# gmweir/PYFFT

Measured on AMD Instinct MI355X. Metric: Msamples/sec Welch-PSD 4096-pt Hann 50% overlap, complex64, higher is better.
Workload: dtype f32

## Files before the change

include/spectral.h:

```cpp
#ifndef SPECTRAL_H
#define SPECTRAL_H

#include <stdint.h>

#ifdef __cplusplus
extern "C" {
#endif

#define SP_DTYPE_F32 0
#define SP_DTYPE_C64 1

#define SP_SIDED_ONE 1
#define SP_SIDED_TWO 2
#define SP_SIDED_RAW 3
#define SP_SIDED_HALF 4

int sp_init(int device_id);
void sp_shutdown(void);
const char *sp_last_error(void);
int sp_set_stream(void *hip_stream);
int sp_synchronize(void);
int sp_version(void);
int sp_max_wg_fft(void);
int sp_profile_enable(int on);
int sp_profile_last_ms(double *ms);
const char *sp_profile_last_kernel(void);
int sp_device_info(int64_t out[4]);

int sp_fft_c2c(const void *in, void *out, int64_t n, int64_t batch, int direction, int mem);

#define SP_DETREND_CONST 0
#define SP_DETREND_MEAN 1
#define SP_DETREND_LINEAR 2
#define SP_DETREND_SEGMEAN 3
#define SP_DETREND_SEGLINEAR 4
int sp_welch_psd(const void *x, int x_dtype, int64_t nsig, const float *win, int nfft, int hop,
                 int64_t nframes, int detrend, double mean_re, double mean_im, int sided,
                 double scale, double *pxx_out, int mem);

int sp_welch_accum(const void *x, int x_dtype, int64_t nsig, const float *win, int nfft, int hop, int64_t nframes,
                   int64_t nmean, double *sum_out, int mem);
int sp_welch_finish(const double *mean, int64_t frames_total, int sided, double scale, double *pxx_out, int mem);
int sp_welch_export(const void *x, int x_dtype, int64_t nsig, const float *win, int nfft, int hop,
                    int64_t nframes, int64_t nmean, double *state, int mem);
int sp_welch_apply(const double *state, const float *win, int nfft, int64_t frames_total, int sided, double scale,
                   double *pxx_out, int mem);

#define SP_COMM_ID_BYTES 128
int sp_comm_unique_id(void *id_out );
int sp_comm_init(const void *id, int world, int rank);
int sp_comm_info(int out[2] );
int sp_comm_destroy(void);
int sp_welch_dist_submit(const void *x, int x_dtype, int64_t nsig, const float *win, int nfft, int hop, int64_t nframes,
                         int64_t nmean, int64_t frames_total, int sided, double scale, double *pxx_out, int *ndone);
int sp_welch_dist_flush(int *ndone);
int sp_welch_psd_dist(const void *x, int x_dtype, int64_t nsig, const float *win, int nfft, int hop, int64_t nframes,
                      int64_t nmean, int64_t frames_total, int sided, double scale, double *pxx_out);

int sp_welch_csd(const void *x, const void *y, int dtype, int64_t nsig, int nch, int64_t y_ld,
                 const float *win, int nfft, int hop, int64_t nframes, int detrend,
                 const double *mean_x , const double *mean_y , int sided,
                 double scale, double *pxx, double *pyy, double *pxy, int mem);

int sp_csd_matrix(const float *x, int nch, int64_t nsig, int64_t x_ld, const float *win, int nfft,
                  int hop, int64_t nframes, int detrend, double scale, double *g_out, int mem);
int sp_csd_matrix_means(const float *x, int nch, int64_t nsig, int64_t x_ld, const float *win, int nfft,
                        int hop, int64_t nframes, const double *means, double scale, double *g_out, int mem);
int sp_channel_means(const float *x, int nch, int64_t nsig, int64_t x_ld, double *means_out, int mem);

int sp_stft(const void *x, int x_dtype, int64_t nsig, const float *win, int nfft, int hop, int64_t nframes,
            int detrend, double mean_re, double mean_im, int sided, double amp_scale, int out_kind,
            int out_major, void *out, double *pseg_out, int mem);

int sp_istft(const void *Z, int sided, int in_major, int nch, int64_t nframes, const float *win, int nfft, int hop,
             double scale, int64_t skip, int64_t nout, void *y, int mem);

int sp_bispectrum(const void *x, const void *y, const void *z, int x_dtype, int64_t nsig, const float *win, int nfft, int hop,
                  int64_t nframes, int detrend, double mean_re, double mean_im, void *B_out, double *b2_out, double *pzz_out,
                  int mem);

int sp_stft_cog(const void *x, int x_dtype, int64_t nsig, const float *win, int nfft, int hop, int64_t nframes,
                int detrend, double mean_re, double mean_im, double fs, double fmin, double fmax, double *cog_out, int mem);

int sp_hilbert(const float *x, int64_t n_in, int64_t x_ld, int64_t nfft, int64_t batch, void *out, int mem);

int sp_frame_sum(const void *x, int x_dtype, int64_t nsig, int nch, int64_t x_ld, int nfft, int hop, int64_t nframes,
                 int detrend, double *out, int mem);

int sp_spectral_filter(const float *x, int64_t n_in, int64_t x_ld, int64_t nfft, int64_t batch, const void *H, void *out,
                       int mem);

int sp_xcorr(const float *x1, const float *x2, int64_t n, float *co_out, int mem);

int sp_fftfilt(const float *h, int ntaps, const float *x, int64_t n, int nfft, float *y, int mem);

int64_t sp_csd_epilogue_doubles(int nch, int nb, int nfft);
int sp_csd_epilogue(const double *pxx, const double *pyy, const double *pxy, int nch, int nb, int nfft, int onesided, double enbw,
                    double *out, int mem);

int sp_biquad(const double *b, const double *a, const float *x, int64_t n, float *y, int mem);

int sp_sosfilt(const double *sos, int nsec, const float *x, int64_t nrows, int64_t n, const double *zi, float *y, double *zf,
               int mem);
int sp_sosfiltfilt(const double *sos, int nsec, const float *x, int64_t nrows, int64_t n, int padtype, int64_t padlen, float *y,
                   int mem);

int sp_mean(const void *x, int x_dtype, int64_t n, double out[2], int mem);

#ifdef __cplusplus
}
#endif
#endif
```

pyfft_amd/_ffi.py:

```python
import ctypes as C
import os

import numpy as np

_HERE = os.path.dirname(os.path.abspath(__file__))
LIB_PATH = os.environ.get("SP_LIB_PATH") or os.path.join(_HERE, "lib", "libspectral.so")

DTYPE_F32, DTYPE_C64 = 0, 1
SIDED_ONE, SIDED_TWO, SIDED_RAW, SIDED_HALF = 1, 2, 3, 4
DETREND_CONST, DETREND_MEAN, DETREND_LINEAR, DETREND_SEGMEAN, DETREND_SEGLINEAR = 0, 1, 2, 3, 4

_lib = None

_vp, _i, _i64, _d = C.c_void_p, C.c_int, C.c_int64, C.c_double

SIGNATURES = {
    "sp_init": (_i, [_i]),
    "sp_shutdown": (None, []),
    "sp_last_error": (C.c_char_p, []),
    "sp_set_stream": (_i, [_vp]),
    "sp_synchronize": (_i, []),
    "sp_version": (_i, []),
    "sp_max_wg_fft": (_i, []),
    "sp_device_info": (_i, [C.POINTER(_i64)]),
    "sp_profile_enable": (_i, [_i]),
    "sp_profile_last_ms": (_i, [C.POINTER(_d)]),
    "sp_profile_last_kernel": (C.c_char_p, []),
    "sp_fft_c2c": (_i, [_vp, _vp, _i64, _i64, _i, _i]),
    "sp_welch_psd": (_i, [_vp, _i, _i64, _vp, _i, _i, _i64, _i, _d, _d, _i, _d, _vp, _i]),
    "sp_welch_accum": (_i, [_vp, _i, _i64, _vp, _i, _i, _i64, _i64, _vp, _i]),
    "sp_welch_finish": (_i, [_vp, _i64, _i, _d, _vp, _i]),
    "sp_welch_export": (_i, [_vp, _i, _i64, _vp, _i, _i, _i64, _i64, _vp, _i]),
    "sp_welch_apply": (_i, [_vp, _vp, _i, _i64, _i, _d, _vp, _i]),
    "sp_comm_unique_id": (_i, [_vp]),
    "sp_comm_init": (_i, [_vp, _i, _i]),
    "sp_comm_info": (_i, [C.POINTER(_i)]),
    "sp_comm_destroy": (_i, []),
    "sp_welch_dist_submit": (_i, [_vp, _i, _i64, _vp, _i, _i, _i64, _i64, _i64, _i, _d, _vp, C.POINTER(_i)]),
    "sp_welch_dist_flush": (_i, [C.POINTER(_i)]),
    "sp_welch_psd_dist": (_i, [_vp, _i, _i64, _vp, _i, _i, _i64, _i64, _i64, _i, _d, _vp]),
    "sp_welch_csd": (_i, [_vp, _vp, _i, _i64, _i, _i64, _vp, _i, _i, _i64, _i, _vp, _vp, _i, _d, _vp, _vp, _vp, _i]),
    "sp_csd_matrix": (_i, [_vp, _i, _i64, _i64, _vp, _i, _i, _i64, _i, _d, _vp, _i]),
    "sp_csd_matrix_means": (_i, [_vp, _i, _i64, _i64, _vp, _i, _i, _i64, _vp, _d, _vp, _i]),
    "sp_channel_means": (_i, [_vp, _i, _i64, _i64, _vp, _i]),
    "sp_stft": (_i, [_vp, _i, _i64, _vp, _i, _i, _i64, _i, _d, _d, _i, _d, _i, _i, _vp, _vp, _i]),
    "sp_istft": (_i, [_vp, _i, _i, _i, _i64, _vp, _i, _i, _d, _i64, _i64, _vp, _i]),
    "sp_bispectrum": (_i, [_vp, _vp, _vp, _i, _i64, _vp, _i, _i, _i64, _i, _d, _d, _vp, _vp, _vp, _i]),
    "sp_stft_cog": (_i, [_vp, _i, _i64, _vp, _i, _i, _i64, _i, _d, _d, _d, _d, _d, _vp, _i]),
    "sp_hilbert": (_i, [_vp, _i64, _i64, _i64, _i64, _vp, _i]),
    "sp_frame_sum": (_i, [_vp, _i, _i64, _i, _i64, _i, _i, _i64, _i, _vp, _i]),
    "sp_spectral_filter": (_i, [_vp, _i64, _i64, _i64, _i64, _vp, _vp, _i]),
    "sp_xcorr": (_i, [_vp, _vp, _i64, _vp, _i]),
    "sp_fftfilt": (_i, [_vp, _i, _vp, _i64, _i, _vp, _i]),
    "sp_biquad": (_i, [_vp, _vp, _vp, _i64, _vp, _i]),
    "sp_sosfilt": (_i, [_vp, _i, _vp, _i64, _i64, _vp, _vp, _vp, _i]),
    "sp_sosfiltfilt": (_i, [_vp, _i, _vp, _i64, _i64, _i, _i64, _vp, _i]),
    "sp_csd_epilogue_doubles": (_i64, [_i, _i, _i]),
    "sp_csd_epilogue": (_i, [_vp, _vp, _vp, _i, _i, _i, _i, _d, _vp, _i]),
    "sp_mean": (_i, [_vp, _i, _i64, C.POINTER(_d), _i]),
}


class SpectralError(RuntimeError):
    pass


def load_library():
    global _lib
    if _lib is not None:
        return _lib
    if not os.path.exists(LIB_PATH):
        raise SpectralError("libspectral.so not found at %s -- run `make` (or __graft_entry__.build()); "
                            "pyfft_amd has no CPU fallback" % LIB_PATH)
    lib = C.CDLL(LIB_PATH)
    for name, (res, args) in SIGNATURES.items():
        fn = getattr(lib, name)
        fn.restype = res
        fn.argtypes = args
    _lib = lib
    return lib


def lib():
    l = load_library()
    return l


def check(rc):
    if rc != 0:
        raise SpectralError((lib().sp_last_error() or b"unknown error").decode())


def init(device=-1):
    check(lib().sp_init(int(device)))


def ptr(a):
    if a is None:
        return None
    if isinstance(a, (int, np.integer)):
        return C.c_void_p(int(a))
    assert a.flags["C_CONTIGUOUS"]
    return C.c_void_p(a.ctypes.data)


def dtype_code(arr_dtype):
    if arr_dtype == np.float32:
        return DTYPE_F32
    if arr_dtype == np.complex64:
        return DTYPE_C64
    raise TypeError("device path takes float32 or complex64 samples, got %s" % arr_dtype)


def as_samples(x):
    x = np.asarray(x)
    if np.iscomplexobj(x):
        return np.ascontiguousarray(x, dtype=np.complex64)
    return np.ascontiguousarray(x, dtype=np.float32)
```

pyfft_amd/csrc/fft_core.h:

```cpp
#pragma once
#include <type_traits>
#include <hip/hip_runtime.h>

namespace sp {

typedef float2 cf;

__device__ __forceinline__ cf mk(float a, float b) { return make_float2(a, b); }
__device__ __forceinline__ cf operator+(cf a, cf b) { return mk(a.x + b.x, a.y + b.y); }
__device__ __forceinline__ cf operator-(cf a, cf b) { return mk(a.x - b.x, a.y - b.y); }
__device__ __forceinline__ cf operator*(float s, cf a) { return mk(s * a.x, s * a.y); }
__device__ __forceinline__ cf cmul(cf a, cf b) { return mk(a.x * b.x - a.y * b.y, a.x * b.y + a.y * b.x); }
__device__ __forceinline__ cf cmulc(cf a, cf b) { return mk(a.x * b.x + a.y * b.y, a.y * b.x - a.x * b.y); }
__device__ __forceinline__ cf cconj(cf a) { return mk(a.x, -a.y); }
__device__ __forceinline__ float cnorm(cf a) { return a.x * a.x + a.y * a.y; }

template <bool INV> __device__ __forceinline__ cf rot(cf a) { return INV ? mk(-a.y, a.x) : mk(a.y, -a.x); }
template <bool INV> __device__ __forceinline__ cf twc(cf a, float C, float S) {
    return INV ? mk(a.x * C - a.y * S, a.y * C + a.x * S) : mk(a.x * C + a.y * S, a.y * C - a.x * S);
}
template <bool INV> __device__ __forceinline__ cf twm(cf a, cf w) { return INV ? cmulc(a, w) : cmul(a, w); }

#define SP_C8 0.70710678118654752440f
#define SP_C16 0.92387953251128675613f
#define SP_S16 0.38268343236508977173f

template <bool INV> __device__ __forceinline__ void dft2(cf &a, cf &b) {
    cf t = a - b;
    a = a + b;
    b = t;
}

template <bool INV> __device__ __forceinline__ void dft4(cf &a, cf &b, cf &c, cf &d) {
    cf t0 = a + c, t1 = a - c, t2 = b + d, t3 = rot<INV>(b - d);
    a = t0 + t2;
    c = t0 - t2;
    b = t1 + t3;
    d = t1 - t3;
}

template <bool INV> __device__ __forceinline__ void dft8(cf (&x)[8]) {
    dft4<INV>(x[0], x[2], x[4], x[6]);
    dft4<INV>(x[1], x[3], x[5], x[7]);
    cf o1 = twc<INV>(x[3], SP_C8, SP_C8);
    cf o2 = rot<INV>(x[5]);
    cf o3 = twc<INV>(x[7], -SP_C8, SP_C8);
    cf e0 = x[0], e1 = x[2], e2 = x[4], e3 = x[6], o0 = x[1];
    x[0] = e0 + o0;
    x[4] = e0 - o0;
    x[1] = e1 + o1;
    x[5] = e1 - o1;
    x[2] = e2 + o2;
    x[6] = e2 - o2;
    x[3] = e3 + o3;
    x[7] = e3 - o3;
}

template <bool INV> __device__ __forceinline__ void dft16(cf (&x)[16]) {
#pragma unroll
    for (int b = 0; b < 4; ++b) dft4<INV>(x[b], x[b + 4], x[b + 8], x[b + 12]);
    x[5] = twc<INV>(x[5], SP_C16, SP_S16);
    x[9] = twc<INV>(x[9], SP_C8, SP_C8);
    x[13] = twc<INV>(x[13], SP_S16, SP_C16);
    x[6] = twc<INV>(x[6], SP_C8, SP_C8);
    x[10] = rot<INV>(x[10]);
    x[14] = twc<INV>(x[14], -SP_C8, SP_C8);
    x[7] = twc<INV>(x[7], SP_S16, SP_C16);
    x[11] = twc<INV>(x[11], -SP_C8, SP_C8);
    x[15] = twc<INV>(x[15], -SP_C16, -SP_S16);
#pragma unroll
    for (int c = 0; c < 4; ++c) dft4<INV>(x[4 * c], x[4 * c + 1], x[4 * c + 2], x[4 * c + 3]);
    cf t;
#define SP_SWAP(i, j) t = x[i]; x[i] = x[j]; x[j] = t;
    SP_SWAP(1, 4) SP_SWAP(2, 8) SP_SWAP(3, 12) SP_SWAP(6, 9) SP_SWAP(7, 13) SP_SWAP(11, 14)
#undef SP_SWAP
}

struct Tw16 {
    float f[40];
    static constexpr int TAU = 0, RB = 15, RC = 19, RD = 23, S1 = 27, S2 = 31, S3 = 35;
};

#define SP_T16 0.41421356237309504880f
#define SP_T316 2.41421356237309504880f

__device__ __forceinline__ void dft4s(cf &a, cf &b, cf &c, cf &d, float rb, float rc, float rd) {
    const cf t0 = mk(fmaf(rc, c.x, a.x), fmaf(rc, c.y, a.y));
    const cf t1 = mk(fmaf(-rc, c.x, a.x), fmaf(-rc, c.y, a.y));
    const cf t2 = mk(fmaf(rd, d.x, b.x), fmaf(rd, d.y, b.y));
    const cf t3 = mk(fmaf(-rd, d.x, b.x), fmaf(-rd, d.y, b.y));
    a = mk(fmaf(rb, t2.x, t0.x), fmaf(rb, t2.y, t0.y));
    c = mk(fmaf(-rb, t2.x, t0.x), fmaf(-rb, t2.y, t0.y));
    b = mk(fmaf(rb, t3.y, t1.x), fmaf(-rb, t3.x, t1.y));
    d = mk(fmaf(-rb, t3.y, t1.x), fmaf(rb, t3.x, t1.y));
}
__device__ __forceinline__ cf rot_tan(cf a, float t) { return mk(fmaf(t, a.y, a.x), fmaf(-t, a.x, a.y)); }

template <bool TWD, bool PREROT = false> __device__ __forceinline__ void dft16s(cf (&x)[16], const Tw16 &w) {
    if constexpr (TWD) {
        if constexpr (!PREROT) {
#pragma unroll
            for (int s = 1; s < 16; ++s) x[s] = rot_tan(x[s], w.f[Tw16::TAU + s - 1]);
        }
#pragma unroll
        for (int b = 0; b < 4; ++b) dft4s(x[b], x[b + 4], x[b + 8], x[b + 12], w.f[Tw16::RB + b], w.f[Tw16::RC + b], w.f[Tw16::RD + b]);
    } else {
#pragma unroll
        for (int b = 0; b < 4; ++b) dft4<false>(x[b], x[b + 4], x[b + 8], x[b + 12]);
    }
    x[5] = rot_tan(x[5], SP_T16);
    x[9] = mk(x[9].x + x[9].y, x[9].y - x[9].x);
    x[13] = rot_tan(x[13], SP_T316);
    x[6] = mk(x[6].x + x[6].y, x[6].y - x[6].x);
    x[10] = mk(x[10].y, -x[10].x);
    x[14] = mk(x[14].x - x[14].y, x[14].y + x[14].x);
    x[7] = rot_tan(x[7], SP_T316);
    x[11] = mk(x[11].x - x[11].y, x[11].y + x[11].x);
    x[15] = rot_tan(x[15], SP_T16);
    if constexpr (TWD) {
#pragma unroll
        for (int c = 0; c < 4; ++c) dft4s(x[4 * c], x[4 * c + 1], x[4 * c + 2], x[4 * c + 3], w.f[Tw16::S1 + c], w.f[Tw16::S2 + c], w.f[Tw16::S3 + c]);
    } else {
        dft4<false>(x[0], x[1], x[2], x[3]);
        dft4s(x[4], x[5], x[6], x[7], SP_C16, SP_C8, SP_S16 / SP_C16);
        dft4s(x[8], x[9], x[10], x[11], SP_C8, 1.f, -1.f);
        dft4s(x[12], x[13], x[14], x[15], SP_S16, -SP_C8, -SP_C16 / SP_S16);
    }
    cf t;
#define SP_SWAP(i, j) t = x[i]; x[i] = x[j]; x[j] = t;
    SP_SWAP(1, 4) SP_SWAP(2, 8) SP_SWAP(3, 12) SP_SWAP(6, 9) SP_SWAP(7, 13) SP_SWAP(11, 14)
#undef SP_SWAP
}

template <bool TWD, class Store, bool PREROT = false> __device__ __forceinline__ void dft16s_es(cf (&x)[16], const Tw16 &w, Store store) {
    if constexpr (TWD) {
        if constexpr (!PREROT) {
#pragma unroll
            for (int s = 1; s < 16; ++s) x[s] = rot_tan(x[s], w.f[Tw16::TAU + s - 1]);
        }
#pragma unroll
        for (int b = 0; b < 4; ++b) dft4s(x[b], x[b + 4], x[b + 8], x[b + 12], w.f[Tw16::RB + b], w.f[Tw16::RC + b], w.f[Tw16::RD + b]);
    } else {
#pragma unroll
        for (int b = 0; b < 4; ++b) dft4<false>(x[b], x[b + 4], x[b + 8], x[b + 12]);
    }
    x[5] = rot_tan(x[5], SP_T16);
    x[9] = mk(x[9].x + x[9].y, x[9].y - x[9].x);
    x[13] = rot_tan(x[13], SP_T316);
    x[6] = mk(x[6].x + x[6].y, x[6].y - x[6].x);
    x[10] = mk(x[10].y, -x[10].x);
    x[14] = mk(x[14].x - x[14].y, x[14].y + x[14].x);
    x[7] = rot_tan(x[7], SP_T316);
    x[11] = mk(x[11].x - x[11].y, x[11].y + x[11].x);
    x[15] = rot_tan(x[15], SP_T16);
    __builtin_amdgcn_sched_barrier(0);
#define SP_ES_OUT(c)                                                                                                 \
    store(c, x[4 * c]);                                                                                              \
    store(c + 4, x[4 * c + 1]);                                                                                      \
    store(c + 8, x[4 * c + 2]);                                                                                      \
    store(c + 12, x[4 * c + 3]);                                                                                     \
    __builtin_amdgcn_sched_barrier(0);
    if constexpr (TWD) {
        dft4s(x[0], x[1], x[2], x[3], w.f[Tw16::S1 + 0], w.f[Tw16::S2 + 0], w.f[Tw16::S3 + 0]);
        SP_ES_OUT(0)
        dft4s(x[4], x[5], x[6], x[7], w.f[Tw16::S1 + 1], w.f[Tw16::S2 + 1], w.f[Tw16::S3 + 1]);
        SP_ES_OUT(1)
        dft4s(x[8], x[9], x[10], x[11], w.f[Tw16::S1 + 2], w.f[Tw16::S2 + 2], w.f[Tw16::S3 + 2]);
        SP_ES_OUT(2)
        dft4s(x[12], x[13], x[14], x[15], w.f[Tw16::S1 + 3], w.f[Tw16::S2 + 3], w.f[Tw16::S3 + 3]);
        SP_ES_OUT(3)
    } else {
        dft4<false>(x[0], x[1], x[2], x[3]);
        SP_ES_OUT(0)
        dft4s(x[4], x[5], x[6], x[7], SP_C16, SP_C8, SP_S16 / SP_C16);
        SP_ES_OUT(1)
        dft4s(x[8], x[9], x[10], x[11], SP_C8, 1.f, -1.f);
        SP_ES_OUT(2)
        dft4s(x[12], x[13], x[14], x[15], SP_S16, -SP_C8, -SP_C16 / SP_S16);
        SP_ES_OUT(3)
    }
#undef SP_ES_OUT
}

__device__ __forceinline__ void dft4w(cf &a, cf &b, cf &c, cf &d, float wa, float wb, float wc, float wd) {
    const cf pa = mk(wa * a.x, wa * a.y), pb = mk(wb * b.x, wb * b.y);
    const cf t0 = mk(fmaf(wc, c.x, pa.x), fmaf(wc, c.y, pa.y));
    const cf t1 = mk(fmaf(-wc, c.x, pa.x), fmaf(-wc, c.y, pa.y));
    const cf t2 = mk(fmaf(wd, d.x, pb.x), fmaf(wd, d.y, pb.y));
    const cf t3 = mk(fmaf(-wd, d.x, pb.x), fmaf(-wd, d.y, pb.y));
    a = t0 + t2;
    c = t0 - t2;
    b = mk(t1.x + t3.y, t1.y - t3.x);
    d = mk(t1.x - t3.y, t1.y + t3.x);
}
struct NoMid {
    __device__ __forceinline__ void operator()(int) const {}
};
template <class Store, class Mid = NoMid> __device__ __forceinline__ void dft16s_es_win(cf (&x)[16], const float (&w)[16], Store store, Mid mid = Mid()) {
#pragma unroll
    for (int b = 0; b < 4; ++b) {
        dft4w(x[b], x[b + 4], x[b + 8], x[b + 12], w[b], w[b + 4], w[b + 8], w[b + 12]);
        if constexpr (!std::is_same<Mid, NoMid>::value) {
            if (b < 3) {
                __builtin_amdgcn_sched_barrier(0);
                mid(b);
                __builtin_amdgcn_sched_barrier(0);
            }
        }
    }
    x[5] = rot_tan(x[5], SP_T16);
    x[9] = mk(x[9].x + x[9].y, x[9].y - x[9].x);
    x[13] = rot_tan(x[13], SP_T316);
    x[6] = mk(x[6].x + x[6].y, x[6].y - x[6].x);
    x[10] = mk(x[10].y, -x[10].x);
    x[14] = mk(x[14].x - x[14].y, x[14].y + x[14].x);
    x[7] = rot_tan(x[7], SP_T316);
    x[11] = mk(x[11].x - x[11].y, x[11].y + x[11].x);
    x[15] = rot_tan(x[15], SP_T16);
    __builtin_amdgcn_sched_barrier(0);
#define SP_ES_OUT(c)                                                                                                 \
    store(c, x[4 * c]);                                                                                              \
    store(c + 4, x[4 * c + 1]);                                                                                      \
    store(c + 8, x[4 * c + 2]);                                                                                      \
    store(c + 12, x[4 * c + 3]);                                                                                     \
    __builtin_amdgcn_sched_barrier(0);
    dft4<false>(x[0], x[1], x[2], x[3]);
    SP_ES_OUT(0)
    dft4s(x[4], x[5], x[6], x[7], SP_C16, SP_C8, SP_S16 / SP_C16);
    SP_ES_OUT(1)
    dft4s(x[8], x[9], x[10], x[11], SP_C8, 1.f, -1.f);
    SP_ES_OUT(2)
    dft4s(x[12], x[13], x[14], x[15], SP_S16, -SP_C8, -SP_C16 / SP_S16);
    SP_ES_OUT(3)
#undef SP_ES_OUT
}

__device__ __forceinline__ void make_tw16(Tw16 &w, const cf (&wv)[15]) {
    float g[16];
    g[0] = 1.f;
    w.f[39] = 0.f;
#pragma unroll
    for (int s = 1; s < 16; ++s) {
        float c = wv[s - 1].x;
        if (fabsf(c) < 9.094947e-13f) c = c < 0.f ? -9.094947e-13f : 9.094947e-13f;
        g[s] = c;
        w.f[Tw16::TAU + s - 1] = -wv[s - 1].y / c;
    }
#pragma unroll
    for (int b = 0; b < 4; ++b) {
        w.f[Tw16::RB + b] = g[b + 4] / g[b];
        w.f[Tw16::RC + b] = g[b + 8] / g[b];
        w.f[Tw16::RD + b] = g[b + 12] / g[b + 4];
    }
    const float K1[4] = {1.f, SP_C16, SP_C8, SP_S16}, K2[4] = {1.f, SP_C8, 1.f, -SP_C8}, K3[4] = {1.f, SP_S16, -SP_C8, -SP_C16};
#pragma unroll
    for (int c = 0; c < 4; ++c) {
        w.f[Tw16::S1 + c] = g[1] * K1[c];
        w.f[Tw16::S2 + c] = g[2] * K2[c];
        w.f[Tw16::S3 + c] = (g[3] * K3[c]) / (g[1] * K1[c]);
    }
}

typedef float sp_f2v __attribute__((ext_vector_type(2)));
__device__ __forceinline__ cf lds_load_single(const cf *p) { return *p; }
template <int RDX, bool INV> __device__ __forceinline__ void dftR(cf (&x)[RDX]) {
    if constexpr (RDX == 2) dft2<INV>(x[0], x[1]);
    else if constexpr (RDX == 4) dft4<INV>(x[0], x[1], x[2], x[3]);
    else if constexpr (RDX == 8) dft8<INV>(x);
    else if constexpr (RDX == 16) dft16<INV>(x);
}

constexpr int ilog2c(int n) { return n <= 1 ? 0 : 1 + ilog2c(n >> 1); }

template <int N> struct FftPlan {
    static_assert(N >= 2 && (N & (N - 1)) == 0, "power of two");
    static constexpr int LOG2N = ilog2c(N);
    static constexpr int R = N < 16 ? N : 16;
    static constexpr int T = N / R;
    static constexpr int NP16 = N < 16 ? 0 : LOG2N / 4;
    static constexpr int REM = N < 16 ? N : (1 << (LOG2N % 4));
    static constexpr int NP = N < 16 ? 1 : NP16 + (REM > 1 ? 1 : 0);
    static constexpr int radix(int p) { return N < 16 ? N : (p < NP16 ? 16 : REM); }
    static constexpr int ns(int p) { int s = 1; for (int i = 0; i < p; ++i) s *= radix(i); return s; }
    static constexpr int ntw_before(int p) { int c = 0; for (int i = 1; i < p; ++i) c += (R / radix(i)) * (radix(i) - 1); return c; }
    static constexpr int NTW = ntw_before(NP);
    static constexpr int PITCH1 = T + 1;
    static constexpr int LDS_ELEMS = NP > 1 ? (R * PITCH1 > N ? R * PITCH1 : N) : 0;
};

#define SP_TW1_PITCH 44
template <int N, bool TW1LDS = false> struct WgFft {
    using PL = FftPlan<N>;
    static constexpr int R = PL::R, T = PL::T, NP = PL::NP;
    static constexpr int IMG0 = PL::LDS_ELEMS;
    static constexpr int N16 = PL::NP16 > 1 ? PL::NP16 - 1 : 0;
    static constexpr int NTR = (N >= 16 && PL::REM > 1) ? (R / PL::REM) * (PL::REM - 1) : 0;
    Tw16 t16[N16 > 0 ? N16 : 1];
    cf twr[NTR > 0 ? NTR : 1];
    const float *tw1 = nullptr;

    __device__ __forceinline__ void publish_tw1(float *table, int tid) {
        if constexpr (TW1LDS && N16 > 0) {
            if (tid < 16) {
#pragma unroll
                for (int j = 0; j < 40; ++j) table[tid * SP_TW1_PITCH + j] = t16[0].f[j];
            }
            tw1 = table;
        }
    }

    __device__ __forceinline__ void load_twiddles(const cf *__restrict__ table, int tid) {
        load_tw<1>(table, tid);
    }

    template <int P> __device__ __forceinline__ void load_tw(const cf *__restrict__ table, int tid) {
        if constexpr (P < NP) {
            constexpr int r = PL::radix(P), NS = PL::ns(P), NB = R / r;
            if constexpr (r == 16) {
                const int e = (tid % NS) * (N / (NS * 16));
                cf wv[15];
#pragma unroll
                for (int s = 1; s < 16; ++s) wv[s - 1] = table[e * s];
                make_tw16(t16[P - 1], wv);
            } else {
#pragma unroll
                for (int u = 0; u < NB; ++u) {
                    const int q = tid + T * u;
                    const int e = (q % NS) * (N / (NS * r));
#pragma unroll
                    for (int s = 1; s < r; ++s) twr[u * (r - 1) + (s - 1)] = table[e * s];
                }
            }
            load_tw<P + 1>(table, tid);
        }
    }

    template <int P> __device__ __forceinline__ void load_tw_one(const cf *__restrict__ table, int tid) {
        static_assert(P >= 1 && P < NP && PL::radix(P) == 16, "a twiddled radix-16 pass");
        constexpr int NS = PL::ns(P);
        const int e = (tid % NS) * (N / (NS * 16));
        cf wv[15];
#pragma unroll
        for (int s = 1; s < 16; ++s) wv[s - 1] = table[e * s];
        make_tw16(t16[P - 1], wv);
    }

    template <int E> static __device__ __forceinline__ int phys(int i) {
        if constexpr (E == 0) return (i % PL::radix(0)) * PL::PITCH1 + i / PL::radix(0);
        else return i;
    }

    template <int P> __device__ __forceinline__ void bfly(cf (&v)[R], int tid) const {
        constexpr int r = PL::radix(P), NB = R / r;
#pragma unroll
        for (int u = 0; u < NB; ++u) {
            cf x[r];
#pragma unroll
            for (int s = 0; s < r; ++s) x[s] = v[u + s * NB];
            if constexpr (r == 16) {
                if constexpr (TW1LDS && P == 1) {
                    Tw16 wl;
                    const float4 *row = reinterpret_cast<const float4 *>(tw1 + (tid % 16) * SP_TW1_PITCH);
#pragma unroll
                    for (int j = 0; j < 10; ++j) {
                        const float4 q = row[j];
                        wl.f[4 * j] = q.x;
                        wl.f[4 * j + 1] = q.y;
                        wl.f[4 * j + 2] = q.z;
                        wl.f[4 * j + 3] = q.w;
                    }
                    dft16s<true>(x, wl);
                } else if constexpr (P > 0) {
                    dft16s<true>(x, t16[P - 1]);
                } else {
                    dft16s<false>(x, t16[0]);
                }
            } else {
                if constexpr (P > 0) {
#pragma unroll
                    for (int s = 1; s < r; ++s) x[s] = twm<false>(x[s], twr[u * (r - 1) + (s - 1)]);
                }
                dftR<r, false>(x);
            }
#pragma unroll
            for (int s = 0; s < r; ++s) v[u + s * NB] = x[s];
        }
    }
    template <int P> __device__ __forceinline__ void scatter(const cf (&v)[R], cf *lds, int tid) const {
        constexpr int r = PL::radix(P), NS = PL::ns(P), NB = R / r;
#pragma unroll
        for (int u = 0; u < NB; ++u) {
            const int q = tid + T * u;
            const int base = (q / NS) * (NS * r) + (q % NS);
#pragma unroll
            for (int s = 0; s < r; ++s) lds[phys<P>(base + s * NS)] = v[u + s * NB];
        }
    }
    template <int P> __device__ __forceinline__ void gather(cf (&v)[R], const cf *lds, int tid) const {
        if constexpr (P == 0 && (T % 16) == 0 && PL::radix(0) == 16) {
            const int b = (tid % 16) * PL::PITCH1 + tid / 16;
#pragma unroll
            for (int t = 0; t < R; ++t) v[t] = lds_load_single(&lds[b + (T / 16) * t]);
        } else {
#pragma unroll
            for (int t = 0; t < R; ++t) v[t] = lds_load_single(&lds[phys<P>(tid + T * t)]);
        }
    }

    template <bool SINGLE, bool WL = false> __device__ __forceinline__ void run(cf (&v)[R], cf *lds0, cf *lds1, int tid) const {
        static_assert(!WL || T <= 64, "wave-local exchange: one wave holds the whole transform");
        pass<0, SINGLE, WL>(v, lds0, lds1, tid);
    }
    template <bool WL> static __device__ __forceinline__ void xsync() {
        if constexpr (WL) __builtin_amdgcn_wave_barrier();
        else __syncthreads();
    }

    template <int P> __device__ __forceinline__ void bfly_scatter(cf (&v)[R], cf *lds, int tid) const {
        constexpr int NS = PL::ns(P);
        const int base = (tid / NS) * (NS * 16) + (tid % NS);
        auto store = [&](int k, cf val) __attribute__((always_inline)) { lds[phys<P>(base + k * NS)] = val; };
        if constexpr (P > 0) dft16s_es<true>(v, t16[P - 1], store);
        else dft16s_es<false>(v, t16[0], store);
    }

    template <int P> __device__ __forceinline__ void load_tau_out(const cf *__restrict__ table, int tid, float (&tau)[16]) const {
        static_assert(P + 1 < NP && PL::radix(P) == 16 && PL::radix(P + 1) == 16 && R == 16, "between two radix-16 passes");
        constexpr int NS = PL::ns(P), NS2 = PL::ns(P + 1);
#pragma unroll
        for (int k = 0; k < 16; ++k) {
            const int p = (tid / NS) * (NS * 16) + (tid % NS) + k * NS;
            const int tc = p % T, sc = p / T;
            const int e = (tc % NS2) * (N / (NS2 * 16));
            const cf w = table[(e * sc) & (N - 1)];
            float c = w.x;
            if (fabsf(c) < 9.094947e-13f) c = c < 0.f ? -9.094947e-13f : 9.094947e-13f;
            tau[k] = sc == 0 ? 0.f : -w.y / c;
        }
    }
    template <int P, bool PREROT> __device__ __forceinline__ void bfly_scatter_rot(cf (&v)[R], const float (&tau)[16], cf *lds, int tid) const {
        constexpr int NS = PL::ns(P);
        const int base = (tid / NS) * (NS * 16) + (tid % NS);
        auto store = [&](int k, cf val) __attribute__((always_inline)) { lds[phys<P>(base + k * NS)] = rot_tan(val, tau[k]); };
        if constexpr (P > 0) dft16s_es<true, decltype(store), PREROT>(v, t16[P - 1], store);
        else dft16s_es<false>(v, t16[0], store);
    }
    __device__ __forceinline__ void bfly_scatter_win_rot(cf (&v)[R], const float (&w)[R], const float (&tau)[16], cf *lds, int tid) const {
        static_assert(R == 16, "radix-16 first pass");
        constexpr int NS = PL::ns(0);
        const int base = (tid / NS) * (NS * 16) + (tid % NS);
        auto store = [&](int k, cf val) __attribute__((always_inline)) { lds[phys<0>(base + k * NS)] = rot_tan(val, tau[k]); };
        dft16s_es_win(v, w, store);
    }
    template <int P> __device__ __forceinline__ void bfly_prerot(cf (&v)[R], int tid) const {
        (void)tid;
        static_assert(P > 0 && PL::radix(P) == 16 && R == 16, "a twiddled radix-16 pass");
        dft16s<true, true>(v, t16[P - 1]);
    }

    __device__ __forceinline__ void bfly_scatter_win(cf (&v)[R], const float (&w)[R], cf *lds, int tid) const {
        static_assert(R == 16, "radix-16 first pass");
        constexpr int NS = PL::ns(0);
        const int base = (tid / NS) * (NS * 16) + (tid % NS);
        auto store = [&](int k, cf val) __attribute__((always_inline)) { lds[phys<0>(base + k * NS)] = val; };
        dft16s_es_win(v, w, store);
    }

    template <int P, bool SINGLE, bool WL = false> __device__ __forceinline__ void pass(cf (&v)[R], cf *lds0, cf *lds1, int tid) const {
        constexpr bool LAST = (P == NP - 1);
        cf *lds = (P & 1) ? lds1 : lds0;
        if constexpr (!LAST && SINGLE) xsync<WL>();
        bfly<P>(v, tid);
        if constexpr (!LAST) {
            scatter<P>(v, lds, tid);
            xsync<WL>();
            gather<P>(v, lds, tid);
            pass<P + 1, SINGLE, WL>(v, lds0, lds1, tid);
        }
    }
};

}
```

pyfft_amd/csrc/k_welch_pipe.hip:

```cpp
#include "launch.h"
#include <type_traits>
#define SP_PIPE_AHEAD 2
namespace sp {

template <bool CPLX, int SHIFT, int MODE>
__global__ __launch_bounds__(768) void k_welch_pipe(const void *__restrict__ x_in, const float *__restrict__ win,
                                                     int64_t nframes, int64_t fpg, float *__restrict__ trend_in, XfTables tb,
                                                     float *__restrict__ partial, cf *__restrict__ spartial, int64_t x_cs, int gpr) {
    constexpr int N = 4096;
    constexpr bool RP = MODE >= 3 && MODE != 8 && MODE != 9;
    constexpr bool ONEPASS = MODE == 1 || MODE == 4 || MODE == 7 || MODE == 8 || MODE == 9, COG = MODE == 2 || MODE == 8;
    constexpr bool LOBE = MODE == 9;
    constexpr bool SPEC = MODE == 5 || MODE == 7;
    const void *x = SPEC ? (const void *)(reinterpret_cast<const float *>(x_in) + (int64_t)blockIdx.y * x_cs) : x_in;
    float *trend = SPEC ? trend_in + 4 * blockIdx.y : trend_in;
    static_assert(!RP || (!CPLX && SHIFT == 8), "the real-pair form is for real input at hop = nfft / 2");
    using PL = FftPlan<N>;
    using F = WgFft<N>;
    constexpr int T = PL::T, R = PL::R, KEEP = R - SHIFT, IMG = F::IMG0, IMGB = PL::LDS_ELEMS;
    static_assert(T == 256 && R == 16 && PL::NP == 3, "three radix-16 passes over 256 threads");
    extern __shared__ __attribute__((aligned(16))) unsigned char smem_raw[];
    cf *smem = reinterpret_cast<cf *>(smem_raw);
    cf *imgA = smem, *imgB = smem + 2 * IMG;
    const int role = __builtin_amdgcn_readfirstlane((int)threadIdx.x >> 8);
    const int tid = (int)threadIdx.x & 255;
    const int hop = SHIFT * T;

    cf mu;
    if constexpr (ONEPASS) {
        const int64_t span = (nframes - 1) * (int64_t)hop + N;
        const int64_t pitch = span / 16;
        constexpr int NU = SPEC ? 4 : 1, NTH = SPEC ? 3 * T : T, NWV = SPEC ? 12 : 4;
        const int lt = SPEC ? (int)threadIdx.x : tid;
        float sx = 0.f, sy = 0.f;
#pragma unroll
        for (int r = 0; r < 16; ++r)
#pragma unroll
            for (int u = 0; u < NU; ++u) {
                int64_t i = pitch * r + (int64_t)(lt + NTH * u);
                i = i < span ? i : span - 1;
                const cf v = load_sample(x, i, CPLX);
                sx += v.x;
                sy += v.y;
            }
        sx = wave_sum64(sx);
        sy = wave_sum64(sy);
        float *red = reinterpret_cast<float *>(smem);
        if ((SPEC || role == 0) && (tid & 63) == 0) {
            red[2 * (lt >> 6)] = sx;
            red[2 * (lt >> 6) + 1] = sy;
        }
        __syncthreads();
        double tx = 0.0, ty = 0.0;
#pragma unroll
        for (int wv = 0; wv < NWV; ++wv) {
            tx += (double)red[2 * wv];
            ty += (double)red[2 * wv + 1];
        }
        mu = mk((float)(tx / (16.0 * NTH * NU)), (float)(ty / (16.0 * NTH * NU)));
        __syncthreads();
        if (blockIdx.x == 0 && threadIdx.x == 0) {
            trend[0] = mu.x;
            trend[1] = mu.y;
            trend[2] = 0.f;
            trend[3] = 0.f;
        }
    } else {
        mu = load_trend(trend).m;
    }
    const int64_t gid = blockIdx.x;
    const int64_t g0 = gid * fpg;
    const int64_t last = nframes - 1;
    int64_t trips = (RP ? (nframes + 1) / 2 : nframes) - g0;
    trips = trips < 0 ? 0 : (trips > fpg ? fpg : trips);
    constexpr int DRAIN = 4;
    const int64_t periods = trips + DRAIN;
    F f;
    constexpr bool UPROT = !RP;
    float tau_out[16];
    if constexpr (UPROT) {
        if (role == 0) f.template load_tau_out<0>(tb.tw, tid, tau_out);
        else if (role == 1) f.template load_tau_out<1>(tb.tw, tid, tau_out);
    }

    if (role == 0 && RP) {
        const float *xr = reinterpret_cast<const float *>(x);
        float m = mu.x;
        asm volatile("" : "+v"(m));
        float w[R], sacc[SHIFT];
#pragma unroll
        for (int t = 0; t < R; ++t) w[t] = win[tid + T * t];
#pragma unroll
        for (int s = 0; s < SHIFT; ++s) sacc[s] = 0.f;
        auto issue_chunk = [&](float (&dst)[R], int64_t q) __attribute__((always_inline)) {
            const int64_t q1 = 2 * q <= nframes ? q : 0, q2 = 2 * q + 1 <= nframes ? q : 0;
            const float *b1 = xr + q1 * (int64_t)N, *b2 = xr + q2 * (int64_t)N;
#pragma unroll
            for (int t = 0; t < R; ++t) {
                const unsigned off = (unsigned)(tid + T * t);
                dst[t] = __builtin_nontemporal_load((t < R / 2 ? b1 : b2) + off);
            }
        };
        float ca[R], cb[R], cc[R];
        issue_chunk(ca, g0);
        issue_chunk(cb, g0 + 1);
#pragma unroll
        for (int t = 0; t < R; ++t) {
            ca[t] -= m;
            cb[t] -= m;
        }
        auto frame = [&](auto hb, int64_t i, cf *img, float (&cur)[R], float (&nxt)[R], float (&fill)[R]) __attribute__((always_inline)) {
            constexpr bool HB = decltype(hb)::value;
            issue_chunk(fill, g0 + i + 2);
            __builtin_amdgcn_sched_barrier(0);
            cf v[R];
            if constexpr (!ONEPASS) {
#pragma unroll
                for (int t = 0; t < R; ++t) v[t] = mk(cur[t], HB ? (t < R / 2 ? cur[t + R / 2] : nxt[t - R / 2]) : 0.f);
                if constexpr (UPROT) f.bfly_scatter_win_rot(v, w, tau_out, img, tid);
                else f.bfly_scatter_win(v, w, img, tid);
            } else {
#pragma unroll
                for (int t = 0; t < R; ++t) v[t] = mk(w[t] * cur[t], HB ? w[t] * (t < R / 2 ? cur[t + R / 2] : nxt[t - R / 2]) : 0.f);
                if constexpr (UPROT) f.template bfly_scatter_rot<0, false>(v, tau_out, img, tid);
                else f.template bfly_scatter<0>(v, img, tid);
            }
            __builtin_amdgcn_sched_barrier(0);
            if constexpr (ONEPASS) {
#pragma unroll
                for (int s = 0; s < SHIFT; ++s) sacc[s] += HB ? cur[R / 2 + s] + nxt[s] : cur[R / 2 + s];
            }
#pragma unroll
            for (int t = 0; t < R; ++t) fill[t] -= m;
        };
        const std::true_type yes;
        const std::false_type no;
        int64_t i = 0;
        for (; i + 6 < trips; i += 6) {
            frame(yes, i, imgA, ca, cb, cc);
            __syncthreads();
            frame(yes, i + 1, imgA + IMG, cb, cc, ca);
            __syncthreads();
            frame(yes, i + 2, imgA, cc, ca, cb);
            __syncthreads();
            frame(yes, i + 3, imgA + IMG, ca, cb, cc);
            __syncthreads();
            frame(yes, i + 4, imgA, cb, cc, ca);
            __syncthreads();
            frame(yes, i + 5, imgA + IMG, cc, ca, cb);
            __syncthreads();
        }
        for (; i < trips; ++i) {
            cf *img = (i & 1) ? imgA + IMG : imgA;
            const bool has_b = 2 * (g0 + i) + 1 < nframes;
            if (has_b) {
                if (i % 3 == 0) frame(yes, i, img, ca, cb, cc);
                else if (i % 3 == 1) frame(yes, i, img, cb, cc, ca);
                else frame(yes, i, img, cc, ca, cb);
            } else {
                if (i % 3 == 0) frame(no, i, img, ca, cb, cc);
                else if (i % 3 == 1) frame(no, i, img, cb, cc, ca);
                else frame(no, i, img, cc, ca, cb);
            }
            __syncthreads();
        }
#pragma unroll
        for (int d = 0; d < DRAIN; ++d) __syncthreads();
        if constexpr (ONEPASS) {
#pragma unroll
            for (int s = 0; s < SHIFT; ++s)
                spartial[((SPEC ? (int64_t)blockIdx.y * gridDim.x : 0) + gid) * hop + tid + T * s] = mk(sacc[s], 0.f);
        }
    } else if (role == 0) {
        asm volatile("" : "+v"(mu.x), "+v"(mu.y));
        float w[R];
        cf sacc[SHIFT], raw[R];
#pragma unroll
        for (int t = 0; t < R; ++t) w[t] = win[tid + T * t];
#pragma unroll
        for (int s = 0; s < SHIFT; ++s) sacc[s] = mk(0.f, 0.f);
        {
            const int64_t base = (g0 < nframes ? g0 : last) * hop + tid;
#pragma unroll
            for (int t = 0; t < R; ++t) raw[t] = load_sample(x, base + T * t, CPLX) - mu;
        }
        auto issue_part = [&](cf (&dst)[SHIFT], int64_t q, int s0, int s1) __attribute__((always_inline)) {
            const int64_t gq = g0 + q;
            const int64_t gn = gq < nframes ? gq : last;
            const int64_t ubase = gn * hop + (int64_t)T * KEEP;
#pragma unroll
            for (int s = s0; s < s1; ++s) {
                const unsigned off = (unsigned)(tid + T * s);
                if (CPLX) {
                    const sp_f2v r = __builtin_nontemporal_load(reinterpret_cast<const sp_f2v *>(x) + ubase + off);
                    dst[s] = mk(r.x, r.y);
                } else {
                    dst[s] = mk(__builtin_nontemporal_load(reinterpret_cast<const float *>(x) + ubase + off), 0.f);
                }
            }
        };
        auto issue = [&](cf (&dst)[SHIFT], int64_t q) __attribute__((always_inline)) { issue_part(dst, q, 0, SHIFT); };
        constexpr int AHEAD = (SP_PIPE_AHEAD >= 2 && SHIFT <= 8) ? (SP_PIPE_AHEAD >= 3 ? 3 : 2) : 1;
        constexpr bool SPREAD = AHEAD >= 2;
        auto frame = [&](int64_t i, cf *img, cf (&fill)[SHIFT], cf (&take)[SHIFT]) __attribute__((always_inline)) {
            if constexpr (SPREAD) issue_part(fill, i + AHEAD, 0, SHIFT / 4);
            else issue(fill, i + AHEAD);
            __builtin_amdgcn_sched_barrier(0);
            cf v[R];
            constexpr bool WINFOLD = SPREAD;
#pragma unroll
            for (int t = 0; t < R; ++t) v[t] = WINFOLD ? raw[t] : w[t] * raw[t];
            if constexpr (SPREAD) {
            {
                auto store = [&](int k, cf val) __attribute__((always_inline)) {
                    img[F::template phys<0>(tid * 16 + k)] = UPROT ? rot_tan(val, tau_out[k]) : val;
                    if (k >= 12 && k < 15) issue_part(fill, i + AHEAD, (k - 11) * (SHIFT / 4), (k - 10) * (SHIFT / 4));
                };
                if constexpr (WINFOLD) dft16s_es_win(v, w, store);
                else dft16s_es<false>(v, f.t16[0], store);
            }
            } else {
            if constexpr (UPROT) f.template bfly_scatter_rot<0, false>(v, tau_out, img, tid);
            else f.template bfly_scatter<0>(v, img, tid);
            }
            __builtin_amdgcn_sched_barrier(0);
#pragma unroll
            for (int s = 0; s < SHIFT; ++s)
                if constexpr (ONEPASS && !LOBE) sacc[s] = sacc[s] + raw[KEEP + s];
#pragma unroll
            for (int t = 0; t < KEEP; ++t) raw[t] = raw[t + SHIFT];
#pragma unroll
            for (int s = 0; s < SHIFT; ++s) raw[KEEP + s] = take[s] - mu;
        };
        int64_t i = 0;
        if constexpr (AHEAD == 3) {
            cf s0[SHIFT], s1[SHIFT], s2[SHIFT];
            issue(s1, 1);
            issue(s2, 2);
            for (; i + 2 < trips; i += 3) {
                frame(i, (i & 1) ? imgA + IMG : imgA, s0, s1);
                __syncthreads();
                frame(i + 1, ((i + 1) & 1) ? imgA + IMG : imgA, s1, s2);
                __syncthreads();
                frame(i + 2, ((i + 2) & 1) ? imgA + IMG : imgA, s2, s0);
                __syncthreads();
            }
            for (; i < trips; ++i) {
                cf *img = (i & 1) ? imgA + IMG : imgA;
                if (i % 3 == 0) frame(i, img, s0, s1);
                else if (i % 3 == 1) frame(i, img, s1, s2);
                else frame(i, img, s2, s0);
                __syncthreads();
            }
        } else if constexpr (AHEAD == 2) {
            cf nxa[SHIFT], nxb[SHIFT];
            issue(nxa, 1);
            for (; i + 1 < trips; i += 2) {
                frame(i, imgA, nxb, nxa);
                __syncthreads();
                frame(i + 1, imgA + IMG, nxa, nxb);
                __syncthreads();
            }
            if (i < trips) {
                frame(i, imgA, nxb, nxa);
                __syncthreads();
            }
        } else {
            for (; i + 1 < trips; i += 2) {
                cf nx0[SHIFT], nx1[SHIFT];
                frame(i, imgA, nx0, nx0);
                __syncthreads();
                frame(i + 1, imgA + IMG, nx1, nx1);
                __syncthreads();
            }
            if (i < trips) {
                cf nx0[SHIFT];
                frame(i, imgA, nx0, nx0);
                __syncthreads();
            }
        }
#pragma unroll
        for (int d = 0; d < DRAIN; ++d) __syncthreads();
#pragma unroll
        for (int s = 0; s < SHIFT; ++s)
            if constexpr (ONEPASS && !LOBE) spartial[gid * hop + tid + T * s] = sacc[s];
    } else if (role == 1) {
        f.template load_tw_one<1>(tb.tw, tid);
        cf va[R], vb[R];
        auto step = [&](cf (&fill)[R], cf (&use)[R], int64_t p, const cf *src, cf *dst) __attribute__((always_inline)) {
            if (p >= 1 && p <= trips) f.template gather<0>(fill, src, tid);
            if (p >= 2 && p <= trips + 1) {
                if constexpr (UPROT) f.template bfly_scatter_rot<1, true>(use, tau_out, dst, tid);
                else f.template bfly_scatter<1>(use, dst, tid);
            }
            __syncthreads();
        };
        for (int64_t p = 0; p < periods; p += 2) {
            step(va, vb, p, imgA + IMG, imgB);
            if (p + 1 < periods) step(vb, va, p + 1, imgA, imgB + IMGB);
        }
    } else {
        f.template load_tw_one<2>(tb.tw, tid);
        float acc[R];
#pragma unroll
        for (int t = 0; t < R; ++t) acc[t] = 0.f;
        cf bs_lo = mk(0.f, 0.f), bs_hi = mk(0.f, 0.f);
        const unsigned zlo = (unsigned)((tid >> 3) * 512 + (tid & 7));
        cf held[SPEC ? R : 1];
        cf va[R], vb[R];
        cf pend = mk(0.f, 0.f);
        auto flush = [&](int64_t i) __attribute__((always_inline)) {
            const int sel = (int)(i & 63), li = tid & 63;
            const int64_t gg = g0 + (i - sel) + li;
            if (li <= sel && gg < nframes) reinterpret_cast<cf *>(partial)[(int64_t)(tid >> 6) * nframes + gg] = pend;
        };
        auto step = [&](cf (&fill)[R], cf (&use)[R], int64_t p, const cf *src) __attribute__((always_inline)) {
            if (p >= 3 && p <= trips + 2) {
                f.template gather<1>(fill, src, tid);
            }
            if (p >= 4 && p <= trips + 3) {
                if constexpr (UPROT) f.template bfly_prerot<2>(use, tid);
                else f.template bfly<2>(use, tid);
                if constexpr (SPEC) {
                    const int64_t pr = g0 + (p - 4);
                    const bool lone = (pr & 1) == 0 && p == trips + 3;
                    if ((pr & 1) == 0 && !lone) {
#pragma unroll
                        for (int t = 0; t < R; ++t) held[t] = use[t];
                    } else {
                        float4 *zb = reinterpret_cast<float4 *>(partial) + ((pr >> 1) * (int64_t)gpr * 512 + (int64_t)blockIdx.y * 8);
                        unsigned bl = zlo;
                        asm volatile("" : "+v"(bl));
#pragma unroll
                        for (int t = 0; t < R; ++t) {
                            const float4 q = lone ? make_float4(use[t].x, use[t].y, 0.f, 0.f)
                                                  : make_float4(held[t].x, held[t].y, use[t].x, use[t].y);
                            st_stream(zb + (bl + 16384u * t), q);
                        }
                    }
                } else if constexpr (COG) {
                    if constexpr (MODE == 8) {
                        const int64_t gf = g0 + (p - 4);
                        cf *lobe = reinterpret_cast<cf *>(partial) + 4 * nframes + gf * 8;
                        if (gf < nframes) {
                            if (tid <= 3) lobe[3 + tid] = use[0];
                            if (tid >= T - 3) lobe[3 - (T - tid)] = use[R - 1];
                        }
                    }
                    float numc = 0.f, den = 0.f;
#pragma unroll
                    for (int t = 0; t < R; ++t) {
                        const float pw = cnorm(use[t]);
                        numc = fmaf(pw, (float)(T * t - (t >= R / 2 ? N : 0)), numc);
                        den += pw;
                    }
                    float num = fmaf((float)tid, den, numc);
                    num = wave_sum64(num);
                    den = wave_sum64(den);
                    const int64_t i = p - 4;
                    if ((tid & 63) == (int)(i & 63)) pend = mk(num, den);
                    if ((i & 63) == 63 || i == trips - 1) flush(i);
                } else {
#pragma unroll
                    for (int t = 0; t < R; ++t) acc[t] = fmaf(use[t].y, use[t].y, fmaf(use[t].x, use[t].x, acc[t]));
                    if constexpr (LOBE) {
                        bs_lo = bs_lo + use[0];
                        bs_hi = bs_hi + use[R - 1];
                    }
                }
            }
            __syncthreads();
        };
        for (int64_t p = 0; p < periods; p += 2) {
            step(va, vb, p, imgB + IMGB);
            if (p + 1 < periods) step(vb, va, p + 1, imgB);
        }
        if constexpr (!COG && !SPEC) {
#pragma unroll
            for (int t = 0; t < R; ++t) partial[gid * N + tid + T * t] = acc[t];
            if constexpr (LOBE) {
                if (tid <= 3) spartial[gid * 8 + 3 + tid] = bs_lo;
                if (tid >= T - 3) spartial[gid * 8 + 3 - (T - tid)] = bs_hi;
                if (tid == 4) spartial[gid * 8 + 7] = mk(0.f, 0.f);
            }
        }
    }
}

bool welch_pipe_eligible(const Xf &xf, int hop) {
    return !xf.blue && xf.L == 4096 && (hop == 2048 || hop == 1024 || hop == 4096);
}

int launch_welch_pipe(LaunchCtx c, const void *x, bool cplx, const float *win, int hop, int64_t nframes, float *trend,
                      const Xf &xf, float *partial, const RunPart &rp, cf *spartial, int mode, int nch, int64_t x_cs, int gpr) {
    const size_t lds = sizeof(cf) * 4 * (size_t)FftPlan<4096>::LDS_ELEMS;
#define PIPE_(CP, S, OP)                                                                                  \
    {                                                                                                 \
        static bool once = false;                                                                     \
        if (!once) {                                                                                  \
            if (hipFuncSetAttribute((const void *)k_welch_pipe<CP, S, OP>, hipFuncAttributeMaxDynamicSharedMemorySize, (int)lds) != hipSuccess) \
                return -1;                                                                            \
            once = true;                                                                              \
        }                                                                                             \
        if (c.stop)                                                                                   \
            hipExtLaunchKernelGGL((k_welch_pipe<CP, S, OP>), dim3(rp.blocks, gy), dim3(768), lds, c.stream, nullptr, c.stop, 0, x, win, \
                                  nframes, rp.fpg, trend, xf.tb, partial, spartial, x_cs, gpr);       \
        else                                                                                          \
            hipLaunchKernelGGL((k_welch_pipe<CP, S, OP>), dim3(rp.blocks, gy), dim3(768), lds, c.stream, x, win, nframes, rp.fpg, trend, \
                               xf.tb, partial, spartial, x_cs, gpr);                                  \
    }
    const int shift = hop / 256;
    const unsigned gy = mode == 5 ? (unsigned)nch : 1u;
#define PIPE_S_(CP, OP)                                                                               \
    if (shift == 8) PIPE_(CP, 8, OP) else if (shift == 4) PIPE_(CP, 4, OP) else PIPE_(CP, 16, OP)
    if (mode == 5) {
        if (cplx || shift != 8 || nch < 1 || gpr < 1) return -1;
        if (spartial) PIPE_(false, 8, 7) else PIPE_(false, 8, 5)
    } else if (mode == 3) {
        if (cplx || shift != 8) return -1;
        if (spartial) PIPE_(false, 8, 4) else PIPE_(false, 8, 3)
    } else if (mode == 2 && spartial) {
        if (shift == 8) { if (cplx) PIPE_(true, 8, 8) else PIPE_(false, 8, 8) }
        else if (shift == 4) { if (cplx) PIPE_(true, 4, 8) else PIPE_(false, 4, 8) }
        else return -1;
    } else if (mode == 2) {
        if (cplx) { PIPE_S_(true, 2) } else { PIPE_S_(false, 2) }
    } else if (mode == 9) {
        if (!spartial || shift == 16) return -1;
        if (shift == 8) { if (cplx) PIPE_(true, 8, 9) else PIPE_(false, 8, 9) }
        else { if (cplx) PIPE_(true, 4, 9) else PIPE_(false, 4, 9) }
    } else if (spartial) {
        if (cplx) { PIPE_S_(true, 1) } else { PIPE_S_(false, 1) }
    } else {
        if (cplx) { PIPE_S_(true, 0) } else { PIPE_S_(false, 0) }
    }
#undef PIPE_S_
#undef PIPE_
    return 0;
}

}
```

pyfft_amd/csrc/launch.h:

```cpp
#pragma once
#include <stdlib.h>
#include "kernels.h"
#include <hip/hip_runtime.h>
#include <hip/hip_ext.h>

namespace sp {

inline bool env_flag(const char *name) {
    const char *v = getenv(name);
    return v && v[0] && v[0] != '0';
}
inline int env_int(const char *name, int dflt) {
    const char *v = getenv(name);
    return v ? atoi(v) : dflt;
}

struct LaunchCtx {
    hipStream_t stream;
    int ncu;
    hipEvent_t stop = nullptr;
};

struct Xf {
    XfTables tb;
    int L;
    bool blue;
};

inline int fpw_of(int L) {
    const int R = L < 16 ? L : 16, T = L / R, WG = T >= 256 ? T : 256;
    return WG / T;
}

struct RunPart {
    int64_t groups, fpg;
    int blocks;
};
inline RunPart run_partition(int L, int64_t nframes, int ncu, int groups_per_cu = 0) {
    if (groups_per_cu <= 0) groups_per_cu = 4;
    const int fpw = fpw_of(L);
    const int64_t target = (int64_t)ncu * groups_per_cu * fpw;
    int64_t f = (nframes + target - 1) / target;
    if (f < 1) f = 1;
    const int64_t G = (nframes + f - 1) / f;
    RunPart r;
    r.fpg = f;
    r.blocks = (int)((G + fpw - 1) / fpw);
    r.groups = (int64_t)r.blocks * fpw;
    return r;
}
inline RunPart run_partition_2d(int L, int64_t nframes, int ncu, int ny, int64_t slots = 0) {
    const int fpw = fpw_of(L);
    int64_t target = ((int64_t)ncu * 8 + ny - 1) / (ny > 0 ? ny : 1) * fpw;
    if (target < 8 * fpw) target = 8 * fpw;
    int64_t f = (nframes + target - 1) / target;
    if (f < 1) f = 1;
    if (slots > 0 && ny > 0) {
        const int64_t wg = ((nframes + f - 1) / f + fpw - 1) / fpw * ny;
        int64_t rounds = (wg + slots / 2) / slots;
        if (rounds < 1) rounds = 1;
        const int64_t groups = rounds * slots / ny * fpw;
        if (groups >= 1) {
            const int64_t f2 = (nframes + groups - 1) / groups;
            if (f2 >= 1 && f2 <= 4 * f) f = f2;
        }
    }
    const int64_t G = (nframes + f - 1) / f;
    RunPart r;
    r.fpg = f;
    r.blocks = (int)((G + fpw - 1) / fpw);
    r.groups = (int64_t)r.blocks * fpw;
    return r;
}
inline int strided_blocks(int L, int64_t items, int ncu, int per_cu = 4) {
    const int fpw = fpw_of(L);
    int64_t b = (items + fpw - 1) / fpw;
    int64_t cap = (int64_t)ncu * (L >= 4096 ? per_cu : 16);
    if (L == 2048) {
        const int64_t q = b / 4;
        if (q < cap) cap = q > (int64_t)ncu * 2 ? q : (int64_t)ncu * 2;
    }
    if (b > cap) b = cap;
    if (b < 1) b = 1;
    return (int)b;
}

int resident_per_cu(const void *fn, int threads, size_t lds_bytes);
int welch_rp_groups_per_cu(const Xf &xf, bool lin);
int csd_pair_resident(const Xf &xf, bool lin, bool onepass);
int stft_rp_groups_per_cu(const Xf &xf, bool lin, int hop, int sided, int out_power, bool pseg);

int launch_fft_c2c(LaunchCtx c, const cf *in, cf *out, int64_t batch, int inverse, const Xf &xf,
                   BigTw bt = BigTw{nullptr, nullptr, 0, 0});
int launch_fft_cols(LaunchCtx c, const cf *in, cf *out, int64_t ncols, int64_t nouter, int64_t es, int64_t os, int64_t twmul,
                    int conj_in, const Xf &xf, BigTw bt, int64_t hmask_n = 0,
                    ColsIn ci = ColsIn{0, nullptr, nullptr, nullptr, 0}, int tw_outer = 0);
int launch_fft_rows_rev(LaunchCtx c, const cf *in, cf *out, int64_t A, int64_t B, int conj_out, float scale, const Xf &xf,
                        RowsOut ro = RowsOut{nullptr, 0, 0, nullptr});
int launch_transpose_c(LaunchCtx c, const cf *in, cf *out, int64_t rows, int64_t cols, int conj, float scale, int64_t batch = 1);
int launch_pack_real(LaunchCtx c, const float *x, int64_t n_in, const double *mean, int64_t L, cf *out);
int launch_cmul_vec(LaunchCtx c, const cf *a, const cf *b, int64_t n, int conj_out, cf *out, int64_t batch = 1);
int launch_blue_pre(LaunchCtx c, const cf *in, const cf *chirp, int64_t n, int64_t L, int conj_in, cf *out, int64_t batch = 1);
int launch_blue_post(LaunchCtx c, const cf *in, const cf *chirp, int64_t n, int conj_out, float scale, cf *out, int64_t batch = 1,
                     int64_t in_ld = 0);
int launch_hilbert_mask(LaunchCtx c, cf *X, int64_t n);
int launch_xc_pack(LaunchCtx c, const float *x1, const float *x2, int64_t n, int64_t L, const double *mom, cf *z);
int launch_xc_mid(LaunchCtx c, const cf *Z, int64_t L, cf *R);
int launch_xc_mid_half(LaunchCtx c, const cf *Z, int64_t L, BigTw bt, cf *Zp);
int launch_xc_out(LaunchCtx c, const cf *r, int64_t n, int64_t L, const double *mom, float *co);
bool welch_carry_eligible(const Xf &xf, int hop, bool lin);
int launch_welch(LaunchCtx c, const void *x, bool cplx, const float *win, int hop, int64_t nframes, const float *trend,
                 bool lin, const Xf &xf, float *partial, const RunPart &rp, bool allow_carry, cf *spartial,
                 const char **kname, int segmean = 0);
bool welch_pipe_eligible(const Xf &xf, int hop);
int launch_welch_pipe(LaunchCtx c, const void *x, bool cplx, const float *win, int hop, int64_t nframes, float *trend,
                      const Xf &xf, float *partial, const RunPart &rp, cf *spartial, int mode = 0, int nch = 1, int64_t x_cs = 0,
                      int gpr = 0);
int launch_op_estimate(LaunchCtx c, const void *x, bool cplx, int64_t nsig, double *part, float *trend);
int launch_op_reduce(LaunchCtx c, const void *x, bool cplx, const float *trend, const float *partial, const cf *spartial,
                     int64_t G, const Xf &xf, int hop, int64_t nframes, int64_t nmean, OnePass st, double *sum_out);
int launch_op_finish(LaunchCtx c, const void *x, bool cplx, const float *trend, const float *win, OnePass st,
                     const double *mean_in, int64_t nmean, const Xf &xf, int hop, int64_t nframes, cf *cw, const cf *Wf,
                     int sided, double scale, double *out, bool export_state = false);
int launch_op_apply(LaunchCtx c, const double *state, const cf *Wf, int n, int sided, double scale, double *out,
                    const double *mean = nullptr);
int opx_tot_blocks();
int launch_welch_opx(LaunchCtx c, const void *x, bool cplx, bool pair, const float *win, int hop, int64_t nframes,
                     const float *trend, const Xf &xf, const RunPart &rp, float *partial, cf *cpart);
int launch_opx_reduce(LaunchCtx c, const float *partial, const cf *cpart, int64_t G, const Xf &xf, const void *x, bool cplx,
                      const float *trend, int hop, int64_t nframes, int64_t nmean, double *A, double *csum, double *tpart);
int launch_opx_finish(LaunchCtx c, const float *win, const double *A, const double *csum, const double *tpart, const float *trend,
                      int hop, int64_t nframes, int64_t nmean, bool sym, const Xf &xf, double *out);
int launch_op_fused(LaunchCtx c, const void *x, bool cplx, const float *trend, const float *win, const float *partial,
                    const cf *spartial, int64_t G, int n, int hop, int64_t nframes, int64_t nmean, OnePass st, unsigned *ticket,
                    CogLobe lb, const double *mean_in, int sided, double scale, double *out, bool export_state,
                    OpPrev prev = OpPrev{nullptr, nullptr, nullptr, 0, 0.0}, bool light = false, double cola_c = 0.0);
int launch_welch_finish(LaunchCtx c, const float *partial, int64_t G, const Xf &xf, int sided, double scale, double *out,
                        int sym = 0);
int launch_welch_rp(LaunchCtx c, const float *x, const float *win, int hop, int64_t nframes, const float *trend, bool lin,
                    const Xf &xf, float *partial, const RunPart &rp);
int launch_stft_rp(LaunchCtx c, const float *x, const float *win, int hop, int64_t nframes, const float *trend, bool lin,
                   const Xf &xf, const RunPart &rp, int sided, float amp, int out_power, void *out, double *pseg,
                   int nchan = 1, int64_t x_cs = 0, int64_t out_cs = 0, int out_ld = 0);
int launch_csd(LaunchCtx c, const void *x, const void *y, bool cplx, int nch, int64_t y_ld, const float *win, int hop,
               int64_t nframes, const float *trend_x, const float *trend_y, bool lin, const Xf &xf, float *partial,
               const RunPart &rp, int segmean = 0);
int launch_csd_finish(LaunchCtx c, const float *partial, int64_t G, const Xf &xf, int nch, int sided, double scale,
                      double *pxx, double *pyy, double *pxy);
int launch_stft(LaunchCtx c, const void *x, bool cplx, const float *win, int hop, int64_t nframes, const float *trend,
                bool lin, const Xf &xf, const RunPart &rp, int sided, float amp, int out_power, void *out, double *pseg, int segmean = 0,
                cf *cog = nullptr, int klo = 0, int khi = 0);
int launch_cog_finish(LaunchCtx c, const cf *acc, int wpf, int64_t nframes, double df, double *out);
int launch_cog_carry(LaunchCtx c, const void *x, bool cplx, const float *win, int hop, int64_t nframes, const float *trend,
                     const Xf &xf, cf *cog, const RunPart &rp, int klo, int khi);
bool csd_rp_eligible(const Xf &xf);
int launch_csd_rp(LaunchCtx c, const float *x, const float *y, int nch, int64_t y_ld, const float *win, int hop,
                  int64_t nframes, const float *trend_x, const float *trend_y, bool lin, const Xf &xf, float *partial,
                  const RunPart &rp);
int launch_csd_rp_finish(LaunchCtx c, const float *partial, int64_t G, const Xf &xf, int nch, int sided, double scale,
                         double *pxx, double *pyy, double *pxy);
int launch_pairspec(LaunchCtx c, const float *x, const float *win, int hop, int64_t nframes, const float *trend, bool lin,
                    const Xf &xf, const RunPart &rp, cf *Zx);
int launch_csd_pair(LaunchCtx c, const float *y, int nch, int64_t y_ld, const float *win, int hop, int64_t nframes,
                    float *trend_y, bool lin, const Xf &xf, const cf *Zx, float *partial, const RunPart &rp, cf *spartial = nullptr);
int launch_csd_pair_finish(LaunchCtx c, const float *partial, int64_t G, const Xf &xf, int nch, int sided, double scale,
                           double *pyy, double *pxy, const double *st_y = nullptr, const double *st_x = nullptr, const cf *Wf = nullptr,
                           const float *trend_x = nullptr, const float *trend_y = nullptr, int64_t nmean = 0, int64_t M = 0);
#define SP_COLSUM_SLICES 256
int launch_colsum_real(LaunchCtx c, const float *x, const float *trend, int H, int64_t M, cf *out);
int launch_csdm_finish(LaunchCtx c, double *G, int nch, int nb, double scale);
int launch_csdm_transpose_kgc(LaunchCtx c, const cf *Xs, cf *Xt, int nch, int nchp, int64_t m, int64_t mp, int nb);
int launch_csdm_mfma(LaunchCtx c, const cf *Xt, int nch, int nchp, int64_t mp, int nb, double *G);
int launch_csdm_bf16(LaunchCtx c, const cf *Xs, cf *Xt_tail, int nch, int64_t m, int nb, double *G, int ld, int two_pieces = 0, int init = 0);
int launch_csdm_fold(LaunchCtx c, const double *H, double *G, int nch, int n, const double *st = nullptr, const cf *Wf = nullptr,
                     const float *trend = nullptr, int64_t nmean = 0, int64_t M = 0, double scale = 1.0, int init = 0);
int launch_cm_blocksums(LaunchCtx c, const cf *spartial, int nch, int runs, int hop, double *Sl);
int launch_op_finish_channels(LaunchCtx c, const void *x, int64_t x_cs, int nch, const float *trend, const float *win,
                              const double *Sl, const cf *Wf, int hop, int64_t nframes, int64_t nmean, const Xf &xf, double *out,
                              bool cplx = false);
int launch_cog_finish_op(LaunchCtx c, const cf *acc, int wpf, int64_t nframes, double df, double *out, const cf *lobe, CogLobe lb,
                         const double *st, const float *trend, int64_t nmean, int n);
int launch_csdm_fused(LaunchCtx c, const cf *Xs, cf *Xt_tail, int nch, int64_t m, int nb, double *G, int ld = 0);
int launch_hilbert_mid(LaunchCtx c, cf *Z, int64_t M, BigTw bt);
int launch_hilbert_rowsmid(LaunchCtx c, cf *Tm, int64_t A, int64_t B, const Xf &xc, BigTw btN, const cf *tw2c);
int launch_xc_rowsmid(LaunchCtx c, cf *Tm, int64_t A, int64_t B, const Xf &xc, const Xf &xc2, BigTw btL, BigTw btM);
int launch_fft_cols_lag(LaunchCtx c, const cf *in, int64_t ncols, int64_t nouter, int64_t es, int64_t os, const Xf &xf, RowsOut ro);
int launch_fft_cols_inv(LaunchCtx c, const cf *in, cf *out, int64_t ncols, int64_t nouter, int64_t es, int64_t os, int64_t twmul,
                        const Xf &xf, BigTw bt, float scale, const RowsOut *analytic);
int launch_hilbert(LaunchCtx c, const float *x, int64_t n_in, int64_t x_ld, int64_t batch, const Xf &xf, cf *out,
                   const cf *H = nullptr);
int launch_spec_mul(LaunchCtx c, cf *X, const cf *H, int64_t n);
int frame_sum_slices(int ncu, int nch, int nfft, int64_t nframes);
int launch_frame_sum(LaunchCtx c, const void *x, bool cplx, int64_t x_ld, int nch, int nfft, int hop, int64_t nframes,
                     const float *trend, bool lin, double *out, double *part);
int launch_fftfilt(LaunchCtx c, const float *x, int64_t n, int ntaps, const cf *Hs, const Xf &xf, float *y);
int launch_xcorr(LaunchCtx c, const float *x1, const float *x2, int64_t n, const double *mom, const Xf &xf, float *co);
int launch_moments(LaunchCtx c, const void *x, bool cplx, int64_t n, int mode, double *partial_scratch, double *out_d,
                   float *trend_f, int nsignals = 1, int64_t x_cs = 0);
int launch_moments_xc(LaunchCtx c, const float *x, int64_t n, double *partial, double *out_d, double *xc_out, int64_t x_cs);
int launch_transpose(LaunchCtx c, const void *in, void *out, int64_t rows, int64_t cols, int elem_bytes);
int launch_long_segstats(LaunchCtx c, const void *x, bool cplx, int64_t f0, int64_t m, int hop, int nfft, int mode, float *rec);
int launch_long_pack(LaunchCtx c, const void *x, bool cplx, const float *win, int nfft, int hop, int64_t f0, int64_t m,
                     const float *trend, bool lin, const float *segrec, cf *S, double *pseg);
int launch_long_acc_psd(LaunchCtx c, const cf *S, int64_t m, int nfft, double *acc);
int launch_long_acc_csd(LaunchCtx c, const cf *Sx, const cf *Sy, int64_t m, int nfft, double *ayy, double *axy);
int launch_long_finish(LaunchCtx c, const double *acc, int nfft, int sided, double scale, bool cplx, double *out);
int launch_long_stft_out(LaunchCtx c, const cf *S, int64_t m, int nfft, int sided, float amp, int out_power, void *out,
                         int64_t f0, int nb);
int launch_long_cog(LaunchCtx c, const cf *S, int64_t m, int nfft, int klo, int khi, cf *acc, int64_t f0);

int64_t biquad_tiles(int64_t n);
int launch_biquad(LaunchCtx c, const double *b, const double *a, const float *x, int64_t n, float *y, double *work);

#define SP_SOS_MAXK 8
struct SosIO {
    const float *x;
    int64_t x_ld, n;
    int64_t len;
    int64_t pad;
    int padtype;
    int rev;
    float *y;
    int64_t y_ld, out_off, out_n;
};
int64_t sos_tiles(int64_t len);
int64_t sos_work_doubles(int nsec, int64_t len, int64_t nrows);
int sos_plan_doubles(int nsec);
void sos_build_plan(const double *sos, int nsec, int64_t len, double *plan);
int launch_sos_pass(LaunchCtx c, int nsec, const double *plan, const SosIO &io, int64_t nrows, int zmode, const double *zi,
                    double *zf, double *work);

int launch_epi_elem(LaunchCtx c, const double *pxx, const double *pyy, const double *pxy, int nch, int nb, int nfft, int onesided,
                    double enbw, double *cxy, double *cxy2, double *phi, double *lxx, double *lyy, double *lxy);
int launch_epi_spec(LaunchCtx c, const double *pxx, const double *pyy, const double *pxy, const double *cxy, int nch, int nb,
                    int nfft, int onesided, cf *X, double *rowmax );
int launch_epi_corr(LaunchCtx c, const cf *X, int nch, int nfft, int onesided, double *rxx, double *ryy, double *rxy, double *icxy,
                    double *ee, double *cc, const double *rowmax);

int bispec_tile_dim();
int bispec_frame_chunk();
size_t bispec_part_floats();
int launch_bispec_tile(LaunchCtx c, const cf *X, const cf *Y, const cf *Z, int nb, int c0, int64_t m, const int2 *tiles, int ntiles,
                       float *part);
int launch_bispec_pzz(LaunchCtx c, const cf *Z, int nb, int64_t m, double *ppart);
int launch_bispec_reduce(LaunchCtx c, const float *part, const double *ppart, int ntiles, int64_t m, int nb, int first, double *acc,
                         double *p64);
int launch_bispec_finish(LaunchCtx c, const double *acc, const double *p64, const int *tmap, int ntd, int nb, int c0, int sym, int64_t M,
                         void *B, double *b2, double *pzz);
int launch_bispec_trend_shift(LaunchCtx c, const float *src, float *dst, int nrec, int64_t off);

int istft_resident(const Xf &xf, int mode);
int launch_istft(LaunchCtx c, const cf *Z, int64_t z_cs, int64_t zbase, int64_t M, int64_t fbeg, int64_t fend, int64_t fpg, int halo,
                 const float *win, float wscale, int hop, const Xf &xf, int mode, const float *rcp, int64_t head_len, int64_t skip,
                 int64_t nout, void *y, int nch, int emit_tail);
int launch_istft_gather(LaunchCtx c, const cf *in, int64_t M, int nb, int64_t f0, int64_t m, cf *out, int nch);

#define SP_CASE_P(Lv, MACRO) case Lv: { MACRO(XfPow2<Lv>) } break;
#define SP_CASE_B(Lv, MACRO) case Lv: { MACRO(XfBlue<Lv>) } break;
#define SP_DISPATCH_X(xf, MACRO)                                                                      \
    if (!(xf).blue) {                                                                                 \
        switch ((xf).L) {                                                                             \
            SP_CASE_P(2, MACRO) SP_CASE_P(4, MACRO) SP_CASE_P(8, MACRO) SP_CASE_P(16, MACRO)          \
            SP_CASE_P(32, MACRO) SP_CASE_P(64, MACRO) SP_CASE_P(128, MACRO) SP_CASE_P(256, MACRO)     \
            SP_CASE_P(512, MACRO) SP_CASE_P(1024, MACRO) SP_CASE_P(2048, MACRO) SP_CASE_P(4096, MACRO) \
            SP_CASE_P(8192, MACRO)                                                                    \
            default: return -1;                                                                       \
        }                                                                                             \
    } else {                                                                                          \
        switch ((xf).L) {                                                                             \
            SP_CASE_B(16, MACRO) SP_CASE_B(32, MACRO) SP_CASE_B(64, MACRO) SP_CASE_B(128, MACRO)      \
// ... 16 lines not shown
```

pyfft_amd/csrc/spectral.hip:

```cpp
#include "../../include/spectral.h"
#include "launch.h"
#include "table_cache.h"

#include <hip/hip_runtime.h>
#include <rccl/rccl.h>
#include <dlfcn.h>
#include <limits.h>
#include <math.h>
#include <stdarg.h>
#include <stdio.h>
#include <stdlib.h>
#include <string.h>

#include <map>
#include <mutex>
#include <string>
#include <vector>

using namespace sp;

#define SP_VERSION 107
#define SP_MAX_WG_FFT 8192
#define SP_MAX_BIG_LOG2 26

namespace {

thread_local std::string g_err;

int fail(const char *fmt, ...) {
    char buf[512];
    va_list ap;
    va_start(ap, fmt);
    vsnprintf(buf, sizeof buf, fmt, ap);
    va_end(ap);
    g_err = buf;
    return -1;
}

#define HIPCHK(expr)                                                                                  \
    do {                                                                                              \
        hipError_t e_ = (expr);                                                                       \
        if (e_ != hipSuccess) return fail("%s failed: %s (%s:%d)", #expr, hipGetErrorString(e_), __FILE__, __LINE__); \
    } while (0)
#define LAUNCHCHK(expr)                                                                               \
    do {                                                                                              \
        if ((expr) != 0) return fail("%s: no kernel instantiated for this transform length (%s:%d)", #expr, __FILE__, __LINE__); \
        HIPCHK(hipGetLastError());                                                                    \
    } while (0)

struct Scratch {
    void *p = nullptr;
    size_t cap = 0;
    int ensure(size_t bytes) {
        if (bytes <= cap) return 0;
        if (p) (void)hipFree(p);
        p = nullptr;
        cap = 0;
        size_t want = bytes + (bytes >> 3) + 4096;
        if (hipMalloc(&p, want) != hipSuccess) return fail("hipMalloc(%zu) failed", want);
        cap = want;
        return 0;
    }
    void release() {
        if (p) (void)hipFree(p);
        p = nullptr;
        cap = 0;
    }
};

struct BlueTab {
    cf *chirp, *bf;
    int L;
};

struct Ctx {
    bool ready = false;
    int device = 0;
    int ncu = 256;
    hipStream_t stream = nullptr;
    std::map<int64_t, cf *> twiddles;
    std::map<int64_t, BlueTab> blue;
    Scratch in0, in1, out0, work, small, trends, onepass, ticket, epi;
    Scratch pend_trend;
    Scratch bigA, bigB, bigT, blueA, blueB, longrec;
    Scratch sosY, sosZ;
    Scratch bsIn, bsS, bsP, bsA;
    Scratch cmS, cmT, cmG, cmH, cmO;
    std::map<int64_t, BigTw> bigtw;
    std::map<int64_t, BlueTab> blue_big;
    std::mutex mu;
    bool profile = false, prof_valid = false;
    hipEvent_t ev0 = nullptr, ev1 = nullptr, ev_sw = nullptr;
    const char *last_kernel = "";
} g;

LaunchCtx lc() { return LaunchCtx{g.stream, g.ncu}; }

struct Pending {
    bool valid = false;
    const void *xd = nullptr;
    bool cplx = false;
    int64_t nsig = 0, nframes = 0, nmean = 0;
    int nfft = 0, hop = 0;
    Xf xf;
    const float *win_d = nullptr;
    const cf *Wf = nullptr;
    OnePass st;
    float *trend_f = nullptr;
    cf *cw = nullptr;
    double *sum_d = nullptr;
    double *state = nullptr;
} g_pend;

struct ProfScope {
    bool on;
    hipStream_t st;
    explicit ProfScope(hipStream_t s = nullptr) : on(g.profile), st(s ? s : g.stream) {
        if (on) (void)hipEventRecord(g.ev0, st);
    }
    ~ProfScope() {
        if (on) {
            (void)hipEventRecord(g.ev1, st);
            g.prof_valid = true;
        }
    }
};

int ensure_init() {
    if (g.ready) return 0;
    return sp_init(-1);
}

bool is_pow2(int64_t n) { return n >= 1 && (n & (n - 1)) == 0; }
int64_t next_pow2(int64_t n) {
    int64_t p = 1;
    while (p < n) p <<= 1;
    return p;
}

int get_twiddles(int64_t n, const cf **out) {
    auto it = g.twiddles.find(n);
    if (it != g.twiddles.end()) {
        *out = it->second;
        return 0;
    }
    std::vector<cf> h((size_t)n);
    for (int64_t m = 0; m < n; ++m) {
        const double a = -2.0 * M_PI * (double)m / (double)n;
        h[(size_t)m] = make_float2((float)cos(a), (float)sin(a));
    }
    cf *d = nullptr;
    HIPCHK(hipMalloc((void **)&d, sizeof(cf) * (size_t)n));
    HIPCHK(hipMemcpy(d, h.data(), sizeof(cf) * (size_t)n, hipMemcpyHostToDevice));
    g.twiddles[n] = d;
    *out = d;
    return 0;
}

int get_xf(int64_t n, Xf *xf) {
    if (n < 2) return fail("transform length %lld too short", (long long)n);
    if (is_pow2(n) && n <= SP_MAX_WG_FFT) {
        xf->L = (int)n;
        xf->blue = false;
        xf->tb.n = (int)n;
        xf->tb.chirp = xf->tb.bf = nullptr;
        return get_twiddles(n, &xf->tb.tw);
    }
    int64_t L = next_pow2(2 * n - 1);
    if (L < 16) L = 16;
    if (L > SP_MAX_WG_FFT)
        return fail("transform length %lld not supported yet (powers of two up to %d, other lengths up to %d)",
                    (long long)n, SP_MAX_WG_FFT, SP_MAX_WG_FFT / 2);
    xf->L = (int)L;
    xf->blue = true;
    xf->tb.n = (int)n;
    if (get_twiddles(L, &xf->tb.tw)) return -1;
    auto it = g.blue.find(n);
    if (it == g.blue.end()) {
        std::vector<cf> ch((size_t)n), bw((size_t)L, make_float2(0.f, 0.f));
        for (int64_t m = 0; m < n; ++m) {
            const int64_t q = (m * m) % (2 * n);
            const double a = M_PI * (double)q / (double)n;
            ch[(size_t)m] = make_float2((float)cos(a), (float)-sin(a));
            const cf b = make_float2((float)(cos(a) / (double)L), (float)(sin(a) / (double)L));
            bw[(size_t)m] = b;
            if (m > 0) bw[(size_t)(L - m)] = b;
        }
        BlueTab t;
        t.L = (int)L;
        HIPCHK(hipMalloc((void **)&t.chirp, sizeof(cf) * (size_t)n));
        HIPCHK(hipMalloc((void **)&t.bf, sizeof(cf) * (size_t)L));
        HIPCHK(hipMemcpy(t.chirp, ch.data(), sizeof(cf) * (size_t)n, hipMemcpyHostToDevice));
        HIPCHK(hipMemcpy(t.bf, bw.data(), sizeof(cf) * (size_t)L, hipMemcpyHostToDevice));
        Xf p2;
        if (get_xf(L, &p2)) return -1;
        LAUNCHCHK(launch_fft_c2c(lc(), t.bf, t.bf, 1, 0, p2));
        HIPCHK(hipStreamSynchronize(g.stream));
        g.blue[n] = t;
        it = g.blue.find(n);
    }
// ... 314 lines not shown
    }
    const int64_t L = is_pow2(n) ? n : next_pow2(2 * n - 1);
    if (L > ((int64_t)1 << SP_MAX_BIG_LOG2))
        return fail("transform length %lld needs a %lld-point multi-pass transform; the limit is 2^%d", (long long)n,
                    (long long)L, SP_MAX_BIG_LOG2);
    int64_t slice = (int64_t)(SP_LONG_SLICE_BYTES / (sizeof(cf) * (size_t)L));
    if (slice < 1) slice = 1;
    if (slice > 32768) slice = 32768;
    if (is_pow2(n)) {
        for (int64_t b0 = 0; b0 < batch; b0 += slice) {
            const int64_t m = batch - b0 < slice ? batch - b0 : slice;
            if (dev_fft_big_pow2(in + b0 * n, out + b0 * n, n, inverse, 0, m)) return -1;
        }
        return 0;
    }
    BlueTab bt;
    if (get_blue_big(n, &bt)) return -1;
    if (slice > batch) slice = batch;
    if (g.blueA.ensure(sizeof(cf) * (size_t)L * (size_t)slice)) return -1;
    cf *A = (cf *)g.blueA.p;
    for (int64_t b0 = 0; b0 < batch; b0 += slice) {
        const int64_t m = batch - b0 < slice ? batch - b0 : slice;
        LAUNCHCHK(launch_blue_pre(lc(), in + b0 * n, bt.chirp, n, L, inverse, A, m));
        if (dev_fft_big_pow2(A, A, L, 0, 0, m)) return -1;
        LAUNCHCHK(launch_cmul_vec(lc(), A, bt.bf, L, 0, A, m));
        if (dev_fft_big_pow2(A, A, L, 1, 0, m)) return -1;
        LAUNCHCHK(launch_blue_post(lc(), A, bt.chirp, n, inverse, inverse ? (float)(1.0 / (double)n) : 1.f, out + b0 * n, m, L));
    }
    return 0;
}


#define SP_LONG_CHUNK_BYTES ((size_t)192 << 20)
int64_t long_chunk_frames(int nfft, int64_t nframes) {
    int64_t m = (int64_t)(SP_LONG_CHUNK_BYTES / (sizeof(cf) * (size_t)nfft));
    if (m > 32768) m = 32768;
    if (m > nframes) m = nframes;
    if (m < 1) m = 1;
    return m;
}
int long_spectra(const void *xd, bool cplx, const float *win_d, int nfft, int hop, int64_t f0, int64_t m, const float *trend,
                 bool lin, int segmean, cf *buf, double *pseg_d) {
    const float *rec = nullptr;
    if (segmean) {
        if (g.longrec.ensure(sizeof(float) * 4 * (size_t)m)) return -1;
        LAUNCHCHK(launch_long_segstats(lc(), xd, cplx, f0, m, hop, nfft, segmean, (float *)g.longrec.p));
        rec = (const float *)g.longrec.p;
    }
    LAUNCHCHK(launch_long_pack(lc(), xd, cplx, win_d, nfft, hop, f0, m, trend, lin, rec, buf, pseg_d));
    return dev_fft_any(buf, buf, nfft, m, 0);
}


int get_window_spectrum(const float *win, int nfft, const Xf &xf, void **Wf_d) {
    bool fresh = false;
    if (get_table_keyed(3, win, sizeof(float) * (size_t)nfft, nullptr, sizeof(cf) * (size_t)nfft, Wf_d, &fresh)) return -1;
    if (fresh) {
        std::vector<cf> wc((size_t)nfft);
        for (int i = 0; i < nfft; ++i) wc[(size_t)i] = make_float2(win[i], 0.f);
        HIPCHK(hipMemcpy(*Wf_d, wc.data(), sizeof(cf) * (size_t)nfft, hipMemcpyHostToDevice));
        LAUNCHCHK(launch_fft_c2c(lc(), (const cf *)*Wf_d, (cf *)*Wf_d, 1, 0, xf));
    }
    return 0;
}

#define SP_PIPE_MINFPC_DEFAULT 2
static bool welch_pipe_wanted(const Xf &xf, int hop, int64_t nframes) {
    const int mode = env_int("SP_WELCH_PIPE", 1);
    const int64_t minfpc = SP_PIPE_MINFPC_DEFAULT;
    return welch_pipe_eligible(xf, hop) && (mode >= 2 || (mode == 1 && nframes >= minfpc * (int64_t)g.ncu - minfpc));
}

static bool cog_window_lobe(const float *win, int n, CogLobe *lb) {
    struct Entry {
        uint64_t key;
        int n;
        bool ok;
        CogLobe lb;
    };
    static std::vector<Entry> cache;
    const uint64_t h = mix_key(window_key(win, n), 11, 0);
    for (const Entry &e : cache)
        if (e.key == h && e.n == n) {
            *lb = e.lb;
            return e.ok;
        }
    Entry e{h, n, false, CogLobe{}};
    double tot = 0.0;
    for (int i = 0; i < n; ++i) tot += (double)win[i] * (double)win[i];
    tot *= (double)n;
    double in = 0.0, peak = 0.0;
    CogLobe l{};
    l.K = 3;
    for (int ks = -3; ks <= 3; ++ks) {
        double re = 0.0, im = 0.0;
        for (int i = 0; i < n; ++i) {
            const double a = -2.0 * M_PI * (double)(((int64_t)ks * i) % n) / (double)n;
            re += (double)win[i] * std::cos(a);
            im += (double)win[i] * std::sin(a);
        }
        l.wr[ks + 3] = re;
        l.wi[ks + 3] = im;
        in += re * re + im * im;
        if (re * re + im * im > peak) peak = re * re + im * im;
    }
    e.ok = peak > 0.0 && std::fabs(tot - in) <= 1e-9 * tot;
    e.lb = l;
    if (cache.size() < 64) cache.push_back(e);
    *lb = l;
    return e.ok;
}


static bool window_cola(const float *win, int n, int hop, double *c_out) {
    struct Entry {
        uint64_t key;
        int n, hop;
        bool ok;
        double c;
    };
    static std::vector<Entry> cache;
    if (hop < 1 || n % hop != 0) return false;
    const uint64_t h = mix_key(window_key(win, n), 7, (uint64_t)hop);
    for (const Entry &e : cache)
        if (e.key == h && e.n == n && e.hop == hop) {
            *c_out = e.c;
            return e.ok;
        }
    double lo = 1e300, hi = -1e300, sum = 0.0;
    for (int i = 0; i < hop; ++i) {
        double c = 0.0;
        for (int j = i; j < n; j += hop) c += (double)win[j];
        lo = c < lo ? c : lo;
        hi = c > hi ? c : hi;
        sum += c;
    }
    Entry e{h, n, hop, false, sum / (double)hop};
    e.ok = e.c > 0.0 && (hi - lo) <= 2e-6 * e.c;
    if (cache.size() < 64) cache.push_back(e);
    *c_out = e.c;
    return e.ok;
}

struct FusedOut {
    bool export_state;
    int sided;
    double scale;
    double *out;
    bool done;
    OpPrev prev = OpPrev{nullptr, nullptr, nullptr, 0, 0.0};
    hipEvent_t prev_wait = nullptr;
    bool prev_done = false;
};
unsigned *get_ticket(Scratch &t) {
    if (!t.p) {
        if (t.ensure(1024)) return nullptr;
        if (hipMemset(t.p, 0, 1024) != hipSuccess) return nullptr;
    }
    return (unsigned *)t.p;
}
struct SplitLaunch {
    Scratch *work, *onepass, *trend, *ticket;
    hipStream_t epi;
    hipEvent_t ev_main;
    int reserve_cus = 0;
};

int welch_export_generic(const void *xd, bool cplx, int64_t nsig, const float *win, int nfft, int hop, int64_t nframes,
                         int64_t nmean, const Xf &xf, double *st_d, const void **win_out = nullptr, const SplitLaunch *sl = nullptr) {
    Scratch &S_work = sl ? *sl->work : g.work, &S_trend = sl ? *sl->trend : g.pend_trend;
    void *win_d;
    if (get_table(1, win, sizeof(float) * (size_t)nfft, &win_d, nullptr)) return -1;
    if (win_out) *win_out = win_d;
    void *Wf_d;
    if (get_window_spectrum(win, nfft, xf, &Wf_d)) return -1;
    if (S_trend.ensure(256)) return -1;
    float *trend = (float *)S_trend.p;
    const bool pair = !cplx && nframes >= 2 && !env_flag("SP_NO_REALPAIR");
    const int ncu_p = (sl && sl->reserve_cus > 0 && sl->reserve_cus < g.ncu) ? g.ncu - sl->reserve_cus : g.ncu;
    const RunPart rp = run_partition(xf.L, pair ? (nframes + 1) / 2 : nframes, ncu_p);
    auto pad = [](size_t b) { return (b + 255) & ~(size_t)255; };
    const size_t b_part = pad(sizeof(float) * (size_t)rp.groups * xf.L), b_cpart = pad(sizeof(cf) * (size_t)rp.groups * nfft);
    const size_t b_red = pad(sizeof(double) * (3 * (size_t)nfft + 2 * (size_t)opx_tot_blocks()));
    if (S_work.ensure(b_part + b_cpart + b_red)) return -1;
    char *w0 = (char *)S_work.p;
    float *partial = (float *)w0;
    cf *cpart = (cf *)(w0 + b_part);
    double *A = (double *)(w0 + b_part + b_cpart), *csum = A + nfft, *tpart = csum + 2 * (size_t)nfft;
    const LaunchCtx mc = lc();
    LAUNCHCHK(launch_op_estimate(mc, xd, cplx, nsig, nullptr, trend));
    {
        ProfScope ps(mc.stream);
        LAUNCHCHK(launch_welch_opx(mc, xd, cplx, pair, (const float *)win_d, hop, nframes, trend, xf, rp, partial, cpart));
    }
    g.last_kernel = pair ? "k_welch_opx(realpair)" : "k_welch_opx";
    LaunchCtx ec = mc;
    if (sl) {
        HIPCHK(hipEventRecord(sl->ev_main, mc.stream));
        HIPCHK(hipStreamWaitEvent(sl->epi, sl->ev_main, 0));
        ec = LaunchCtx{sl->epi, g.ncu};
    }
    LAUNCHCHK(launch_opx_reduce(ec, partial, cpart, rp.groups, xf, xd, cplx, trend, hop, nframes, nmean, A, csum, tpart));
    LAUNCHCHK(launch_opx_finish(ec, (const float *)win_d, A, csum, tpart, trend, hop, nframes, nmean, pair, xf, st_d));
    return 0;
}

int welch_accum_locked(const void *xd, bool cplx, int64_t nsig, const float *win, int nfft, int hop, int64_t nframes,
                       int64_t nmean, bool want_sum, FusedOut *fo = nullptr, const SplitLaunch *sl = nullptr) {
    Scratch &S_work = sl ? *sl->work : g.work, &S_one = sl ? *sl->onepass : g.onepass, &S_trend = sl ? *sl->trend : g.pend_trend;
    Scratch &S_ticket = sl ? *sl->ticket : g.ticket;
    if (!wg_capable(nfft))
        return fail("sharded / split Welch PSD (sp_welch_accum, sp_welch_export, sp_welch_dist_*): segments longer than one workgroup "
                    "transform are not sharded (nfft = %d; powers of two up to %d, other lengths up to %d) -- the "
                    "long-segment regime has few, large frames: run sp_welch_psd on one GPU", nfft, SP_MAX_WG_FFT, SP_MAX_WG_FFT / 2);
    Xf xf;
    if (get_xf(nfft, &xf)) return -1;
    if (nmean < 1 || nmean > nsig) return fail("sp_welch_accum: nmean must be in [1, nsig]");
    if (!welch_carry_eligible(xf, hop, false)) {
        if (nmean > nframes * (int64_t)hop + nfft - 1)
            return fail("one-pass Welch: %lld own samples (nmean) cannot belong to %lld frames of %d with hop %d (at most "
                        "nframes * hop + nfft - 1 = %lld)", (long long)nmean, (long long)nframes, nfft, hop,
                        (long long)(nframes * (int64_t)hop + nfft - 1));
        if (fo && fo->export_state) {
            if (welch_export_generic(xd, cplx, nsig, win, nfft, hop, nframes, nmean, xf, fo->out, nullptr, sl)) return -1;
            fo->done = true;
            g_pend.valid = false;
            return 0;
        }
        if (fo || sl) return fail("internal: generic one-pass Welch exports its state only");
        if (S_one.ensure(sizeof(double) * (5 * (size_t)nfft + 8))) return -1;
        double *st_d = (double *)S_one.p;
        const void *win_d = nullptr;
        if (welch_export_generic(xd, cplx, nsig, win, nfft, hop, nframes, nmean, xf, st_d, &win_d)) return -1;
        void *Wf_d;
        if (get_window_spectrum(win, nfft, xf, &Wf_d)) return -1;
        g_pend = Pending{};
        g_pend.valid = true;
        g_pend.xd = xd;
        g_pend.cplx = cplx;
        g_pend.nsig = nsig;
        g_pend.nframes = nframes;
        g_pend.nmean = nmean;
        g_pend.nfft = nfft;
        g_pend.hop = hop;
        g_pend.xf = xf;
        g_pend.win_d = (const float *)win_d;
        g_pend.Wf = (const cf *)Wf_d;
        g_pend.state = st_d;
        g_pend.sum_d = st_d + 5 * (size_t)nfft + 3;
        return 0;
    }
    void *win_d;
    if (get_table(1, win, sizeof(float) * (size_t)nfft, &win_d, nullptr)) return -1;
    void *Wf_d;
    if (get_window_spectrum(win, nfft, xf, &Wf_d)) return -1;
    if (S_trend.ensure(256)) return -1;
    TrendBuf tb{(float *)S_trend.p, nullptr};
    const bool realpair = !cplx && 2 * hop == nfft && nframes >= 2 && !env_flag("SP_NO_REALPAIR") &&
                          welch_pipe_wanted(xf, hop, (nframes + 1) / 2);
    const bool pipe = realpair || ((hop != nfft || env_int("SP_WELCH_PIPE", 1) >= 2) && welch_pipe_wanted(xf, hop, nframes));
    const int ncu_p = (sl && sl->reserve_cus > 0 && sl->reserve_cus < g.ncu) ? g.ncu - sl->reserve_cus : g.ncu;
    const RunPart rp = realpair ? run_partition(xf.L, (nframes + 1) / 2, ncu_p, 1)
                                : (pipe ? run_partition(xf.L, nframes, ncu_p, 1) : run_partition(xf.L, nframes, g.ncu));
    if (S_work.ensure(sizeof(float) * (size_t)rp.groups * xf.L)) return -1;
    const size_t sp_bytes = sizeof(cf) * (size_t)rp.groups * (size_t)hop;
    const size_t st_doubles = (size_t)nfft + 2 * (size_t)hop + 8;
    const size_t sp_pad = (sp_bytes + 255) & ~(size_t)255;
    const size_t st_pad = (sizeof(double) * st_doubles + 255) & ~(size_t)255;
    if (S_one.ensure(sp_pad + st_pad + sizeof(cf) * (size_t)nfft)) return -1;
    cf *spartial = (cf *)S_one.p;
    double *stp = (double *)((char *)S_one.p + sp_pad);
    OnePass st;
    st.A = stp;
    st.Sl = stp + nfft;
    st.tot = st.Sl + 2 * (size_t)hop;
    st.dlt = st.tot + 2;
    double *sum_d = st.dlt + 2;
    cf *cw = (cf *)((char *)S_one.p + sp_pad + st_pad);
    float *partial = (float *)S_work.p;
    double *est = moments_scratch();
    if (!est) return -1;
    (void)est;
    st.sym = realpair ? 1 : 0;
    CogLobe lobe{};
    double cola_c = 0.0;
    const bool fused_ok = fo && !want_sum && !env_flag("SP_OP_UNFUSED") && cog_window_lobe(win, nfft, &lobe);
    const bool lobesum = fused_ok && pipe && !realpair && hop != nfft && !env_flag("SP_OP_NOLOBESUM") && window_cola(win, nfft, hop, &cola_c);
    if (!lobesum) cola_c = 0.0;
    const LaunchCtx mc = lc();
    const bool stop_ev = sl && pipe && !g.profile;
    if (pipe) {
        ProfScope ps(mc.stream);
        LaunchCtx mcs = mc;
        if (stop_ev) mcs.stop = sl->ev_main;
        LAUNCHCHK(launch_welch_pipe(mcs, xd, cplx, (const float *)win_d, hop, nframes, tb.f, xf, partial, rp, spartial,
                                    realpair ? 3 : (lobesum ? 9 : 0)));
        g.last_kernel = realpair ? "k_welch_pipe(onepass,realpair)" : (lobesum ? "k_welch_pipe(onepass,lobesum)" : "k_welch_pipe(onepass)");
    } else {
        ProfScope ps(mc.stream);
        LAUNCHCHK(launch_welch(mc, xd, cplx, (const float *)win_d, hop, nframes, tb.f, false, xf, partial, rp, true,
                               spartial, &g.last_kernel));
    }
    if (!want_sum) st.dlt = nullptr;
    LaunchCtx ec = lc();
    if (sl) {
        if (!stop_ev) HIPCHK(hipEventRecord(sl->ev_main, mc.stream));
        HIPCHK(hipStreamWaitEvent(sl->epi, sl->ev_main, 0));
        ec = LaunchCtx{sl->epi, g.ncu};
    }
    if (fused_ok) {
        unsigned *ticket = get_ticket(S_ticket);
        if (!ticket) return fail("ticket allocation failed");
        if (fo->prev.st && fo->prev_wait) HIPCHK(hipStreamWaitEvent(ec.stream, fo->prev_wait, 0));
        LAUNCHCHK(launch_op_fused(ec, xd, cplx, tb.f, (const float *)win_d, partial, spartial, rp.groups, nfft, hop, nframes, nmean,
                                  st, ticket, lobe, nullptr, fo->sided, fo->scale, fo->out, fo->export_state, fo->prev,
                                  sl != nullptr, cola_c));
        fo->done = true;
        fo->prev_done = fo->prev.st != nullptr;
        g_pend.valid = false;
        return 0;
    }
    LAUNCHCHK(launch_op_reduce(ec, xd, cplx, tb.f, partial, spartial, rp.groups, xf, hop, nframes, nmean, st,
                               want_sum ? sum_d : nullptr));
    g_pend.state = nullptr;
    g_pend.valid = true;
    g_pend.xd = xd;
    g_pend.cplx = cplx;
    g_pend.nsig = nsig;
    g_pend.nframes = nframes;
    g_pend.nmean = nmean;
    g_pend.nfft = nfft;
    g_pend.hop = hop;
    g_pend.xf = xf;
    g_pend.win_d = (const float *)win_d;
    g_pend.Wf = (const cf *)Wf_d;
    g_pend.st = st;
    g_pend.trend_f = tb.f;
    g_pend.cw = cw;
    g_pend.sum_d = sum_d;
    return 0;
}

int welch_finish_locked(const double *mean_d , int64_t frames_total, int sided, double scale,
                        double *out_d, const LaunchCtx *ctx = nullptr) {
    if (!g_pend.valid) return fail("sp_welch_finish: no pending sp_welch_accum");
    g_pend.valid = false;
    if (g_pend.state) {
        LAUNCHCHK(launch_op_apply(ctx ? *ctx : lc(), g_pend.state, g_pend.Wf, g_pend.nfft, sided, scale / (double)frames_total, out_d,
                                  mean_d));
        return 0;
    }
    LAUNCHCHK(launch_op_finish(ctx ? *ctx : lc(), g_pend.xd, g_pend.cplx, g_pend.trend_f, g_pend.win_d, g_pend.st, mean_d, g_pend.nmean,
                               g_pend.xf, g_pend.hop, g_pend.nframes, g_pend.cw, g_pend.Wf, sided,
                               scale / (double)frames_total, out_d));
    return 0;
}

struct Rccl {
    void *dl = nullptr;
    ncclResult_t (*GetUniqueId)(ncclUniqueId *) = nullptr;
    ncclResult_t (*CommInitRank)(ncclComm_t *, int, ncclUniqueId, int) = nullptr;
    ncclResult_t (*CommInitRankConfig)(ncclComm_t *, int, ncclUniqueId, int, void *) = nullptr;
    ncclResult_t (*CommDestroy)(ncclComm_t) = nullptr;
    ncclResult_t (*AllReduce)(const void *, void *, size_t, ncclDataType_t, ncclRedOp_t, ncclComm_t, hipStream_t) = nullptr;
    const char *(*GetErrorString)(ncclResult_t) = nullptr;
} rccl;

int rccl_load() {
    if (rccl.dl) return 0;
    const char *names[] = {"librccl.so.1", "/opt/rocm/lib/librccl.so.1", "librccl.so"};
    void *h = nullptr;
    for (const char *nm : names)
        if ((h = dlopen(nm, RTLD_NOW | RTLD_LOCAL))) break;
    if (!h) return fail("RCCL not found (librccl.so.1): %s", dlerror());
    *(void **)&rccl.GetUniqueId = dlsym(h, "ncclGetUniqueId");
    *(void **)&rccl.CommInitRank = dlsym(h, "ncclCommInitRank");
    *(void **)&rccl.CommInitRankConfig = dlsym(h, "ncclCommInitRankConfig");
    *(void **)&rccl.CommDestroy = dlsym(h, "ncclCommDestroy");
    *(void **)&rccl.AllReduce = dlsym(h, "ncclAllReduce");
    *(void **)&rccl.GetErrorString = dlsym(h, "ncclGetErrorString");
    if (!rccl.GetUniqueId || !rccl.CommInitRank || !rccl.CommDestroy || !rccl.AllReduce || !rccl.GetErrorString)
        return fail("librccl lacks an expected symbol");
    rccl.dl = h;
    return 0;
}
#define NCCLCHK(expr)                                                                                 \
    do {                                                                                              \
        ncclResult_t r_ = (expr);                                                                     \
        if (r_ != ncclSuccess) return fail("%s failed: %s (%s:%d)", #expr, rccl.GetErrorString(r_), __FILE__, __LINE__); \
    } while (0)

struct Comm {
    ncclComm_t comm = nullptr;
    int world = 0, rank = -1;
    int ctas = 0;
} gcomm;

static int dist_rccl_ctas() {
    const int v = env_int("SP_DIST_RCCL_CTAS", 4);
    return v < 0 ? 0 : (v > 64 ? 64 : v);
}
static int dist_reserved_cus() {
    if (getenv("SP_DIST_RESERVE_CUS")) {
        const int v = env_int("SP_DIST_RESERVE_CUS", 0);
        return v < 0 ? 0 : (v > g.ncu / 2 ? g.ncu / 2 : v);
    }
    const int want = 2 * gcomm.ctas > 8 ? 2 * gcomm.ctas : 8;
    return (gcomm.comm && gcomm.world > 1) ? (want + 7) / 8 * 8 : 0;
}

struct EngineSlot {
    bool busy = false;
    std::vector<float> win;
    int64_t frames_total = 0;
    int sided = 0;
    double scale = 0;
    double *out = nullptr;
};
struct Engine {
    hipStream_t epi = nullptr;
    hipEvent_t ev_main[2] = {nullptr, nullptr}, ev_epi[2] = {nullptr, nullptr};
    Scratch work[2], onepass[2], trend[2], ticket[2], st[2];
    EngineSlot slot[2];
    int64_t nsub = 0;
    bool with_comm = false;
} geng;

int engine_init() {
    if (geng.epi) return 0;
    HIPCHK(hipStreamCreateWithFlags(&geng.epi, hipStreamNonBlocking));
    for (int i = 0; i < 2; ++i) {
        HIPCHK(hipEventCreateWithFlags(&geng.ev_main[i], hipEventDisableTiming));
        HIPCHK(hipEventCreateWithFlags(&geng.ev_epi[i], hipEventDisableTiming));
    }
    return 0;
}
void engine_release() {
    if (!geng.epi) return;
    (void)hipStreamSynchronize(geng.epi);
    for (int i = 0; i < 2; ++i) {
        (void)hipEventDestroy(geng.ev_main[i]);
        (void)hipEventDestroy(geng.ev_epi[i]);
        geng.ev_main[i] = geng.ev_epi[i] = nullptr;
        geng.work[i].release();
        geng.onepass[i].release();
        geng.trend[i].release();
        geng.ticket[i].release();
        geng.st[i].release();
        geng.slot[i].busy = false;
    }
    (void)hipStreamDestroy(geng.epi);
    geng.epi = nullptr;
    geng.nsub = 0;
}

int engine_apply_locked(int s) {
    EngineSlot &sl = geng.slot[s];
    const int nfft = (int)sl.win.size();
    Xf xf;
    if (get_xf(nfft, &xf)) return -1;
    void *Wf_d;
    if (get_window_spectrum(sl.win.data(), nfft, xf, &Wf_d)) return -1;
    LAUNCHCHK(launch_op_apply(LaunchCtx{geng.epi, g.ncu}, (const double *)geng.st[s].p, (const cf *)Wf_d, nfft, sl.sided,
                              sl.scale / (double)sl.frames_total, sl.out));
    return 0;
}

bool welch_generic_shape(int nfft, int hop) {
    if (!wg_capable(nfft)) return false;
    Xf xf;
    if (get_xf(nfft, &xf)) return false;
    return !welch_carry_eligible(xf, hop, false);
}

int welch_export_locked(const void *xd, bool cplx, int64_t nsig, const float *win, int nfft, int hop, int64_t nframes,
                        int64_t nmean, double *st_d, const OpPrev *prev = nullptr, hipEvent_t prev_wait = nullptr,
                        bool *prev_done = nullptr, const SplitLaunch *sl = nullptr) {
    FusedOut fo{true, SP_SIDED_RAW, 1.0, st_d, false};
    if (prev) {
        fo.prev = *prev;
        fo.prev_wait = prev_wait;
    }
    if (welch_accum_locked(xd, cplx, nsig, win, nfft, hop, nframes, nmean, false, &fo, sl)) return -1;
    g_pend.valid = false;
    if (prev_done) *prev_done = fo.prev_done;
    if (fo.done) return 0;
    LAUNCHCHK(launch_op_finish(sl ? LaunchCtx{sl->epi, g.ncu} : lc(), g_pend.xd, g_pend.cplx, g_pend.trend_f, g_pend.win_d, g_pend.st, nullptr, g_pend.nmean,
                               g_pend.xf, g_pend.hop, g_pend.nframes, g_pend.cw, g_pend.Wf, SP_SIDED_RAW, 1.0, st_d, true));
    return 0;
}

}

extern "C" {

int sp_version(void) { return SP_VERSION; }
int sp_max_wg_fft(void) { return SP_MAX_WG_FFT; }
const char *sp_last_error(void) { return g_err.c_str(); }

int sp_init(int device_id) {
    std::lock_guard<std::mutex> lk(g.mu);
    if (g.ready && (device_id < 0 || device_id == g.device)) return 0;
    if (g.ready)
        return fail("libspectral is bound to device %d for the life of the process (asked for %d)", g.device, device_id);
    int count = 0;
    if (hipGetDeviceCount(&count) != hipSuccess || count <= 0)
        return fail("no HIP device visible (libspectral has no CPU fallback)");
    if (device_id < 0) {
        if (hipGetDevice(&device_id) != hipSuccess) device_id = 0;
    }
    if (device_id >= count) return fail("device %d out of range (%d visible)", device_id, count);
    HIPCHK(hipSetDevice(device_id));
    hipDeviceProp_t prop;
    HIPCHK(hipGetDeviceProperties(&prop, device_id));
    if (strncmp(prop.gcnArchName, "gfx950", 6) != 0)
        return fail("device %d is %s; libspectral is built for gfx950 only", device_id, prop.gcnArchName);
    g.device = device_id;
    g.ncu = prop.multiProcessorCount > 0 ? prop.multiProcessorCount : 256;
    g.ready = true;
    return 0;
}

void sp_shutdown(void) {
    (void)sp_comm_destroy();
    std::lock_guard<std::mutex> lk(g.mu);
    if (!g.ready) return;
    engine_release();
    (void)hipDeviceSynchronize();
    for (auto &kv : g.twiddles) (void)hipFree(kv.second);
    g.twiddles.clear();
    for (auto &kv : g.blue) {
        (void)hipFree(kv.second.chirp);
        (void)hipFree(kv.second.bf);
    }
    g.blue.clear();
    g.in0.release();
    g.in1.release();
    g.out0.release();
    g.work.release();
    g.small.release();
    g.trends.release();
    g.onepass.release();
    g.ticket.release();
    g.epi.release();
    g.pend_trend.release();
    g.cmS.release();
    g.cmT.release();
    g.cmG.release();
    g.cmH.release();
    g.cmO.release();
    g.bigA.release();
    g.bigB.release();
    g.bigT.release();
    g.blueA.release();
    g.blueB.release();
    g.longrec.release();
    for (auto &kv : g.bigtw) {
        (void)hipFree((void *)kv.second.hi);
        (void)hipFree((void *)kv.second.lo);
    }
    g.bigtw.clear();
    for (auto &kv : g.blue_big) {
        (void)hipFree(kv.second.chirp);
        (void)hipFree(kv.second.bf);
    }
    g.blue_big.clear();
    g_pend.valid = false;
    tables_release();
    g.ready = false;
}

int sp_set_stream(void *hip_stream) {
    if (ensure_init()) return -1;
    ApiLock lk;
    hipStream_t ns = (hipStream_t)hip_stream;
    if (ns != g.stream) {
        if (!g.ev_sw && hipEventCreateWithFlags(&g.ev_sw, hipEventDisableTiming) != hipSuccess) g.ev_sw = nullptr;
        if (g.ev_sw) {
            if (hipEventRecord(g.ev_sw, g.stream) == hipSuccess) (void)hipStreamWaitEvent(ns, g.ev_sw, 0);
            (void)hipGetLastError();
        }
        g.stream = ns;
    }
    return 0;
}

int sp_synchronize(void) {
    if (ensure_init()) return -1;
    HIPCHK(hipStreamSynchronize(g.stream));
    return 0;
}

int sp_profile_enable(int on) {
    if (ensure_init()) return -1;
    if (on && !g.ev0) {
        HIPCHK(hipEventCreate(&g.ev0));
        HIPCHK(hipEventCreate(&g.ev1));
    }
    g.profile = on != 0;
    g.prof_valid = false;
    return 0;
}

int sp_profile_last_ms(double *ms) {
    if (ensure_init()) return -1;
    if (!g.profile || !g.prof_valid) return fail("sp_profile_last_ms: no profiled launch recorded");
    HIPCHK(hipEventSynchronize(g.ev1));
    float t = 0.f;
    HIPCHK(hipEventElapsedTime(&t, g.ev0, g.ev1));
    *ms = (double)t;
    return 0;
}

const char *sp_profile_last_kernel(void) { return g.last_kernel; }

int sp_device_info(int64_t out[4]) {
    if (ensure_init()) return -1;
    hipDeviceProp_t prop;
    HIPCHK(hipGetDeviceProperties(&prop, g.device));
    out[0] = prop.multiProcessorCount;
    out[1] = (int64_t)prop.maxSharedMemoryPerMultiProcessor;
    out[2] = prop.clockRate;
    out[3] = prop.warpSize;
    return 0;
}

int sp_mean(const void *x, int x_dtype, int64_t n, double out[2], int mem) {
    if (ensure_init()) return -1;
    if (n <= 0) return fail("sp_mean: n must be positive");
    ApiLock lk;
    const size_t esz = x_dtype == SP_DTYPE_C64 ? 8 : 4;
    const void *xd = x;
    if (!mem) {
        if (g.in0.ensure(esz * (size_t)n)) return -1;
        HIPCHK(hipMemcpyAsync(g.in0.p, x, esz * (size_t)n, hipMemcpyHostToDevice, g.stream));
        xd = g.in0.p;
    }
    TrendBuf tb;
    if (get_trendbuf(1, &tb)) return -1;
    if (set_trend(tb, 0, xd, x_dtype == SP_DTYPE_C64, n, 1, 0, 0)) return -1;
    double h[2];
    HIPCHK(hipMemcpyAsync(h, tb.d, sizeof h, hipMemcpyDeviceToHost, g.stream));
    HIPCHK(hipStreamSynchronize(g.stream));
    out[0] = h[0];
    out[1] = h[1];
    return 0;
}

int sp_fft_c2c(const void *in, void *out, int64_t n, int64_t batch, int direction, int mem) {
    if (ensure_init()) return -1;
    if (n < 1 || batch < 0) return fail("sp_fft_c2c: bad n/batch");
    if (direction != -1 && direction != 1) return fail("sp_fft_c2c: direction must be -1 or +1");
    if (batch == 0) return 0;
    ApiLock lk;
    const size_t bytes = sizeof(cf) * (size_t)n * (size_t)batch;
    const cf *din = (const cf *)in;
    cf *dout = (cf *)out;
    if (!mem) {
        if (g.in0.ensure(bytes)) return -1;
        HIPCHK(hipMemcpyAsync(g.in0.p, in, bytes, hipMemcpyHostToDevice, g.stream));
        din = (const cf *)g.in0.p;
        dout = (cf *)g.in0.p;
    }
    if (dev_fft_any(din, dout, n, batch, direction > 0)) return -1;
    if (!mem) {
        HIPCHK(hipMemcpyAsync(out, dout, bytes, hipMemcpyDeviceToHost, g.stream));
        HIPCHK(hipStreamSynchronize(g.stream));
    }
    return 0;
}

int sp_welch_psd(const void *x, int x_dtype, int64_t nsig, const float *win, int nfft, int hop, int64_t nframes,
                 int detrend, double mean_re, double mean_im, int sided, double scale, double *pxx_out, int mem) {
    if (ensure_init()) return -1;
    if (check_frames("sp_welch_psd", nsig, nfft, hop, nframes)) return -1;
    if (sided < 1 || sided > 3) return fail("sp_welch_psd: bad sided");
    if (detrend < 0 || detrend > 4) return fail("sp_welch_psd: detrend must be 0..4");
    const int segmean = detrend == SP_DETREND_SEGMEAN ? 1 : (detrend == SP_DETREND_SEGLINEAR ? 2 : 0);
    if (segmean) {
        detrend = SP_DETREND_CONST;
        mean_re = mean_im = 0.0;
    }
    ApiLock lk;
    const bool lng = !wg_capable(nfft);
    Xf xf;
    if (!lng && get_xf(nfft, &xf)) return -1;
    const bool cplx = x_dtype == SP_DTYPE_C64;
    const size_t esz = cplx ? 8 : 4;
    const void *xd = x;
    if (!mem) {
        if (g.in0.ensure(esz * (size_t)nsig)) return -1;
        HIPCHK(hipMemcpyAsync(g.in0.p, x, esz * (size_t)nsig, hipMemcpyHostToDevice, g.stream));
        xd = g.in0.p;
    }
    const int nb = nbins_host(nfft, sided);
    double *out_d = pxx_out;
    if (!mem) {
        if (g.out0.ensure(sizeof(double) * (size_t)nb)) return -1;
        out_d = (double *)g.out0.p;
    }
    const bool allow_carry = !env_flag("SP_WELCH_GENERIC");
    if (lng) {
        void *win_d;
        if (get_table(1, win, sizeof(float) * (size_t)nfft, &win_d, nullptr)) return -1;
        TrendBuf tb;
        if (get_trendbuf(1, &tb)) return -1;
        if (set_trend(tb, 0, xd, cplx, nsig, detrend, mean_re, mean_im)) return -1;
        const int64_t mc = long_chunk_frames(nfft, nframes);
        if (g.bigA.ensure(sizeof(cf) * (size_t)mc * (size_t)nfft) || g.work.ensure(sizeof(double) * (size_t)nfft)) return -1;
        cf *S = (cf *)g.bigA.p;
        double *acc = (double *)g.work.p;
        HIPCHK(hipMemsetAsync(acc, 0, sizeof(double) * (size_t)nfft, g.stream));
        for (int64_t f0 = 0; f0 < nframes; f0 += mc) {
            const int64_t m = nframes - f0 < mc ? nframes - f0 : mc;
            if (long_spectra(xd, cplx, (const float *)win_d, nfft, hop, f0, m, tb.f, detrend == 2, segmean, S, nullptr)) return -1;
            LAUNCHCHK(launch_long_acc_psd(lc(), S, m, nfft, acc));
        }
        LAUNCHCHK(launch_long_finish(lc(), acc, nfft, sided, scale / (double)nframes, false, out_d));
        g.last_kernel = "k_long_acc_psd";
    } else if (detrend == SP_DETREND_MEAN && allow_carry && !segmean && !env_flag("SP_WELCH_TWOPASS") &&
               welch_carry_eligible(xf, hop, false) &&
               (cplx || (2 * hop == nfft && nframes >= 2 && !env_flag("SP_NO_REALPAIR") &&
                         welch_pipe_wanted(xf, hop, (nframes + 1) / 2)))) {
        FusedOut fo{false, sided, scale / (double)nframes, out_d, false};
        if (welch_accum_locked(xd, cplx, nsig, win, nfft, hop, nframes, nsig, false, &fo)) return -1;
        if (!fo.done && welch_finish_locked(nullptr, nframes, sided, scale, out_d)) return -1;
    } else {
        void *win_d;
        if (get_table(1, win, sizeof(float) * (size_t)nfft, &win_d, nullptr)) return -1;
        TrendBuf tb;
        if (get_trendbuf(1, &tb)) return -1;
        if (set_trend(tb, 0, xd, cplx, nsig, detrend, mean_re, mean_im)) return -1;
        const bool pair = !cplx && nframes >= 2 && !segmean && !env_flag("SP_NO_REALPAIR");
        const bool pipe = !pair && !segmean && detrend != 2 && allow_carry && welch_pipe_wanted(xf, hop, nframes);
        const bool pipe_rp = pair && detrend != 2 && allow_carry && 2 * hop == nfft && welch_pipe_wanted(xf, hop, (nframes + 1) / 2);
        const RunPart rp = pipe_rp ? run_partition(xf.L, (nframes + 1) / 2, g.ncu, 1)
                                   : (pipe ? run_partition(xf.L, nframes, g.ncu, 1)
                                           : (pair ? run_partition(xf.L, (nframes + 1) / 2, g.ncu,
                                                                   welch_rp_groups_per_cu(xf, detrend == 2))
                                                   : run_partition(xf.L, nframes, g.ncu)));
        if (g.work.ensure(sizeof(float) * (size_t)rp.groups * xf.L)) return -1;
        float *partial = (float *)g.work.p;
        {
            ProfScope ps;
            if (pipe_rp) {
                LAUNCHCHK(launch_welch_pipe(lc(), xd, false, (const float *)win_d, hop, nframes, tb.f, xf, partial, rp, nullptr, 3));
                g.last_kernel = "k_welch_pipe(realpair)";
            } else if (pair) {
                LAUNCHCHK(launch_welch_rp(lc(), (const float *)xd, (const float *)win_d, hop, nframes, tb.f, detrend == 2, xf,
                                          partial, rp));
                g.last_kernel = "k_welch_rp";
            } else if (pipe) {
                LAUNCHCHK(launch_welch_pipe(lc(), xd, cplx, (const float *)win_d, hop, nframes, tb.f, xf, partial, rp, nullptr));
                g.last_kernel = "k_welch_pipe";
            } else {
                LAUNCHCHK(launch_welch(lc(), xd, cplx, (const float *)win_d, hop, nframes, tb.f, detrend == 2, xf, partial,
                                       rp, allow_carry, nullptr, &g.last_kernel, segmean));
            }
        }
        LAUNCHCHK(launch_welch_finish(lc(), partial, rp.groups, xf, sided, scale / (double)nframes, out_d, pair ? 1 : 0));
    }
    if (!mem) {
        HIPCHK(hipMemcpyAsync(pxx_out, out_d, sizeof(double) * (size_t)nb, hipMemcpyDeviceToHost, g.stream));
        HIPCHK(hipStreamSynchronize(g.stream));
    }
    return 0;
}

int sp_welch_accum(const void *x, int x_dtype, int64_t nsig, const float *win, int nfft, int hop, int64_t nframes,
                   int64_t nmean, double *sum_out, int mem) {
    if (ensure_init()) return -1;
    if (check_frames("sp_welch_accum", nsig, nfft, hop, nframes)) return -1;
    ApiLock lk;
    const bool cplx = x_dtype == SP_DTYPE_C64;
    const size_t esz = cplx ? 8 : 4;
    const void *xd = x;
    if (!mem) {
        if (g.in0.ensure(esz * (size_t)nsig)) return -1;
        HIPCHK(hipMemcpyAsync(g.in0.p, x, esz * (size_t)nsig, hipMemcpyHostToDevice, g.stream));
        xd = g.in0.p;
    }
    if (welch_accum_locked(xd, cplx, nsig, win, nfft, hop, nframes, nmean, true)) return -1;
    if (sum_out) {
        if (mem) HIPCHK(hipMemcpyAsync(sum_out, g_pend.sum_d, sizeof(double) * 2, hipMemcpyDeviceToDevice, g.stream));
        else {
            HIPCHK(hipMemcpyAsync(sum_out, g_pend.sum_d, sizeof(double) * 2, hipMemcpyDeviceToHost, g.stream));
            HIPCHK(hipStreamSynchronize(g.stream));
        }
    }
    return 0;
}

int sp_welch_finish(const double *mean, int64_t frames_total, int sided, double scale, double *pxx_out, int mem) {
    if (ensure_init()) return -1;
    if (sided < 1 || sided > 3) return fail("sp_welch_finish: bad sided");
    if (frames_total < 1) return fail("sp_welch_finish: frames_total must be positive");
    ApiLock lk;
    if (!g_pend.valid) return fail("sp_welch_finish: no pending sp_welch_accum");
    const int nb = nbins_host(g_pend.nfft, sided);
    double *out_d = pxx_out;
    const double *mean_d = mean;
    if (!mem) {
        if (g.out0.ensure(sizeof(double) * (size_t)nb + 64)) return -1;
        out_d = (double *)g.out0.p;
        if (mean) {
            double *md = out_d + nb + 2;
            HIPCHK(hipMemcpyAsync(md, mean, sizeof(double) * 2, hipMemcpyHostToDevice, g.stream));
            mean_d = md;
        }
    }
    if (welch_finish_locked(mean_d, frames_total, sided, scale, out_d)) return -1;
    if (!mem) {
        HIPCHK(hipMemcpyAsync(pxx_out, out_d, sizeof(double) * (size_t)nb, hipMemcpyDeviceToHost, g.stream));
        HIPCHK(hipStreamSynchronize(g.stream));
    }
    return 0;
}

int sp_welch_export(const void *x, int x_dtype, int64_t nsig, const float *win, int nfft, int hop, int64_t nframes,
                    int64_t nmean, double *state, int mem) {
    if (ensure_init()) return -1;
    if (check_frames("sp_welch_export", nsig, nfft, hop, nframes)) return -1;
    ApiLock lk;
    const bool cplx = x_dtype == SP_DTYPE_C64;
    const size_t esz = cplx ? 8 : 4;
    const void *xd = x;
    if (!mem) {
        if (g.in0.ensure(esz * (size_t)nsig)) return -1;
        HIPCHK(hipMemcpyAsync(g.in0.p, x, esz * (size_t)nsig, hipMemcpyHostToDevice, g.stream));
        xd = g.in0.p;
    }
    const size_t nst = 5 * (size_t)nfft + 8;
    double *st_d = state;
    if (!mem) {
        if (g.out0.ensure(sizeof(double) * nst)) return -1;
        st_d = (double *)g.out0.p;
    }
    if (welch_export_locked(xd, cplx, nsig, win, nfft, hop, nframes, nmean, st_d)) return -1;
    if (!mem) {
        HIPCHK(hipMemcpyAsync(state, st_d, sizeof(double) * nst, hipMemcpyDeviceToHost, g.stream));
        HIPCHK(hipStreamSynchronize(g.stream));
    }
    return 0;
}

int sp_welch_apply(const double *state, const float *win, int nfft, int64_t frames_total, int sided, double scale,
                   double *pxx_out, int mem) {
    if (ensure_init()) return -1;
    if (sided < 1 || sided > 3) return fail("sp_welch_apply: bad sided");
    if (frames_total < 1) return fail("sp_welch_apply: frames_total must be positive");
    ApiLock lk;
    if (!wg_capable(nfft))
        return fail("sp_welch_apply: segments longer than one workgroup transform are not sharded (nfft = %d, at most %d)", nfft,
                    SP_MAX_WG_FFT);
    Xf xf;
    if (get_xf(nfft, &xf)) return -1;
    void *Wf_d;
    if (get_window_spectrum(win, nfft, xf, &Wf_d)) return -1;
    const int nb = nbins_host(nfft, sided);
    const size_t nst = 5 * (size_t)nfft + 8;
    const double *st_d = state;
    double *out_d = pxx_out;
    if (!mem) {
        if (g.out0.ensure(sizeof(double) * (nst + (size_t)nb) + 64)) return -1;
        double *sd = (double *)g.out0.p;
        HIPCHK(hipMemcpyAsync(sd, state, sizeof(double) * nst, hipMemcpyHostToDevice, g.stream));
        st_d = sd;
        out_d = sd + nst;
    }
    LAUNCHCHK(launch_op_apply(lc(), st_d, (const cf *)Wf_d, nfft, sided, scale / (double)frames_total, out_d));
    if (!mem) {
        HIPCHK(hipMemcpyAsync(pxx_out, out_d, sizeof(double) * (size_t)nb, hipMemcpyDeviceToHost, g.stream));
        HIPCHK(hipStreamSynchronize(g.stream));
    }
    return 0;
}

int sp_comm_unique_id(void *id_out) {
    if (!id_out) return fail("sp_comm_unique_id: null pointer");
    std::lock_guard<std::mutex> lk(g.mu);
    if (rccl_load()) return -1;
    static_assert(sizeof(ncclUniqueId) == SP_COMM_ID_BYTES, "ncclUniqueId size");
    ncclUniqueId id;
    NCCLCHK(rccl.GetUniqueId(&id));
    memcpy(id_out, &id, sizeof id);
    return 0;
}

int sp_comm_init(const void *id_in, int world, int rank) {
    if (ensure_init()) return -1;
    if (!id_in || world < 1 || rank < 0 || rank >= world) return fail("sp_comm_init: bad id/world/rank");
    ApiLock lk;
    if (gcomm.comm) return fail("sp_comm_init: a communicator exists already (sp_comm_destroy first)");
    if (geng.nsub) return fail("sp_comm_init: streaming steps are in flight (sp_welch_dist_flush first)");
    if (rccl_load()) return -1;
    HIPCHK(hipSetDevice(g.device));
    ncclUniqueId id;
    memcpy(&id, id_in, sizeof id);
    struct ConfigV217 {
        size_t size;
        unsigned magic, version;
        int blocking, cgaClusterSize, minCTAs, maxCTAs;
        const char *netName;
    };
    const int ctas = dist_rccl_ctas();
    gcomm.ctas = 0;
    if (rccl.CommInitRankConfig && ctas > 0) {
        ConfigV217 cfg{sizeof(ConfigV217), 0xcafebeefu, 21700u, INT_MIN, INT_MIN, 1, ctas, nullptr};
        NCCLCHK(rccl.CommInitRankConfig(&gcomm.comm, world, id, rank, &cfg));
        gcomm.ctas = ctas;
    } else {
        NCCLCHK(rccl.CommInitRank(&gcomm.comm, world, id, rank));
    }
    gcomm.world = world;
    gcomm.rank = rank;
    return 0;
}
// ... 252 lines not shown
            LAUNCHCHK(launch_csd_pair_finish(lc(), partial, rpp.groups, xf, nch, sided, scale / (double)nframes, pyy_d, pxy_d));
        }
        if (g.bigT.ensure(sizeof(float) * (size_t)rpx.groups * xf.L)) return -1;
        float *px = (float *)g.bigT.p;
        LAUNCHCHK(launch_welch_rp(lc(), (const float *)xd, (const float *)win_d, hop, nframes, tb.f, detrend == 2, xf, px, rpx));
        LAUNCHCHK(launch_welch_finish(lc(), px, rpx.groups, xf, sided, scale / (double)nframes, pxx_d, 1));
    } else if (!cplx && !segmean && csd_rp_eligible(xf) && !env_flag("SP_NO_REALPAIR")) {
        LAUNCHCHK(launch_csd_rp(lc(), (const float *)xd, (const float *)yd, nch, y_ld, (const float *)win_d, hop, nframes,
                                tb.f, tb.f + 4, detrend == 2, xf, partial, rp));
        LAUNCHCHK(launch_csd_rp_finish(lc(), partial, rp.groups, xf, nch, sided, scale / (double)nframes, pxx_d, pyy_d,
                                       pxy_d));
    } else {
        LAUNCHCHK(launch_csd(lc(), xd, yd, cplx, nch, y_ld, (const float *)win_d, hop, nframes, tb.f, tb.f + 4,
                             detrend == 2, xf, partial, rp, segmean));
        LAUNCHCHK(launch_csd_finish(lc(), partial, rp.groups, xf, nch, sided, scale / (double)nframes, pxx_d, pyy_d,
                                    pxy_d));
    }
    if (!mem) {
        HIPCHK(hipMemcpyAsync(pxx, pxx_d, sizeof(double) * nb, hipMemcpyDeviceToHost, g.stream));
        HIPCHK(hipMemcpyAsync(pyy, pyy_d, sizeof(double) * nb * nch, hipMemcpyDeviceToHost, g.stream));
        HIPCHK(hipMemcpyAsync(pxy, pxy_d, sizeof(double) * nb * nch * 2, hipMemcpyDeviceToHost, g.stream));
        HIPCHK(hipStreamSynchronize(g.stream));
    }
    return 0;
}

__global__ void k_set_trends(const double *__restrict__ means, float *__restrict__ trend, int nch) {
    const int c = blockIdx.x * blockDim.x + threadIdx.x;
    if (c < nch) {
        trend[4 * c + 0] = (float)means[c];
        trend[4 * c + 1] = 0.f;
        trend[4 * c + 2] = 0.f;
        trend[4 * c + 3] = 0.f;
    }
}

static int csd_matrix_impl(const char *who, const float *x, int nch, int64_t nsig, int64_t x_ld, const float *win, int nfft,
                           int hop, int64_t nframes, int detrend, const double *means_host, double scale, double *g_out,
                           int mem) {
    if (ensure_init()) return -1;
    if (check_frames(who, nsig, nfft, hop, nframes)) return -1;
    if (nch < 1 || x_ld < nsig) return fail("%s: bad nch / x_ld", who);
    if (detrend < 0 || detrend > 2) return fail("%s: detrend must be 0, 1 or 2", who);
    ApiLock lk;
    const bool lng = !wg_capable(nfft);
    Xf xf;
    xf.L = 0;
    xf.blue = true;
    if (!lng && get_xf(nfft, &xf)) return -1;
    const int nb = nfft / 2 + 1;
    const float *xd = x;
    if (!mem) {
        const size_t ib = sizeof(float) * (size_t)x_ld * (size_t)nch;
        if (g.in0.ensure(ib)) return -1;
        HIPCHK(hipMemcpyAsync(g.in0.p, x, ib, hipMemcpyHostToDevice, g.stream));
        xd = (const float *)g.in0.p;
    }
    void *win_d;
    if (get_table(1, win, sizeof(float) * (size_t)nfft, &win_d, nullptr)) return -1;
    TrendBuf tb;
    if (get_trendbuf(2 * nch, &tb)) return -1;
    const size_t gbytes = sizeof(double) * 2 * (size_t)nb * (size_t)nch * (size_t)nch;
    double *G = g_out;
    if (!mem) {
        if (g.cmG.ensure(gbytes)) return -1;
        G = (double *)g.cmG.p;
    }
    bool g_zeroed = false;
    int64_t mc = ((int64_t)1 << 31) / ((int64_t)nch * nb);
    if (mc > 16384) mc = 16384;
    if (mc < 32) mc = 32;
    mc &= ~(int64_t)31;
    {
        const int64_t nchunks = (nframes + mc - 1) / mc;
        mc = (nframes + nchunks - 1) / nchunks;
        mc = (mc + 31) & ~(int64_t)31;
    }
    if (lng) {
        const int64_t lm = long_chunk_frames(nfft, nframes);
        if (mc > lm) mc = lm;
    }
    if (mc > nframes) mc = nframes;
    const bool use_fused = nch <= 64 && !env_flag("SP_CSDM_TRANSPOSED");
    const int nchp = (nch + 63) / 64 * 64;
    const int64_t mcp = (mc + 31) / 32 * 32;
    const bool rp_stft = !lng && !xf.blue && xf.L >= 32 && nch <= 65535;
    const bool use_bf16 = use_fused && rp_stft && !env_flag("SP_CSDM_FP32");
    const int split2 = env_flag("SP_CSDM_SPLIT3") ? 0 : ((nframes + 1) / 2 >= 1024 ? 1 : 0);
    const int ld = use_bf16 ? (nb + 7) / 8 * 8 : ((use_fused && (rp_stft || lng)) ? (nb + 15) / 16 * 16 : nb);
    const size_t sbytes = use_bf16 ? sizeof(cf) * 2 * (size_t)64 * (size_t)((mc + 1) / 2) * (size_t)ld
                                   : sizeof(cf) * (size_t)nch * (size_t)mc * (size_t)ld;
    const size_t tbytes = sizeof(cf) * (size_t)nchp * (size_t)mcp * (use_fused ? 16 : (size_t)nb);
    if (g.cmS.ensure(sbytes) || g.cmT.ensure(tbytes)) return -1;
    cf *Xs = (cf *)g.cmS.p, *Xt = (cf *)g.cmT.p;
    auto pipe_spec = [&](int64_t m) {
        const int64_t minp = 32;
        return use_bf16 && nfft == 4096 && 2 * hop == nfft && detrend != 2 && (m + 1) / 2 >= minp * (int64_t)((g.ncu + nch - 1) / nch) &&
               welch_pipe_wanted(xf, hop, (int64_t)1 << 40) && !env_flag("SP_CSDM_NOPIPESPEC");
    };
    const bool cm_onepass = detrend == 1 && !means_host && nframes <= mc && pipe_spec(nframes) && !env_flag("SP_CSDM_TWOPASS");
    if (cm_onepass) {
        HIPCHK(hipMemsetAsync(tb.f, 0, sizeof(float) * 4 * (size_t)nch, g.stream));
    } else if (means_host) {
        double *md = tb.d;
        HIPCHK(hipMemcpyAsync(md, means_host, sizeof(double) * (size_t)nch, hipMemcpyHostToDevice, g.stream));
        hipLaunchKernelGGL(k_set_trends, dim3((nch + 63) / 64), dim3(64), 0, g.stream, md, tb.f, nch);
    } else if (detrend == 0) {
        HIPCHK(hipMemsetAsync(tb.f, 0, sizeof(float) * 4 * (size_t)nch, g.stream));
    } else if (nch <= 512) {
        double *scr = moments_scratch();
        if (!scr) return -1;
        LAUNCHCHK(launch_moments(lc(), xd, false, nsig, detrend, scr, tb.d, tb.f, nch, x_ld));
    } else {
        for (int c = 0; c < nch; ++c)
            if (set_trend(tb, c, xd + (size_t)x_ld * (size_t)c, false, nsig, detrend, 0, 0)) return -1;
    }
    size_t op_sp = 0, op_sl = 0;
    int op_runs = 0;
    bool fold_pending = false;
    for (int64_t f0 = 0; f0 < nframes; f0 += mc) {
        const int64_t m = nframes - f0 < mc ? nframes - f0 : mc;
        hipLaunchKernelGGL(k_trend_shift, dim3((nch + 63) / 64), dim3(64), 0, g.stream, tb.f, tb.f + 4 * nch, nch,
                           (double)f0 * (double)hop);
        if (lng) {
            if (g.bigA.ensure(sizeof(cf) * (size_t)m * (size_t)nfft)) return -1;
            cf *S = (cf *)g.bigA.p;
            for (int c = 0; c < nch; ++c) {
                if (long_spectra(xd + (size_t)x_ld * (size_t)c, false, (const float *)win_d, nfft, hop, f0, m, tb.f + 4 * c,
                                 detrend == 2, 0, S, nullptr))
                    return -1;
                LAUNCHCHK(launch_long_stft_out(lc(), S, m, nfft, SP_SIDED_HALF, 1.f, 0, Xs + (size_t)c * (size_t)m * (size_t)ld, 0, ld));
            }
        } else if (pipe_spec(m)) {
            const int64_t pairs = (m + 1) / 2;
            const int runs = (g.ncu + nch - 1) / nch > 0 ? (g.ncu + nch - 1) / nch : 1;
            RunPart rp;
            rp.fpg = ((pairs + runs - 1) / runs + 1) & ~(int64_t)1;
            rp.blocks = (int)((pairs + rp.fpg - 1) / rp.fpg);
            rp.groups = rp.blocks;
            const size_t zbytes = (size_t)128 * 64 * 512 * (size_t)((pairs + 1) / 2);
            const size_t hbytes = sizeof(double) * 2 * (size_t)nfft * (size_t)nch * (size_t)nch;
            if (g.cmS.ensure(zbytes) || g.cmH.ensure(hbytes)) return -1;
            Xs = (cf *)g.cmS.p;
            const int h_init = fold_pending ? 0 : 1;
            fold_pending = true;
            cf *spartial = nullptr;
            if (cm_onepass) {
                op_sp = sizeof(cf) * (size_t)nch * (size_t)rp.blocks * (size_t)hop;
                op_sl = sizeof(double) * 2 * (size_t)hop * (size_t)nch;
                if (g.cmO.ensure(op_sp + op_sl + sizeof(double) * (size_t)(5 * nfft + 8) * (size_t)nch)) return -1;
                spartial = (cf *)g.cmO.p;
                op_runs = rp.blocks;
            }
            LAUNCHCHK(launch_welch_pipe(lc(), xd + (size_t)f0 * (size_t)hop, false, (const float *)win_d, hop, m, tb.f + 4 * nch, xf,
                                        (float *)Xs, rp, spartial, 5, nch, x_ld, nfft / 8));
            LAUNCHCHK(launch_csdm_bf16(lc(), Xs, Xt, nch, pairs, nfft, (double *)g.cmH.p, nfft, split2, h_init));
            continue;
        } else if (use_bf16) {
            const RunPart rp = run_partition_2d(xf.L, (m + 1) / 2, g.ncu, nch);
            LAUNCHCHK(launch_stft_rp(lc(), xd + (size_t)f0 * (size_t)hop, (const float *)win_d, hop, m, tb.f + 4 * nch,
                                     detrend == 2, xf, rp, SP_SIDED_HALF, 1.f, 2, Xs, nullptr, nch, x_ld,
                                     ((m + 1) / 2) * (int64_t)ld * 2, ld));
        } else if (rp_stft && (m >= 2 || ld != nb)) {
            const RunPart rp = run_partition_2d(xf.L, (m + 1) / 2, g.ncu, nch);
            LAUNCHCHK(launch_stft_rp(lc(), xd + (size_t)f0 * (size_t)hop, (const float *)win_d, hop, m, tb.f + 4 * nch,
                                     detrend == 2, xf, rp, SP_SIDED_HALF, 1.f, 0, Xs, nullptr, nch, x_ld,
                                     (int64_t)m * ld, ld));
        } else {
            const RunPart rp = run_partition(xf.L, m, g.ncu, 2);
            for (int c = 0; c < nch; ++c)
                LAUNCHCHK(launch_stft(lc(), xd + (size_t)x_ld * (size_t)c + (size_t)f0 * (size_t)hop, false,
                                      (const float *)win_d, hop, m, tb.f + 4 * (nch + c), detrend == 2, xf, rp, SP_SIDED_HALF,
                                      1.f, 0, Xs + (size_t)c * (size_t)m * (size_t)nb, nullptr));
        }
        if (!g_zeroed) {
            HIPCHK(hipMemsetAsync(G, 0, gbytes, g.stream));
            g_zeroed = true;
        }
        if (use_bf16) {
            LAUNCHCHK(launch_csdm_bf16(lc(), Xs, Xt, nch, m, nb, G, ld, split2));
        } else if (use_fused) {
            LAUNCHCHK(launch_csdm_fused(lc(), Xs, Xt, nch, m, nb, G, ld));
        } else {
            const int64_t mp = (m + 31) / 32 * 32;
            LAUNCHCHK(launch_csdm_transpose_kgc(lc(), Xs, Xt, nch, nchp, m, mp, nb));
            LAUNCHCHK(launch_csdm_mfma(lc(), Xt, nch, nchp, mp, nb, G));
        }
    }
    const double gscale = scale / (double)nframes;
    const int fold_init = (fold_pending && !g_zeroed) ? 1 : 0;
    if (cm_onepass) {
        void *Wf_d;
        if (get_window_spectrum(win, nfft, xf, &Wf_d)) return -1;
        double *Sl = (double *)((char *)g.cmO.p + op_sp), *st = (double *)((char *)g.cmO.p + op_sp + op_sl);
        LAUNCHCHK(launch_cm_blocksums(lc(), (const cf *)g.cmO.p, nch, op_runs, hop, Sl));
        LAUNCHCHK(launch_op_finish_channels(lc(), xd, x_ld, nch, tb.f + 4 * nch, (const float *)win_d, Sl, (const cf *)Wf_d, hop,
                                            nframes, nsig, xf, st));
        LAUNCHCHK(launch_csdm_fold(lc(), (const double *)g.cmH.p, G, nch, nfft, st, (const cf *)Wf_d, tb.f + 4 * nch, nsig, nframes,
                                   gscale, fold_init));
    } else if (fold_pending) {
        LAUNCHCHK(launch_csdm_fold(lc(), (const double *)g.cmH.p, G, nch, nfft, nullptr, nullptr, nullptr, 0, 0, gscale, fold_init));
    }
    if (!fold_init) LAUNCHCHK(launch_csdm_finish(lc(), G, nch, nb, gscale));
    if (!mem) {
        HIPCHK(hipMemcpyAsync(g_out, G, gbytes, hipMemcpyDeviceToHost, g.stream));
        HIPCHK(hipStreamSynchronize(g.stream));
    }
    return 0;
}

int sp_csd_matrix(const float *x, int nch, int64_t nsig, int64_t x_ld, const float *win, int nfft, int hop,
                  int64_t nframes, int detrend, double scale, double *g_out, int mem) {
    return csd_matrix_impl("sp_csd_matrix", x, nch, nsig, x_ld, win, nfft, hop, nframes, detrend, nullptr, scale, g_out, mem);
}

int sp_csd_matrix_means(const float *x, int nch, int64_t nsig, int64_t x_ld, const float *win, int nfft, int hop,
                        int64_t nframes, const double *means, double scale, double *g_out, int mem) {
    if (!means) return fail("sp_csd_matrix_means: means is NULL");
    return csd_matrix_impl("sp_csd_matrix_means", x, nch, nsig, x_ld, win, nfft, hop, nframes, 0, means, scale, g_out, mem);
}

int sp_channel_means(const float *x, int nch, int64_t nsig, int64_t x_ld, double *means_out, int mem) {
    if (ensure_init()) return -1;
    if (nch < 1 || nch > 512 || nsig < 1 || x_ld < nsig) return fail("sp_channel_means: need 1 <= nch <= 512, 1 <= nsig <= x_ld");
    ApiLock lk;
    const float *xd = x;
    if (!mem) {
        const size_t ib = sizeof(float) * (size_t)x_ld * (size_t)nch;
        if (g.in0.ensure(ib)) return -1;
        HIPCHK(hipMemcpyAsync(g.in0.p, x, ib, hipMemcpyHostToDevice, g.stream));
        xd = (const float *)g.in0.p;
    }
    TrendBuf tb;
    if (get_trendbuf(nch, &tb)) return -1;
    double *scr = moments_scratch();
    if (!scr) return -1;
    LAUNCHCHK(launch_moments(lc(), xd, false, nsig, 1, scr, tb.d, tb.f, nch, x_ld));
    HIPCHK(hipMemcpy2DAsync(means_out, sizeof(double), tb.d, sizeof(double) * 8, sizeof(double), (size_t)nch,
                            mem ? hipMemcpyDeviceToDevice : hipMemcpyDeviceToHost, g.stream));
    if (!mem) HIPCHK(hipStreamSynchronize(g.stream));
    return 0;
}

int sp_stft(const void *x, int x_dtype, int64_t nsig, const float *win, int nfft, int hop, int64_t nframes,
            int detrend, double mean_re, double mean_im, int sided, double amp_scale, int out_kind, int out_major,
            void *out, double *pseg_out, int mem) {
    if (ensure_init()) return -1;
    if (check_frames("sp_stft", nsig, nfft, hop, nframes)) return -1;
    if (sided < 1 || sided > 4) return fail("sp_stft: bad sided");
    if (detrend < 0 || detrend > 4) return fail("sp_stft: detrend must be 0..4");
    const int segmean = detrend == SP_DETREND_SEGMEAN ? 1 : (detrend == SP_DETREND_SEGLINEAR ? 2 : 0);
    if (segmean) {
        detrend = SP_DETREND_CONST;
        mean_re = mean_im = 0.0;
    }
    ApiLock lk;
    const bool lng = !wg_capable(nfft);
    Xf xf;
    if (!lng && get_xf(nfft, &xf)) return -1;
    const bool cplx = x_dtype == SP_DTYPE_C64;
    const size_t esz = cplx ? 8 : 4;
    const size_t osz = out_kind ? 4 : 8;
    const size_t nb = (size_t)nbins_host(nfft, sided);
    const size_t obytes = osz * nb * (size_t)nframes;
    const void *xd = x;
    if (!mem) {
        if (g.in0.ensure(esz * (size_t)nsig)) return -1;
        HIPCHK(hipMemcpyAsync(g.in0.p, x, esz * (size_t)nsig, hipMemcpyHostToDevice, g.stream));
        xd = g.in0.p;
    }
    void *win_d;
    if (get_table(1, win, sizeof(float) * (size_t)nfft, &win_d, nullptr)) return -1;
    TrendBuf tb;
    if (get_trendbuf(1, &tb)) return -1;
    if (set_trend(tb, 0, xd, cplx, nsig, detrend, mean_re, mean_im)) return -1;
    void *fin = out;
    double *pseg_d = pseg_out;
    if (!mem) {
        if (g.out0.ensure(obytes + (pseg_out ? sizeof(double) * (size_t)nframes + 16 : 0))) return -1;
        fin = g.out0.p;
        if (pseg_out) pseg_d = (double *)((char *)g.out0.p + ((obytes + 15) & ~(size_t)15));
    }
    void *fm = fin;
    if (out_major == 1) {
        if (g.work.ensure(obytes)) return -1;
        fm = g.work.p;
    }
    if (pseg_d) HIPCHK(hipMemsetAsync(pseg_d, 0, sizeof(double) * (size_t)nframes, g.stream));
    const bool pair = !lng && !cplx && !segmean && !xf.blue && xf.L >= 32 && nframes >= 2 && !env_flag("SP_NO_REALPAIR");
    if (lng) {
        const int64_t mc = long_chunk_frames(nfft, nframes);
        if (g.bigA.ensure(sizeof(cf) * (size_t)mc * (size_t)nfft)) return -1;
        cf *S = (cf *)g.bigA.p;
        for (int64_t f0 = 0; f0 < nframes; f0 += mc) {
            const int64_t m = nframes - f0 < mc ? nframes - f0 : mc;
            if (long_spectra(xd, cplx, (const float *)win_d, nfft, hop, f0, m, tb.f, detrend == 2, segmean, S, pseg_d)) return -1;
            LAUNCHCHK(launch_long_stft_out(lc(), S, m, nfft, sided, (float)amp_scale, out_kind, fm, f0, (int)nb));
        }
    } else if (pair) {
        const RunPart rp = run_partition(xf.L, (nframes + 1) / 2, g.ncu,
                                         stft_rp_groups_per_cu(xf, detrend == 2, hop, sided, out_kind, pseg_d != nullptr));
        LAUNCHCHK(launch_stft_rp(lc(), (const float *)xd, (const float *)win_d, hop, nframes, tb.f, detrend == 2, xf, rp, sided,
                                 (float)amp_scale, out_kind, fm, pseg_d));
    } else {
        const RunPart rp = run_partition(xf.L, nframes, g.ncu);
        LAUNCHCHK(launch_stft(lc(), xd, cplx, (const float *)win_d, hop, nframes, tb.f, detrend == 2, xf, rp, sided,
                              (float)amp_scale, out_kind, fm, pseg_d, segmean));
    }
    if (out_major == 1) LAUNCHCHK(launch_transpose(lc(), fm, fin, nframes, (int64_t)nb, (int)osz));
    if (!mem) {
        HIPCHK(hipMemcpyAsync(out, fin, obytes, hipMemcpyDeviceToHost, g.stream));
        if (pseg_out)
            HIPCHK(hipMemcpyAsync(pseg_out, pseg_d, sizeof(double) * (size_t)nframes, hipMemcpyDeviceToHost, g.stream));
        HIPCHK(hipStreamSynchronize(g.stream));
    }
    return 0;
}

int sp_stft_cog(const void *x, int x_dtype, int64_t nsig, const float *win, int nfft, int hop, int64_t nframes,
                int detrend, double mean_re, double mean_im, double fs, double fmin, double fmax, double *cog_out, int mem) {
    if (ensure_init()) return -1;
    if (check_frames("sp_stft_cog", nsig, nfft, hop, nframes)) return -1;
    if (detrend < 0 || detrend > 4) return fail("sp_stft_cog: detrend must be 0..4");
    if (!(fs > 0.0) || fmin < 0.0 || fmax < fmin) return fail("sp_stft_cog: need fs > 0 and 0 <= fmin <= fmax");
    const int segmean = detrend == SP_DETREND_SEGMEAN ? 1 : (detrend == SP_DETREND_SEGLINEAR ? 2 : 0);
    if (segmean) {
        detrend = SP_DETREND_CONST;
        mean_re = mean_im = 0.0;
    }
    ApiLock lk;
    const bool lng = !wg_capable(nfft);
    Xf xf;
    if (!lng && get_xf(nfft, &xf)) return -1;
    const bool cplx = x_dtype == SP_DTYPE_C64;
    const size_t esz = cplx ? 8 : 4;
    const void *xd = x;
    if (!mem) {
        if (g.in0.ensure(esz * (size_t)nsig)) return -1;
        HIPCHK(hipMemcpyAsync(g.in0.p, x, esz * (size_t)nsig, hipMemcpyHostToDevice, g.stream));
        xd = g.in0.p;
    }
    void *win_d;
    if (get_table(1, win, sizeof(float) * (size_t)nfft, &win_d, nullptr)) return -1;
    TrendBuf tb;
    if (get_trendbuf(1, &tb)) return -1;
    const double df = fs / (double)nfft;
    const double eps = 1e-9;
    const int klo = (int)std::ceil(fmin / df - eps);
    const double kh = std::floor(fmax / df + eps);
    const int khi = kh > (double)nfft ? nfft : (int)kh;
    const int wpf = lng ? 1 : (xf.L / 16 >= 64 ? xf.L / 16 / 64 : 1);
    const bool cog_pipe = !lng && !segmean && detrend != 2 && klo <= 0 && khi >= nfft / 2 && !env_flag("SP_COG_GENERIC") &&
                          welch_pipe_wanted(xf, hop, nframes);
    CogLobe lobe_w{};
    const bool cog_op = cog_pipe && detrend == SP_DETREND_MEAN && xf.L == 4096 && (hop == 2048 || hop == 1024) &&
                        !env_flag("SP_COG_TWOPASS") && cog_window_lobe(win, nfft, &lobe_w);
    if (cog_op) {
        HIPCHK(hipMemsetAsync(tb.f, 0, sizeof(float) * 4, g.stream));
    } else if (set_trend(tb, 0, xd, cplx, nsig, detrend, mean_re, mean_im)) {
        return -1;
    }
    const size_t abytes = sizeof(cf) * (size_t)wpf * (size_t)nframes + (cog_op ? sizeof(cf) * 8 * (size_t)nframes : 0);
    if (g.work.ensure(abytes)) return -1;
    cf *acc = (cf *)g.work.p;
    double *fin = cog_out;
    if (!mem) {
        if (g.out0.ensure(sizeof(double) * (size_t)nframes)) return -1;
        fin = (double *)g.out0.p;
    }
    if (lng) {
        const int64_t mc = long_chunk_frames(nfft, nframes);
        if (g.bigA.ensure(sizeof(cf) * (size_t)mc * (size_t)nfft)) return -1;
        cf *S = (cf *)g.bigA.p;
        for (int64_t f0 = 0; f0 < nframes; f0 += mc) {
            const int64_t m = nframes - f0 < mc ? nframes - f0 : mc;
            if (long_spectra(xd, cplx, (const float *)win_d, nfft, hop, f0, m, tb.f, detrend == 2, segmean, S, nullptr)) return -1;
            LAUNCHCHK(launch_long_cog(lc(), S, m, nfft, klo, khi, acc, f0));
        }
    } else {
        const bool pipe = cog_pipe;
        const RunPart rp = pipe ? run_partition(xf.L, nframes, g.ncu, 1) : run_partition(xf.L, nframes, g.ncu);
        int generic = 1;
        if (cog_op) {
            const size_t b_sp = sizeof(cf) * (size_t)rp.groups * (size_t)hop, b_sl = sizeof(double) * (size_t)(2 * hop > nfft ? 2 * hop : nfft);
            if (g.cmO.ensure(b_sp + b_sl + sizeof(double) * (size_t)(5 * nfft + 8))) return -1;
            cf *spartial = (cf *)g.cmO.p;
            double *Sl = (double *)((char *)g.cmO.p + b_sp), *st = (double *)((char *)g.cmO.p + b_sp + b_sl);
            void *Wf_d;
            if (get_window_spectrum(win, nfft, xf, &Wf_d)) return -1;
            LAUNCHCHK(launch_welch_pipe(lc(), xd, cplx, (const float *)win_d, hop, nframes, tb.f, xf, (float *)acc, rp, spartial, 2));
            LAUNCHCHK(launch_cm_blocksums(lc(), spartial, 1, (int)rp.groups, hop, Sl));
            LAUNCHCHK(launch_op_finish_channels(lc(), xd, 0, 1, tb.f, (const float *)win_d, Sl, (const cf *)Wf_d, hop, nframes, nsig, xf,
                                                st, cplx));
            LAUNCHCHK(launch_cog_finish_op(lc(), acc, wpf, nframes, df, fin, acc + (size_t)wpf * (size_t)nframes, lobe_w, st, tb.f, nsig,
                                           nfft));
            if (!mem) {
                HIPCHK(hipMemcpyAsync(cog_out, fin, sizeof(double) * (size_t)nframes, hipMemcpyDeviceToHost, g.stream));
                HIPCHK(hipStreamSynchronize(g.stream));
            }
            return 0;
        }
        if (pipe) {
            LAUNCHCHK(launch_welch_pipe(lc(), xd, cplx, (const float *)win_d, hop, nframes, tb.f, xf, (float *)acc, rp, nullptr, 2));
            generic = 0;
        } else if (!segmean && detrend != 2 && !env_flag("SP_COG_GENERIC"))
            generic = launch_cog_carry(lc(), xd, cplx, (const float *)win_d, hop, nframes, tb.f, xf, acc, rp, klo, khi);
        if (generic < 0) return fail("sp_stft_cog: launch failed");
        if (generic)
            LAUNCHCHK(launch_stft(lc(), xd, cplx, (const float *)win_d, hop, nframes, tb.f, detrend == 2, xf, rp, 2, 1.f, 1, nullptr,
                                  nullptr, segmean, acc, klo, khi));
    }
    LAUNCHCHK(launch_cog_finish(lc(), acc, wpf, nframes, df, fin));
    if (!mem) {
        HIPCHK(hipMemcpyAsync(cog_out, fin, sizeof(double) * (size_t)nframes, hipMemcpyDeviceToHost, g.stream));
        HIPCHK(hipStreamSynchronize(g.stream));
    }
    return 0;
}

int sp_bispectrum(const void *x, const void *y, const void *z, int x_dtype, int64_t nsig, const float *win, int nfft, int hop,
                  int64_t nframes, int detrend, double mean_re, double mean_im, void *B_out, double *b2_out, double *pzz_out,
                  int mem) {
    if (ensure_init()) return -1;
    if (nfft < 8 || nfft > 4096 || !wg_capable(nfft)) return fail("sp_bispectrum: nfft %d outside 8 .. 4096", nfft);
    if (check_frames("sp_bispectrum", nsig, nfft, hop, nframes)) return -1;
    if (x_dtype != SP_DTYPE_F32 && x_dtype != SP_DTYPE_C64) return fail("sp_bispectrum: unknown dtype %d", x_dtype);
    if (detrend < SP_DETREND_CONST || detrend > SP_DETREND_LINEAR) return fail("sp_bispectrum: detrend must be 0, 1 or 2");
    if (!x || !B_out || !b2_out) return fail("sp_bispectrum: x, B_out and b2_out are required");
    ApiLock lk;
    Xf xf;
    if (get_xf(nfft, &xf)) return -1;
    const bool cplx = x_dtype == SP_DTYPE_C64;
    const bool sym = y == nullptr && z == nullptr;
    const int nsp = sym ? 1 : 3;
    const int nb = cplx ? nfft : nfft / 2 + 1, c0 = cplx ? nfft / 2 : 0;
    const int sided = cplx ? SP_SIDED_TWO : SP_SIDED_HALF;
    const size_t esz = cplx ? 8 : 4;
    const void *src[3] = {x, y ? y : x, z ? z : x};
    const void *xd[3] = {x, src[1], src[2]};
    if (!mem) {
        if (g.bsIn.ensure(esz * (size_t)nsig * (size_t)nsp)) return -1;
        for (int k = 0; k < nsp; ++k) {
            xd[k] = (char *)g.bsIn.p + esz * (size_t)nsig * (size_t)k;
            HIPCHK(hipMemcpyAsync((void *)xd[k], src[k], esz * (size_t)nsig, hipMemcpyHostToDevice, g.stream));
        }
    }
    if (sym) xd[1] = xd[2] = xd[0];
    const int T = bispec_tile_dim(), ntd = (nb + T - 1) / T;
    std::vector<int> tbl((size_t)ntd * ntd, -1);
    std::vector<int> tl;
    for (int ti = 0; ti < ntd; ++ti)
        for (int tj = 0; tj < (sym ? ti + 1 : ntd); ++tj) {
            const int imax = std::min(ti * T + T, nb) - 1, jmax = std::min(tj * T + T, nb) - 1;
            if (ti * T + tj * T - c0 > nb - 1 || imax + jmax - c0 < 0) continue;
            tbl[(size_t)ti * ntd + tj] = (int)tl.size() / 2;
            tl.push_back(ti);
            tl.push_back(tj);
        }
    const int ntiles = (int)tl.size() / 2;
    const size_t nmap = tbl.size() + (tbl.size() & 1);
    tbl.resize(nmap, -1);
    tbl.insert(tbl.end(), tl.begin(), tl.end());
    void *tab_d;
    if (get_table(6, tbl.data(), sizeof(int) * tbl.size(), &tab_d, nullptr)) return -1;
    const int *tmap_d = (const int *)tab_d;
    const int2 *tiles_d = (const int2 *)((const int *)tab_d + nmap);
    const int64_t FC = bispec_frame_chunk();
    const size_t budget = (size_t)std::max(1, env_int("SP_BISPEC_MIB", 256)) << 20;
    const size_t part_bytes = sizeof(float) * bispec_part_floats() * (size_t)ntiles;
    const size_t spec_bytes = sizeof(cf) * (size_t)nb * (size_t)nsp * (size_t)FC;
    int64_t cpc = (int64_t)std::min(budget / spec_bytes, budget / part_bytes);
    cpc = std::max<int64_t>(1, std::min<int64_t>(cpc, 4096));
    const int64_t mc = std::min(nframes, cpc * FC);
    const int64_t nfc = (mc + FC - 1) / FC;
    if (g.bsS.ensure(sizeof(cf) * (size_t)nb * (size_t)nsp * (size_t)mc) || g.bsP.ensure(part_bytes * (size_t)nfc) ||
        g.bsA.ensure(sizeof(double) * (bispec_part_floats() * (size_t)ntiles + (size_t)nb * (size_t)(nfc + 1))))
        return -1;
    cf *S[3];
    for (int k = 0; k < 3; ++k) S[k] = (cf *)g.bsS.p + (size_t)nb * (size_t)mc * (size_t)(sym ? 0 : k);
    float *part = (float *)g.bsP.p;
    double *acc = (double *)g.bsA.p, *p64 = acc + bispec_part_floats() * (size_t)ntiles, *ppart = p64 + nb;
    void *win_d;
    if (get_table(1, win, sizeof(float) * (size_t)nfft, &win_d, nullptr)) return -1;
    TrendBuf tb;
    if (get_trendbuf(6, &tb)) return -1;
    for (int k = 0; k < nsp; ++k)
        if (set_trend(tb, k, xd[k], cplx, nsig, detrend, mean_re, mean_im)) return -1;
    for (int64_t f0 = 0; f0 < nframes; f0 += mc) {
        const int64_t m = std::min(mc, nframes - f0);
        LAUNCHCHK(launch_bispec_trend_shift(lc(), tb.f, tb.f + 12, nsp, f0 * (int64_t)hop));
        const RunPart rp = run_partition(xf.L, m, g.ncu);
        for (int k = 0; k < nsp; ++k)
            LAUNCHCHK(launch_stft(lc(), (const char *)xd[k] + esz * (size_t)(f0 * hop), cplx, (const float *)win_d, hop, m,
                                  tb.f + 12 + 4 * k, detrend == SP_DETREND_LINEAR, xf, rp, sided, 1.f, 0, S[k], nullptr));
        {
            ProfScope ps;
            LAUNCHCHK(launch_bispec_tile(lc(), S[0], S[1], S[2], nb, c0, m, tiles_d, ntiles, part));
        }
        LAUNCHCHK(launch_bispec_pzz(lc(), S[2], nb, m, ppart));
        LAUNCHCHK(launch_bispec_reduce(lc(), part, ppart, ntiles, m, nb, f0 == 0, acc, p64));
    }
    void *Bd = B_out;
    double *b2d = b2_out, *pzd = pzz_out;
    const size_t nn = (size_t)nb * (size_t)nb;
    if (!mem) {
        if (g.out0.ensure(sizeof(double) * (3 * nn + (size_t)nb))) return -1;
        Bd = g.out0.p;
        b2d = (double *)g.out0.p + 2 * nn;
        pzd = pzz_out ? b2d + nn : nullptr;
    }
    LAUNCHCHK(launch_bispec_finish(lc(), acc, p64, tmap_d, ntd, nb, c0, sym ? 1 : 0, nframes, Bd, b2d, pzd));
    if (!mem) {
        HIPCHK(hipMemcpyAsync(B_out, Bd, 2 * sizeof(double) * nn, hipMemcpyDeviceToHost, g.stream));
        HIPCHK(hipMemcpyAsync(b2_out, b2d, sizeof(double) * nn, hipMemcpyDeviceToHost, g.stream));
        if (pzz_out) HIPCHK(hipMemcpyAsync(pzz_out, pzd, sizeof(double) * (size_t)nb, hipMemcpyDeviceToHost, g.stream));
        HIPCHK(hipStreamSynchronize(g.stream));
    }
    return 0;
}

static int64_t istft_head_len(int n, int hop, int64_t M) {
    return M * (int64_t)hop >= (int64_t)(n - hop) ? (int64_t)(n - hop) : (M - 1) * (int64_t)hop + n;
}
static void istft_envelope(const float *win, int n, int hop, int64_t M, std::vector<float> *out) {
    const int64_t H = istft_head_len(n, hop, M);
    const bool whole = H != (int64_t)(n - hop);
    std::vector<double> per((size_t)hop, 0.0), head((size_t)H, 0.0), tail(whole ? 0 : (size_t)(n - hop), 0.0);
    for (int j = 0; j < n; ++j) per[(size_t)(j % hop)] += (double)win[j] * (double)win[j];
    if (whole) {
        for (int64_t g = 0; g < M; ++g)
            for (int j = 0; j < n; ++j) head[(size_t)(g * hop + j)] += (double)win[j] * (double)win[j];
    } else {
        for (int a = 0; a < n - hop; ++a) head[(size_t)a] = (double)win[a] * (double)win[a] + (a >= hop ? head[(size_t)(a - hop)] : 0.0);
        for (int i = n - hop - 1; i >= 0; --i)
            tail[(size_t)i] = (double)win[i + hop] * (double)win[i + hop] + (i + hop < n - hop ? tail[(size_t)(i + hop)] : 0.0);
    }
    out->clear();
    out->reserve(per.size() + head.size() + tail.size());
    for (const std::vector<double> *v : {&per, &head, &tail})
        for (double e : *v) out->push_back(e > 1e-10 ? (float)(1.0 / e) : 1.f);
}

int sp_istft(const void *Z, int sided, int in_major, int nch, int64_t nframes, const float *win, int nfft, int hop, double scale,
             int64_t skip, int64_t nout, void *y, int mem) {
    if (!Z || !win || !y) return fail("sp_istft: Z, win and y are required");
    if (sided != SP_SIDED_HALF && sided != SP_SIDED_RAW) return fail("sp_istft: sided must be SP_SIDED_HALF or SP_SIDED_RAW");
    if (in_major != 0 && in_major != 1) return fail("sp_istft: in_major must be 0 or 1");
    if (nfft < 2 || hop < 1 || hop > nfft) return fail("sp_istft: need nfft >= 2 and 1 <= hop <= nfft (nfft %d, hop %d)", nfft, hop);
    if (nframes < 1 || nch < 1) return fail("sp_istft: nframes and nch must be at least 1");
    if (!wg_capable(nfft))
        return fail("sp_istft: nfft %d not supported (powers of two up to %d, other lengths up to %d)", nfft, SP_MAX_WG_FFT,
                    SP_MAX_WG_FFT / 2);
    if (nframes > ((int64_t)1 << 40) / hop) return fail("sp_istft: too many frames");
    const int64_t M = nframes, Lout = (M - 1) * (int64_t)hop + nfft;
    if (skip < 0 || nout < 1 || skip > Lout || nout > Lout - skip)
        return fail("sp_istft: skip %lld + nout %lld outside the %lld overlap-added samples", (long long)skip, (long long)nout,
// ... 563 lines not shown
```

Baseline: 487,900.

## Replace block-wide barriers in welch pipe with LDS counter hand-off between producer/consumer waves

Removes the per-frame __syncthreads between the fill role and the FFT roles in k_welch_pipe, replacing them with per-wave LDS counters (filled/drained events) that waits spin on with a bounded sleep loop. The image-reuse wait is injected mid-butterfly via a new Half callback so compute overlaps the wait. It also adds fences around wave barriers, a device status word recording spin overruns, and host-side checks that fail the call if an overrun happened. The cost targeted is whole-workgroup barrier stalls between pipeline stages; the risk is spin overhead, extra host checks, and an invalid result if a bound is exceeded.

```diff
diff --git a/include/spectral.h b/include/spectral.h
--- a/include/spectral.h
+++ b/include/spectral.h
@@ -25,6 +25,7 @@
 int sp_profile_enable(int on);
 int sp_profile_last_ms(double *ms);
 const char *sp_profile_last_kernel(void);
+int sp_pipe_status(void);
 int sp_device_info(int64_t out[4]);
 
 int sp_fft_c2c(const void *in, void *out, int64_t n, int64_t batch, int direction, int mem);
diff --git a/pyfft_amd/_ffi.py b/pyfft_amd/_ffi.py
--- a/pyfft_amd/_ffi.py
+++ b/pyfft_amd/_ffi.py
@@ -26,6 +26,7 @@
     "sp_profile_enable": (_i, [_i]),
     "sp_profile_last_ms": (_i, [C.POINTER(_d)]),
     "sp_profile_last_kernel": (C.c_char_p, []),
+    "sp_pipe_status": (_i, []),
     "sp_fft_c2c": (_i, [_vp, _vp, _i64, _i64, _i, _i]),
     "sp_welch_psd": (_i, [_vp, _i, _i64, _vp, _i, _i, _i64, _i, _d, _d, _i, _d, _vp, _i]),
     "sp_welch_accum": (_i, [_vp, _i, _i64, _vp, _i, _i, _i64, _i64, _vp, _i]),
diff --git a/pyfft_amd/csrc/fft_core.h b/pyfft_amd/csrc/fft_core.h
--- a/pyfft_amd/csrc/fft_core.h
+++ b/pyfft_amd/csrc/fft_core.h
@@ -96,7 +96,14 @@
 }
 __device__ __forceinline__ cf rot_tan(cf a, float t) { return mk(fmaf(t, a.y, a.x), fmaf(-t, a.x, a.y)); }
 
-template <bool TWD, bool PREROT = false> __device__ __forceinline__ void dft16s(cf (&x)[16], const Tw16 &w) {
+struct NoMid {
+    __device__ __forceinline__ void operator()(int) const {}
+};
+__device__ __forceinline__ void pin16(cf (&x)[16]) {
+#pragma unroll
+    for (int s = 0; s < 16; ++s) asm volatile("" : "+v"(x[s].x), "+v"(x[s].y));
+}
+template <bool TWD, bool PREROT = false, class Half = NoMid> __device__ __forceinline__ void dft16s(cf (&x)[16], const Tw16 &w, Half half = Half()) {
     if constexpr (TWD) {
         if constexpr (!PREROT) {
 #pragma unroll
@@ -107,6 +114,12 @@
     } else {
 #pragma unroll
         for (int b = 0; b < 4; ++b) dft4<false>(x[b], x[b + 4], x[b + 8], x[b + 12]);
+    }
+    if constexpr (!std::is_same<Half, NoMid>::value) {
+        pin16(x);
+        __builtin_amdgcn_sched_barrier(0);
+        half(0);
+        __builtin_amdgcn_sched_barrier(0);
     }
     x[5] = rot_tan(x[5], SP_T16);
     x[9] = mk(x[9].x + x[9].y, x[9].y - x[9].x);
@@ -132,7 +145,7 @@
 #undef SP_SWAP
 }
 
-template <bool TWD, class Store, bool PREROT = false> __device__ __forceinline__ void dft16s_es(cf (&x)[16], const Tw16 &w, Store store) {
+template <bool TWD, class Store, bool PREROT = false, class Half = NoMid> __device__ __forceinline__ void dft16s_es(cf (&x)[16], const Tw16 &w, Store store, Half half = Half()) {
     if constexpr (TWD) {
         if constexpr (!PREROT) {
 #pragma unroll
@@ -154,6 +167,11 @@
     x[11] = mk(x[11].x - x[11].y, x[11].y + x[11].x);
     x[15] = rot_tan(x[15], SP_T16);
     __builtin_amdgcn_sched_barrier(0);
+    if constexpr (!std::is_same<Half, NoMid>::value) {
+        pin16(x);
+        half(0);
+        __builtin_amdgcn_sched_barrier(0);
+    }
 #define SP_ES_OUT(c)                                                                                                 \
     store(c, x[4 * c]);                                                                                              \
     store(c + 4, x[4 * c + 1]);                                                                                      \
@@ -193,10 +211,7 @@
     b = mk(t1.x + t3.y, t1.y - t3.x);
     d = mk(t1.x - t3.y, t1.y + t3.x);
 }
-struct NoMid {
-    __device__ __forceinline__ void operator()(int) const {}
-};
-template <class Store, class Mid = NoMid> __device__ __forceinline__ void dft16s_es_win(cf (&x)[16], const float (&w)[16], Store store, Mid mid = Mid()) {
+template <class Store, class Mid = NoMid, class Half = NoMid> __device__ __forceinline__ void dft16s_es_win(cf (&x)[16], const float (&w)[16], Store store, Mid mid = Mid(), Half half = Half()) {
 #pragma unroll
     for (int b = 0; b < 4; ++b) {
         dft4w(x[b], x[b + 4], x[b + 8], x[b + 12], w[b], w[b + 4], w[b + 8], w[b + 12]);
@@ -218,6 +233,11 @@
     x[11] = mk(x[11].x - x[11].y, x[11].y + x[11].x);
     x[15] = rot_tan(x[15], SP_T16);
     __builtin_amdgcn_sched_barrier(0);
+    if constexpr (!std::is_same<Half, NoMid>::value) {
+        pin16(x);
+        half(0);
+        __builtin_amdgcn_sched_barrier(0);
+    }
 #define SP_ES_OUT(c)                                                                                                 \
     store(c, x[4 * c]);                                                                                              \
     store(c + 4, x[4 * c + 1]);                                                                                      \
@@ -412,16 +432,21 @@
         pass<0, SINGLE, WL>(v, lds0, lds1, tid);
     }
     template <bool WL> static __device__ __forceinline__ void xsync() {
-        if constexpr (WL) __builtin_amdgcn_wave_barrier();
-        else __syncthreads();
-    }
-
-    template <int P> __device__ __forceinline__ void bfly_scatter(cf (&v)[R], cf *lds, int tid) const {
+        if constexpr (WL) {
+            __builtin_amdgcn_fence(__ATOMIC_RELEASE, "wavefront");
+            __builtin_amdgcn_wave_barrier();
+            __builtin_amdgcn_fence(__ATOMIC_ACQUIRE, "wavefront");
+        } else {
+            __syncthreads();
+        }
+    }
+
+    template <int P, class Half = NoMid> __device__ __forceinline__ void bfly_scatter(cf (&v)[R], cf *lds, int tid, Half half = Half()) const {
         constexpr int NS = PL::ns(P);
         const int base = (tid / NS) * (NS * 16) + (tid % NS);
         auto store = [&](int k, cf val) __attribute__((always_inline)) { lds[phys<P>(base + k * NS)] = val; };
-        if constexpr (P > 0) dft16s_es<true>(v, t16[P - 1], store);
-        else dft16s_es<false>(v, t16[0], store);
+        if constexpr (P > 0) dft16s_es<true, decltype(store), false, Half>(v, t16[P - 1], store, half);
+        else dft16s_es<false, decltype(store), false, Half>(v, t16[0], store, half);
     }
 
     template <int P> __device__ __forceinline__ void load_tau_out(const cf *__restrict__ table, int tid, float (&tau)[16]) const {
@@ -438,32 +463,35 @@
             tau[k] = sc == 0 ? 0.f : -w.y / c;
         }
     }
-    template <int P, bool PREROT> __device__ __forceinline__ void bfly_scatter_rot(cf (&v)[R], const float (&tau)[16], cf *lds, int tid) const {
+    template <int P, bool PREROT, class Half = NoMid>
+    __device__ __forceinline__ void bfly_scatter_rot(cf (&v)[R], const float (&tau)[16], cf *lds, int tid, Half half = Half()) const {
         constexpr int NS = PL::ns(P);
         const int base = (tid / NS) * (NS * 16) + (tid % NS);
         auto store = [&](int k, cf val) __attribute__((always_inline)) { lds[phys<P>(base + k * NS)] = rot_tan(val, tau[k]); };
-        if constexpr (P > 0) dft16s_es<true, decltype(store), PREROT>(v, t16[P - 1], store);
-        else dft16s_es<false>(v, t16[0], store);
-    }
-    __device__ __forceinline__ void bfly_scatter_win_rot(cf (&v)[R], const float (&w)[R], const float (&tau)[16], cf *lds, int tid) const {
+        if constexpr (P > 0) dft16s_es<true, decltype(store), PREROT, Half>(v, t16[P - 1], store, half);
+        else dft16s_es<false, decltype(store), false, Half>(v, t16[0], store, half);
+    }
+    template <class Half = NoMid>
+    __device__ __forceinline__ void bfly_scatter_win_rot(cf (&v)[R], const float (&w)[R], const float (&tau)[16], cf *lds, int tid, Half half = Half()) const {
         static_assert(R == 16, "radix-16 first pass");
         constexpr int NS = PL::ns(0);
         const int base = (tid / NS) * (NS * 16) + (tid % NS);
         auto store = [&](int k, cf val) __attribute__((always_inline)) { lds[phys<0>(base + k * NS)] = rot_tan(val, tau[k]); };
-        dft16s_es_win(v, w, store);
-    }
-    template <int P> __device__ __forceinline__ void bfly_prerot(cf (&v)[R], int tid) const {
+        dft16s_es_win(v, w, store, NoMid(), half);
+    }
+    template <int P, class Half = NoMid> __device__ __forceinline__ void bfly_prerot(cf (&v)[R], int tid, Half half = Half()) const {
         (void)tid;
         static_assert(P > 0 && PL::radix(P) == 16 && R == 16, "a twiddled radix-16 pass");
-        dft16s<true, true>(v, t16[P - 1]);
-    }
-
-    __device__ __forceinline__ void bfly_scatter_win(cf (&v)[R], const float (&w)[R], cf *lds, int tid) const {
+        dft16s<true, true, Half>(v, t16[P - 1], half);
+    }
+
+    template <class Half = NoMid>
+    __device__ __forceinline__ void bfly_scatter_win(cf (&v)[R], const float (&w)[R], cf *lds, int tid, Half half = Half()) const {
         static_assert(R == 16, "radix-16 first pass");
         constexpr int NS = PL::ns(0);
         const int base = (tid / NS) * (NS * 16) + (tid % NS);
         auto store = [&](int k, cf val) __attribute__((always_inline)) { lds[phys<0>(base + k * NS)] = val; };
-        dft16s_es_win(v, w, store);
+        dft16s_es_win(v, w, store, NoMid(), half);
     }
 
     template <int P, bool SINGLE, bool WL = false> __device__ __forceinline__ void pass(cf (&v)[R], cf *lds0, cf *lds1, int tid) const {
diff --git a/pyfft_amd/csrc/k_welch_pipe.hip b/pyfft_amd/csrc/k_welch_pipe.hip
--- a/pyfft_amd/csrc/k_welch_pipe.hip
+++ b/pyfft_amd/csrc/k_welch_pipe.hip
@@ -3,10 +3,37 @@
 #define SP_PIPE_AHEAD 2
 namespace sp {
 
+#define SP_PIPE_SPINS (1u << 18)
+struct PipeSync {
+    unsigned *cnt;
+    unsigned overran;
+    __device__ __forceinline__ void wait(int ev, int64_t need) {
+        if (need <= 0 || overran) return;
+        const unsigned *c = cnt + 4 * ev + (threadIdx.x & 3);
+        const unsigned target = (unsigned)need;
+#pragma nounroll
+        for (unsigned n = 0; n < SP_PIPE_SPINS; ++n) {
+            const unsigned v = __hip_atomic_load(c, __ATOMIC_ACQUIRE, __HIP_MEMORY_SCOPE_WORKGROUP);
+            if (__builtin_amdgcn_ballot_w64((int)(v - target) < 0) == 0) return;
+            __builtin_amdgcn_s_sleep(1);
+        }
+        overran = 1u + (unsigned)ev;
+    }
+    __device__ __forceinline__ void report(unsigned *status) const {
+        if (overran && (threadIdx.x & 63) == 0) *reinterpret_cast<volatile unsigned *>(status) = overran;
+    }
+    __device__ __forceinline__ void signal(int ev, int wv, int64_t done) {
+        if ((threadIdx.x & 63) == 0)
+            __hip_atomic_store(cnt + 4 * ev + wv, (unsigned)done, __ATOMIC_RELEASE, __HIP_MEMORY_SCOPE_WORKGROUP);
+    }
+};
+enum { PIPE_A_FILLED = 0, PIPE_A_DRAINED = 1, PIPE_B_FILLED = 2, PIPE_B_DRAINED = 3 };
+
 template <bool CPLX, int SHIFT, int MODE>
 __global__ __launch_bounds__(768) void k_welch_pipe(const void *__restrict__ x_in, const float *__restrict__ win,
                                                      int64_t nframes, int64_t fpg, float *__restrict__ trend_in, XfTables tb,
-                                                     float *__restrict__ partial, cf *__restrict__ spartial, int64_t x_cs, int gpr) {
+                                                     float *__restrict__ partial, cf *__restrict__ spartial, int64_t x_cs, int gpr,
+                                                     unsigned *__restrict__ status) {
     constexpr int N = 4096;
     constexpr bool RP = MODE >= 3 && MODE != 8 && MODE != 9;
     constexpr bool ONEPASS = MODE == 1 || MODE == 4 || MODE == 7 || MODE == 8 || MODE == 9, COG = MODE == 2 || MODE == 8;
@@ -25,6 +52,9 @@
     const int role = __builtin_amdgcn_readfirstlane((int)threadIdx.x >> 8);
     const int tid = (int)threadIdx.x & 255;
     const int hop = SHIFT * T;
+    const int wv = __builtin_amdgcn_readfirstlane(tid >> 6);
+    PipeSync hs{reinterpret_cast<unsigned *>(smem + 2 * IMG + 2 * IMGB), 0u};
+    if (threadIdx.x < 16) hs.cnt[threadIdx.x] = 0u;
 
     cf mu;
     if constexpr (ONEPASS) {
@@ -67,14 +97,14 @@
         }
     } else {
         mu = load_trend(trend).m;
+        __syncthreads();
     }
     const int64_t gid = blockIdx.x;
     const int64_t g0 = gid * fpg;
     const int64_t last = nframes - 1;
     int64_t trips = (RP ? (nframes + 1) / 2 : nframes) - g0;
     trips = trips < 0 ? 0 : (trips > fpg ? fpg : trips);
-    constexpr int DRAIN = 4;
-    const int64_t periods = trips + DRAIN;
+    const int64_t periods = trips + 4;
     F f;
     constexpr bool UPROT = !RP;
     float tau_out[16];
@@ -114,16 +144,17 @@
             issue_chunk(fill, g0 + i + 2);
             __builtin_amdgcn_sched_barrier(0);
             cf v[R];
+            auto free_img = [&](int) __attribute__((always_inline)) { hs.wait(PIPE_A_DRAINED, i - 1); };
             if constexpr (!ONEPASS) {
 #pragma unroll
                 for (int t = 0; t < R; ++t) v[t] = mk(cur[t], HB ? (t < R / 2 ? cur[t + R / 2] : nxt[t - R / 2]) : 0.f);
-                if constexpr (UPROT) f.bfly_scatter_win_rot(v, w, tau_out, img, tid);
-                else f.bfly_scatter_win(v, w, img, tid);
+                if constexpr (UPROT) f.bfly_scatter_win_rot(v, w, tau_out, img, tid, free_img);
+                else f.bfly_scatter_win(v, w, img, tid, free_img);
             } else {
 #pragma unroll
                 for (int t = 0; t < R; ++t) v[t] = mk(w[t] * cur[t], HB ? w[t] * (t < R / 2 ? cur[t + R / 2] : nxt[t - R / 2]) : 0.f);
-                if constexpr (UPROT) f.template bfly_scatter_rot<0, false>(v, tau_out, img, tid);
-                else f.template bfly_scatter<0>(v, img, tid);
+                if constexpr (UPROT) f.template bfly_scatter_rot<0, false>(v, tau_out, img, tid, free_img);
+                else f.template bfly_scatter<0>(v, img, tid, free_img);
             }
             __builtin_amdgcn_sched_barrier(0);
             if constexpr (ONEPASS) {
@@ -132,23 +163,18 @@
             }
 #pragma unroll
             for (int t = 0; t < R; ++t) fill[t] -= m;
+            hs.signal(PIPE_A_FILLED, wv, i + 1);
         };
         const std::true_type yes;
         const std::false_type no;
         int64_t i = 0;
         for (; i + 6 < trips; i += 6) {
             frame(yes, i, imgA, ca, cb, cc);
-            __syncthreads();
             frame(yes, i + 1, imgA + IMG, cb, cc, ca);
-            __syncthreads();
             frame(yes, i + 2, imgA, cc, ca, cb);
-            __syncthreads();
             frame(yes, i + 3, imgA + IMG, ca, cb, cc);
-            __syncthreads();
             frame(yes, i + 4, imgA, cb, cc, ca);
-            __syncthreads();
             frame(yes, i + 5, imgA + IMG, cc, ca, cb);
-            __syncthreads();
         }
         for (; i < trips; ++i) {
             cf *img = (i & 1) ? imgA + IMG : imgA;
@@ -162,10 +188,7 @@
                 else if (i % 3 == 1) frame(no, i, img, cb, cc, ca);
                 else frame(no, i, img, cc, ca, cb);
             }
-            __syncthreads();
-        }
-#pragma unroll
-        for (int d = 0; d < DRAIN; ++d) __syncthreads();
+        }
         if constexpr (ONEPASS) {
 #pragma unroll
             for (int s = 0; s < SHIFT; ++s)
@@ -208,6 +231,7 @@
             __builtin_amdgcn_sched_barrier(0);
             cf v[R];
             constexpr bool WINFOLD = SPREAD;
+            auto free_img = [&](int) __attribute__((always_inline)) { hs.wait(PIPE_A_DRAINED, i - 1); };
 #pragma unroll
             for (int t = 0; t < R; ++t) v[t] = WINFOLD ? raw[t] : w[t] * raw[t];
             if constexpr (SPREAD) {
@@ -216,12 +240,12 @@
                     img[F::template phys<0>(tid * 16 + k)] = UPROT ? rot_tan(val, tau_out[k]) : val;
                     if (k >= 12 && k < 15) issue_part(fill, i + AHEAD, (k - 11) * (SHIFT / 4), (k - 10) * (SHIFT / 4));
                 };
-                if constexpr (WINFOLD) dft16s_es_win(v, w, store);
-                else dft16s_es<false>(v, f.t16[0], store);
+                if constexpr (WINFOLD) dft16s_es_win(v, w, store, NoMid(), free_img);
+                else dft16s_es<false, decltype(store), false, decltype(free_img)>(v, f.t16[0], store, free_img);
             }
             } else {
-            if constexpr (UPROT) f.template bfly_scatter_rot<0, false>(v, tau_out, img, tid);
-            else f.template bfly_scatter<0>(v, img, tid);
+            if constexpr (UPROT) f.template bfly_scatter_rot<0, false>(v, tau_out, img, tid, free_img);
+            else f.template bfly_scatter<0>(v, img, tid, free_img);
             }
             __builtin_amdgcn_sched_barrier(0);
 #pragma unroll
@@ -231,6 +255,7 @@
             for (int t = 0; t < KEEP; ++t) raw[t] = raw[t + SHIFT];
 #pragma unroll
             for (int s = 0; s < SHIFT; ++s) raw[KEEP + s] = take[s] - mu;
+            hs.signal(PIPE_A_FILLED, wv, i + 1);
         };
         int64_t i = 0;
         if constexpr (AHEAD == 3) {
@@ -239,48 +264,34 @@
             issue(s2, 2);
             for (; i + 2 < trips; i += 3) {
                 frame(i, (i & 1) ? imgA + IMG : imgA, s0, s1);
-                __syncthreads();
                 frame(i + 1, ((i + 1) & 1) ? imgA + IMG : imgA, s1, s2);
-                __syncthreads();
                 frame(i + 2, ((i + 2) & 1) ? imgA + IMG : imgA, s2, s0);
-                __syncthreads();
             }
             for (; i < trips; ++i) {
                 cf *img = (i & 1) ? imgA + IMG : imgA;
                 if (i % 3 == 0) frame(i, img, s0, s1);
                 else if (i % 3 == 1) frame(i, img, s1, s2);
                 else frame(i, img, s2, s0);
-                __syncthreads();
             }
         } else if constexpr (AHEAD == 2) {
             cf nxa[SHIFT], nxb[SHIFT];
             issue(nxa, 1);
             for (; i + 1 < trips; i += 2) {
                 frame(i, imgA, nxb, nxa);
-                __syncthreads();
                 frame(i + 1, imgA + IMG, nxa, nxb);
-                __syncthreads();
-            }
-            if (i < trips) {
-                frame(i, imgA, nxb, nxa);
-                __syncthreads();
-            }
+            }
+            if (i < trips) frame(i, imgA, nxb, nxa);
         } else {
             for (; i + 1 < trips; i += 2) {
                 cf nx0[SHIFT], nx1[SHIFT];
                 frame(i, imgA, nx0, nx0);
-                __syncthreads();
                 frame(i + 1, imgA + IMG, nx1, nx1);
-                __syncthreads();
             }
             if (i < trips) {
                 cf nx0[SHIFT];
                 frame(i, imgA, nx0, nx0);
-                __syncthreads();
-            }
-        }
-#pragma unroll
-        for (int d = 0; d < DRAIN; ++d) __syncthreads();
+            }
+        }
 #pragma unroll
         for (int s = 0; s < SHIFT; ++s)
             if constexpr (ONEPASS && !LOBE) spartial[gid * hop + tid + T * s] = sacc[s];
@@ -288,16 +299,26 @@
         f.template load_tw_one<1>(tb.tw, tid);
         cf va[R], vb[R];
         auto step = [&](cf (&fill)[R], cf (&use)[R], int64_t p, const cf *src, cf *dst) __attribute__((always_inline)) {
-            if (p >= 1 && p <= trips) f.template gather<0>(fill, src, tid);
-            if (p >= 2 && p <= trips + 1) {
-                if constexpr (UPROT) f.template bfly_scatter_rot<1, true>(use, tau_out, dst, tid);
-                else f.template bfly_scatter<1>(use, dst, tid);
-            }
-            __syncthreads();
-        };
-        for (int64_t p = 0; p < periods; p += 2) {
-            step(va, vb, p, imgA + IMG, imgB);
-            if (p + 1 < periods) step(vb, va, p + 1, imgA, imgB + IMGB);
+            const bool take = p <= trips;
+            if (take) {
+                hs.wait(PIPE_A_FILLED, p);
+                f.template gather<0>(fill, src, tid);
+            }
+            if (p >= 2) {
+                auto hand = [&](int) __attribute__((always_inline)) {
+                    if (take) hs.signal(PIPE_A_DRAINED, wv, p);
+                    hs.wait(PIPE_B_DRAINED, p - 3);
+                };
+                if constexpr (UPROT) f.template bfly_scatter_rot<1, true>(use, tau_out, dst, tid, hand);
+                else f.template bfly_scatter<1>(use, dst, tid, hand);
+                hs.signal(PIPE_B_FILLED, wv, p - 1);
+            } else if (take) {
+                hs.signal(PIPE_A_DRAINED, wv, p);
+            }
+        };
+        for (int64_t p = 1; p <= trips + 1; p += 2) {
+            step(vb, va, p, imgA, imgB + IMGB);
+            if (p + 1 <= trips + 1) step(va, vb, p + 1, imgA + IMG, imgB);
         }
     } else {
         f.template load_tw_one<2>(tb.tw, tid);
@@ -315,12 +336,22 @@
             if (li <= sel && gg < nframes) reinterpret_cast<cf *>(partial)[(int64_t)(tid >> 6) * nframes + gg] = pend;
         };
         auto step = [&](cf (&fill)[R], cf (&use)[R], int64_t p, const cf *src) __attribute__((always_inline)) {
-            if (p >= 3 && p <= trips + 2) {
+            const bool take = p <= trips + 2;
+            if (take) {
+                hs.wait(PIPE_B_FILLED, p - 2);
                 f.template gather<1>(fill, src, tid);
             }
-            if (p >= 4 && p <= trips + 3) {
-                if constexpr (UPROT) f.template bfly_prerot<2>(use, tid);
-                else f.template bfly<2>(use, tid);
+            if (p < 4 && take) hs.signal(PIPE_B_DRAINED, wv, p - 2);
+            if (p >= 4) {
+                auto hand = [&](int) __attribute__((always_inline)) {
+                    if (take) hs.signal(PIPE_B_DRAINED, wv, p - 2);
+                };
+                if constexpr (UPROT) {
+                    f.template bfly_prerot<2>(use, tid, hand);
+                } else {
+                    f.template bfly<2>(use, tid);
+                    hand(0);
+                }
                 if constexpr (SPEC) {
                     const int64_t pr = g0 + (p - 4);
                     const bool lone = (pr & 1) == 0 && p == trips + 3;
@@ -369,11 +400,10 @@
                     }
                 }
             }
-            __syncthreads();
-        };
-        for (int64_t p = 0; p < periods; p += 2) {
-            step(va, vb, p, imgB + IMGB);
-            if (p + 1 < periods) step(vb, va, p + 1, imgB);
+        };
+        for (int64_t p = 3; p < periods; p += 2) {
+            step(vb, va, p, imgB);
+            if (p + 1 < periods) step(va, vb, p + 1, imgB + IMGB);
         }
         if constexpr (!COG && !SPEC) {
 #pragma unroll
@@ -385,6 +415,25 @@
             }
         }
     }
+    hs.report(status);
+}
+
+static unsigned *pipe_status_word() {
+    static unsigned *w = nullptr;
+    if (!w) {
+        void *p = nullptr;
+        if (hipHostMalloc(&p, 64, hipHostMallocMapped) != hipSuccess) return nullptr;
+        *reinterpret_cast<volatile unsigned *>(p) = 0u;
+        w = reinterpret_cast<unsigned *>(p);
+    }
+    return w;
+}
+unsigned pipe_overrun() {
+    unsigned *w = pipe_status_word();
+    if (!w) return 0u;
+    const unsigned v = *reinterpret_cast<volatile unsigned *>(w);
+    if (v) *reinterpret_cast<volatile unsigned *>(w) = 0u;
+    return v;
 }
 
 bool welch_pipe_eligible(const Xf &xf, int hop) {
@@ -393,7 +442,9 @@
 
 int launch_welch_pipe(LaunchCtx c, const void *x, bool cplx, const float *win, int hop, int64_t nframes, float *trend,
                       const Xf &xf, float *partial, const RunPart &rp, cf *spartial, int mode, int nch, int64_t x_cs, int gpr) {
-    const size_t lds = sizeof(cf) * 4 * (size_t)FftPlan<4096>::LDS_ELEMS;
+    const size_t lds = sizeof(cf) * 4 * (size_t)FftPlan<4096>::LDS_ELEMS + 64;
+    unsigned *status = pipe_status_word();
+    if (!status) return -1;
 #define PIPE_(CP, S, OP)                                                                                  \
     {                                                                                                 \
         static bool once = false;                                                                     \
@@ -404,10 +455,10 @@
         }                                                                                             \
         if (c.stop)                                                                                   \
             hipExtLaunchKernelGGL((k_welch_pipe<CP, S, OP>), dim3(rp.blocks, gy), dim3(768), lds, c.stream, nullptr, c.stop, 0, x, win, \
-                                  nframes, rp.fpg, trend, xf.tb, partial, spartial, x_cs, gpr);       \
+                                  nframes, rp.fpg, trend, xf.tb, partial, spartial, x_cs, gpr, status); \
         else                                                                                          \
             hipLaunchKernelGGL((k_welch_pipe<CP, S, OP>), dim3(rp.blocks, gy), dim3(768), lds, c.stream, x, win, nframes, rp.fpg, trend, \
-                               xf.tb, partial, spartial, x_cs, gpr);                                  \
+                               xf.tb, partial, spartial, x_cs, gpr, status);                          \
     }
     const int shift = hop / 256;
     const unsigned gy = mode == 5 ? (unsigned)nch : 1u;
diff --git a/pyfft_amd/csrc/launch.h b/pyfft_amd/csrc/launch.h
--- a/pyfft_amd/csrc/launch.h
+++ b/pyfft_amd/csrc/launch.h
@@ -116,6 +116,7 @@
 int launch_welch_pipe(LaunchCtx c, const void *x, bool cplx, const float *win, int hop, int64_t nframes, float *trend,
                       const Xf &xf, float *partial, const RunPart &rp, cf *spartial, int mode = 0, int nch = 1, int64_t x_cs = 0,
                       int gpr = 0);
+unsigned pipe_overrun();
 int launch_op_estimate(LaunchCtx c, const void *x, bool cplx, int64_t nsig, double *part, float *trend);
 int launch_op_reduce(LaunchCtx c, const void *x, bool cplx, const float *trend, const float *partial, const cf *spartial,
                      int64_t G, const Xf &xf, int hop, int64_t nframes, int64_t nmean, OnePass st, double *sum_out);
diff --git a/pyfft_amd/csrc/spectral.hip b/pyfft_amd/csrc/spectral.hip
--- a/pyfft_amd/csrc/spectral.hip
+++ b/pyfft_amd/csrc/spectral.hip
@@ -46,6 +46,17 @@
     do {                                                                                              \
         if ((expr) != 0) return fail("%s: no kernel instantiated for this transform length (%s:%d)", #expr, __FILE__, __LINE__); \
         HIPCHK(hipGetLastError());                                                                    \
+    } while (0)
+
+int pipe_check() {
+    const unsigned v = pipe_overrun();
+    if (v) return fail("k_welch_pipe: a hand-off wait overran its bound (event %u): the result of that launch is invalid", v - 1);
+    return 0;
+}
+#define PIPECHK(expr)                                                                                 \
+    do {                                                                                              \
+        if (pipe_check()) return -1;                                                                  \
+        LAUNCHCHK(expr);                                                                              \
     } while (0)
 
 struct Scratch {
@@ -666,10 +677,10 @@
     hipEvent_t prev_wait = nullptr;
     bool prev_done = false;
 };
-unsigned *get_ticket(Scratch &t) {
+unsigned *get_ticket(Scratch &t, hipStream_t stream) {
     if (!t.p) {
         if (t.ensure(1024)) return nullptr;
-        if (hipMemset(t.p, 0, 1024) != hipSuccess) return nullptr;
+        if (hipMemsetAsync(t.p, 0, 1024, stream) != hipSuccess) return nullptr;
     }
     return (unsigned *)t.p;
 }
@@ -807,7 +818,7 @@
         ProfScope ps(mc.stream);
         LaunchCtx mcs = mc;
         if (stop_ev) mcs.stop = sl->ev_main;
-        LAUNCHCHK(launch_welch_pipe(mcs, xd, cplx, (const float *)win_d, hop, nframes, tb.f, xf, partial, rp, spartial,
+        PIPECHK(launch_welch_pipe(mcs, xd, cplx, (const float *)win_d, hop, nframes, tb.f, xf, partial, rp, spartial,
                                     realpair ? 3 : (lobesum ? 9 : 0)));
         g.last_kernel = realpair ? "k_welch_pipe(onepass,realpair)" : (lobesum ? "k_welch_pipe(onepass,lobesum)" : "k_welch_pipe(onepass)");
     } else {
@@ -823,7 +834,7 @@
         ec = LaunchCtx{sl->epi, g.ncu};
     }
     if (fused_ok) {
-        unsigned *ticket = get_ticket(S_ticket);
+        unsigned *ticket = get_ticket(S_ticket, ec.stream);
         if (!ticket) return fail("ticket allocation failed");
         if (fo->prev.st && fo->prev_wait) HIPCHK(hipStreamWaitEvent(ec.stream, fo->prev_wait, 0));
         LAUNCHCHK(launch_op_fused(ec, xd, cplx, tb.f, (const float *)win_d, partial, spartial, rp.groups, nfft, hop, nframes, nmean,
@@ -1127,6 +1138,12 @@
 }
 
 const char *sp_profile_last_kernel(void) { return g.last_kernel; }
+
+int sp_pipe_status(void) {
+    if (ensure_init()) return -1;
+    HIPCHK(hipDeviceSynchronize());
+    return pipe_check();
+}
 
 int sp_device_info(int64_t out[4]) {
     if (ensure_init()) return -1;
@@ -1258,14 +1275,14 @@
         {
             ProfScope ps;
             if (pipe_rp) {
-                LAUNCHCHK(launch_welch_pipe(lc(), xd, false, (const float *)win_d, hop, nframes, tb.f, xf, partial, rp, nullptr, 3));
+                PIPECHK(launch_welch_pipe(lc(), xd, false, (const float *)win_d, hop, nframes, tb.f, xf, partial, rp, nullptr, 3));
                 g.last_kernel = "k_welch_pipe(realpair)";
             } else if (pair) {
                 LAUNCHCHK(launch_welch_rp(lc(), (const float *)xd, (const float *)win_d, hop, nframes, tb.f, detrend == 2, xf,
                                           partial, rp));
                 g.last_kernel = "k_welch_rp";
             } else if (pipe) {
-                LAUNCHCHK(launch_welch_pipe(lc(), xd, cplx, (const float *)win_d, hop, nframes, tb.f, xf, partial, rp, nullptr));
+                PIPECHK(launch_welch_pipe(lc(), xd, cplx, (const float *)win_d, hop, nframes, tb.f, xf, partial, rp, nullptr));
                 g.last_kernel = "k_welch_pipe";
             } else {
                 LAUNCHCHK(launch_welch(lc(), xd, cplx, (const float *)win_d, hop, nframes, tb.f, detrend == 2, xf, partial,
@@ -1277,6 +1294,7 @@
     if (!mem) {
         HIPCHK(hipMemcpyAsync(pxx_out, out_d, sizeof(double) * (size_t)nb, hipMemcpyDeviceToHost, g.stream));
         HIPCHK(hipStreamSynchronize(g.stream));
+        if (pipe_check()) return -1;
     }
     return 0;
 }
@@ -1835,7 +1853,7 @@
                 spartial = (cf *)g.cmO.p;
                 op_runs = rp.blocks;
             }
-            LAUNCHCHK(launch_welch_pipe(lc(), xd + (size_t)f0 * (size_t)hop, false, (const float *)win_d, hop, m, tb.f + 4 * nch, xf,
+            PIPECHK(launch_welch_pipe(lc(), xd + (size_t)f0 * (size_t)hop, false, (const float *)win_d, hop, m, tb.f + 4 * nch, xf,
                                         (float *)Xs, rp, spartial, 5, nch, x_ld, nfft / 8));
             LAUNCHCHK(launch_csdm_bf16(lc(), Xs, Xt, nch, pairs, nfft, (double *)g.cmH.p, nfft, split2, h_init));
             continue;
@@ -2071,7 +2089,7 @@
             double *Sl = (double *)((char *)g.cmO.p + b_sp), *st = (double *)((char *)g.cmO.p + b_sp + b_sl);
             void *Wf_d;
             if (get_window_spectrum(win, nfft, xf, &Wf_d)) return -1;
-            LAUNCHCHK(launch_welch_pipe(lc(), xd, cplx, (const float *)win_d, hop, nframes, tb.f, xf, (float *)acc, rp, spartial, 2));
+            PIPECHK(launch_welch_pipe(lc(), xd, cplx, (const float *)win_d, hop, nframes, tb.f, xf, (float *)acc, rp, spartial, 2));
             LAUNCHCHK(launch_cm_blocksums(lc(), spartial, 1, (int)rp.groups, hop, Sl));
             LAUNCHCHK(launch_op_finish_channels(lc(), xd, 0, 1, tb.f, (const float *)win_d, Sl, (const cf *)Wf_d, hop, nframes, nsig, xf,
                                                 st, cplx));
@@ -2084,7 +2102,7 @@
             return 0;
         }
         if (pipe) {
-            LAUNCHCHK(launch_welch_pipe(lc(), xd, cplx, (const float *)win_d, hop, nframes, tb.f, xf, (float *)acc, rp, nullptr, 2));
+            PIPECHK(launch_welch_pipe(lc(), xd, cplx, (const float *)win_d, hop, nframes, tb.f, xf, (float *)acc, rp, nullptr, 2));
             generic = 0;
         } else if (!segmean && detrend != 2 && !env_flag("SP_COG_GENERIC"))
             generic = launch_cog_carry(lc(), xd, cplx, (const float *)win_d, hop, nframes, tb.f, xf, acc, rp, klo, khi);
```

Result: slower. 453,100 (-7.1%).
